# AdvancedPhotonSource/tike

Measured on AMD Instinct MI355X. Metric: diffraction patterns/sec/GPU (256x256, 8-mode probe), higher is better.
Workload: dtype c64; 1 GPU; c3; positions_per_gpu=10000, modes=8, detector=256, eigen_probes=1, solver=lstsq_grad, num_batch=10, chunk_positions=1000, position_correction=False, object_update=after every minibatch (batch_method wobbly_center), route=no_farplane

## Files before the change

include/tike_amd.h:

```cpp
#ifndef TIKE_AMD_H
#define TIKE_AMD_H

#ifdef __cplusplus
extern "C" {
#endif

#define TIKE_ERR_ARG 1000001
#define TIKE_ERR_UNSUPPORTED 1000002
#define TIKE_ERR_COMM 2000000
#define TIKE_COMM_ID_BYTES 128

#define TIKE_ABI_VERSION 25

const char* tike_build_id(void);

int tike_abi_version(void);

int tike_set_deterministic(int on, void* scratch, long bytes);

int tike_init(void);

int tike_patch_fwd(const void* images, void* patches, const float* positions, int nimage, int H,
                   int W, int nscan, int nrepeat, int patch_width, int padded_width,
                   void* stream);
// ... 219 lines not shown

int tike_gen_inv_rows_gradients(const void* hand2, const void* patches, const void* probe,
                                int probe_per_scan, const void* unique, const void* eigen_probe,
                                const float* eigen_weights, int num_eigen, int eigen_modes,
                                void* objproj, void* chi0, void* m_probe_update,
                                float probe_update_scale, int nscan, int S, int pw, int det,
                                float inv_scale, void* stream);

int tike_pfa_supported(int S, int pw, int det);

int tike_pfa_fwd_gather(const void* psi, const float* scan, const void* probe,
                        int probe_per_scan, const void* unique, const void* eigen_probe,
                        const float* eigen_weights, int num_eigen, int eigen_modes,
                        void* subtiles, void* patches, int nscan, int S, int pw, int det, int H,
                        int W, void* stream);

int tike_pfa_fft2(const void* in, void* out, long ntile, int det, int inverse, void* stream);

int tike_pfa_fwd_subtiles_supported(int S, int pw, int det);
int tike_pfa_fwd_subtiles(const void* psi, const float* scan, const void* probe,
                          const void* eigen_probe, const float* eigen_weights, int num_eigen,
                          int eigen_modes, void* probe_scratch, void* subtiles, void* patches,
                          int nscan, int S, int pw, int det, int H, int W, void* stream);

int tike_pfa_combine_gradient(void* subtiles, const float* data, const unsigned char* measured,
                              float* costs, int nscan, int S, int det, float fwd_scale, int model,
                              float unmeasured_scaling, long num_measured, int apply_gradient,
                              void* stream);

int tike_pfa_inv_products(const void* subtiles, const void* patches, const void* probe,
                          int probe_per_scan, const void* unique, const void* eigen_probe,
                          const float* eigen_weights, int num_eigen, int eigen_modes,
                          void* objproj, void* chi0, void* m_probe_update,
                          float probe_update_scale, int nscan, int S, int pw, int det,
                          float inv_scale, void* stream);


int tike_fft2_pass1(const void* in, void* out, long ntile, int det, int inverse, void* stream);

int tike_fft2_pass2_inplace(void* tiles, long ntile, int det, int inverse, float scale,
                            void* stream);

int tike_slice_step(void* wave, const void* psi, const float* scan, void* farplane1, int nscan,
                    int S, int det, int H, int W, float scale, void* stream);

int tike_slice_step_back(const void* work, const void* psi, const float* scan, const void* beam,
                         void* objproj, void* farplane1, int nscan, int S, int det, int H, int W,
                         float inv_scale, void* stream);

int tike_fft2_pass2_intensity(void* tiles, float* amplitude, long nscan, int S, int det,
                              int inverse, float scale, int keep, void* stream);

int tike_fresnel_colpass(const void* colin, const void* propagator, int adjoint, void* work,
                         long ntile, int det, float scale, void* stream);

int tike_ifft2_pass2_products(void* work, const void* psi, const float* scan, const void* probe,
                              int probe_per_scan, void* objproj, void* probe_numerator,
                              float numerator_scale, void* chi0, int keep_chi, int nscan, int S,
                              int det, int H, int W, float inv_scale, void* stream);

int tike_fresnel_spect_prop(const void* in, void* out, const void* propagator, long ntile, int n,
                            int adjoint, float fwd_scale, float inv_scale, void* stream);


int tike_object_update_precond(const float* acc, const void* precond, const float* pmax,
                               float alpha, void* upd_sum, void* upd_precond, float* combined,
                               long npix, void* stream);

int tike_lstsq_step_sums(const float* stats, const float* costs, int B, float eps, float* sums,
                         void* stream);
int tike_lstsq_step_solve(const float* stats, int B, float eps, const float* sums, double count,
                          int recover_psi, int recover_probe, float* out, void* stream);

int tike_probe_update(void* probe, void* combined, const void* mpu, const float* beta,
                      float inv_num_batch, long n, void* stream);

int tike_eigen_weights0(float* weights, const float* stats, int B, int C, int S, int m,
                        float* norms, void* stream);
int tike_eigen_proj_mean(const float* first, int first_stride, const float* weights_c,
                         long weights_row, const float* norm, long P, int B, float* pm,
                         void* stream);
int tike_eigen_normalise(void* eigen, const void* update, double count, float beta, int npix,
                         float* esum, float* work, void* stream);
int tike_eigen_dsum(const float* sums, int B, long P, float* dsum, void* stream);
int tike_eigen_weights(const float* sums, int B, long P, const float* dsum, double count,
                       float* weights_c, long weights_row, void* coefs_c, int coef_stride,
                       const float* esum, void* stream);

int tike_cgrad_direction(const float* update_planar, const void* update_complex, void* gradient,
                         void* direction, long n, int first, const float* costs, int ncost,
                         double count, double* state, double* sums, void* stream);

int tike_cgrad_line_search(int variable, const void* x, const void* d, void* xs,
                           const void* other, const float* scan, const void* data,
                           int data_u16, void* scratch, float* costs, int nscan, int chunk,
                           int S, int det, int H, int W, float fwd_scale, double count,
                           double* state, int* skip, int nslots, void* stream);

int tike_cgrad_line_search_masked(int variable, const void* x, const void* d, void* xs,
                                  const void* other, const float* scan, const void* data,
                                  int data_u16, void* scratch, float* costs, int nscan, int chunk,
                                  int S, int det, int H, int W, float fwd_scale, double count,
                                  double* state, int* skip, int nslots,
                                  const unsigned char* measured, int model, long num_measured,
                                  void* stream);

int tike_cgrad_line_search_linear(int variable, const void* x, const void* d, void* xs,
                                  const void* other, const float* scan, const void* data,
                                  int data_u16, void* far_a, int a_valid, void* far_b,
                                  float* costs_k, int nscan, int chunk, int S, int det, int H,
                                  int W, float fwd_scale, double count, double* state,
                                  int stage, double* sums, void* stream);

int tike_cgrad_line_search_linear_masked(int variable, const void* x, const void* d, void* xs,
                                         const void* other, const float* scan, const void* data,
                                         int data_u16, void* far_a, int a_valid, void* far_b,
                                         float* costs_k, int nscan, int chunk, int S, int det,
                                         int H, int W, float fwd_scale, double count,
                                         double* state, int stage, double* sums,
                                         const unsigned char* measured, int model,
                                         long num_measured, void* stream);

int tike_eigen_pixel_update1(const void* patches, const void* chi0, const void* mpu0,
                             const void* eigen0, const float* eigen_proj,
                             const float* weights_c, long weights_row, const float* norm,
                             void* update, int nscan, int pw, int chi_modes, const float* stats,
                             const float* costs, float eps, float* sums3, const void* psi,
                             const float* scan, int H, int W, void* stream);
int tike_lstsq_tail_mid(void* eigen0, const void* update, int npix, float* nacc,
                        float beta_eigen, const float* stats, int B, float eps,
                        const float* sums3, double count, int recover_psi, int recover_probe,
                        float* tail3, void* stream);
int tike_eigen_position_sums1(const void* patches, const void* chi0, const void* mpu0,
                              const void* eigen0, float* sums5, float* dsum, int nscan, int pw,
                              int chi_modes, const void* psi, const float* scan, int H, int W,
                              void* stream);
int tike_lstsq_tail_finish(const float* tail3, const float* sums3, double count, float* steps,
                           void* probe, void* combined, const void* mpu, float inv_num_batch,
                           long nprobe, float* weights, long weights_row, int S, int m,
                           const float* stats, const float* sums5, int B, int npix,
                           void* stream);

int tike_ifft2_pass2_gradients_eproj(const void* work, const void* patches, const void* probe,
                                     const void* eigen_probe, const float* eigen_weights,
                                     int num_eigen, int eigen_modes, void* objproj, void* chi0,
                                     void* m_probe_update, float mpu_scale, int nscan, int S,
                                     int det, float inv_scale, float* qtab, float* q,
                                     void* stream);
int tike_eigen_pixel_update1q(const void* patches, const void* chi0, const void* mpu0,
                              const void* eigen0, const float* q, const float* weights_c,
                              long weights_row, const float* norm, void* update, int nscan,
                              int pw, int chi_modes, const void* psi, const float* scan, int H,
                              int W, float* c0part, float* eproj_out, void* stream);
int tike_lstsq_step_stats_eigen1(const void* chi, const float* scan,
                                 const void* object_update_precond, const void* probe,
                                 const void* eigen_probe, const float* eigen_weights,
                                 int eigen_modes, const void* m_probe_update, const void* patches,
                                 const void* update, float* nacc, double count, float beta_eigen,
                                 float* stats, float* sums5, int nscan, int S, int chi_modes,
                                 int pw, int H, int W, void* stream);
int tike_lstsq_tail_solve1(void* eigen0, const void* update, int npix, const float* nacc,
                           float beta_eigen, const float* stats, const float* costs,
                           const float* sums5, int B, float eps, double count, int recover_psi,
                           int recover_probe, float* sums3, float* tail3, void* stream);

int tike_lstsq_chunk_gradients(const void* psi, const float* scan, const void* probe,
                               const void* eigen_probe, const float* eigen_weights,
                               int num_eigen, int eigen_modes, const void* data, int data_u16,
                               const unsigned char* measured, int model,
                               float unmeasured_scaling, long num_measured, void* scratch,
                               void* work, float* gscale, void* patches, float* costs,
                               void* objproj, void* chi0, void* m_probe_update,
                               float mpu_scale, float* object_acc, int nscan, int S, int det,
                               int H, int W, float fwd_scale, float inv_scale, void* stream);

int tike_lstsq_chunk_gradients_positions(
    const void* psi, const float* scan, const void* probe, const void* eigen_probe,
    const float* eigen_weights, int num_eigen, int eigen_modes, const void* data, int data_u16,
    const unsigned char* measured, int model, float unmeasured_scaling, long num_measured,
    void* scratch, void* work, float* gscale, void* patches, float* costs, void* objproj,
    void* chi0, void* m_probe_update, float mpu_scale, float* object_acc, int nscan, int S,
    int det, int H, int W, float fwd_scale, float inv_scale, const float* taps, int taps_radius,
    float* intensity_work, float* numerator, float* denominator, void* stream);

int tike_position_pd_sums(const void* far0, const void* far_dx, const void* far_dy,
                          const void* data, int data_u16, float inv_dx, float* sums,
                          float* costs, long nscan, int S, long npix, void* stream);

int tike_fly_farplane_gradient(void* farplane, const void* data, int data_u16,
                               const unsigned char* measured, float* intensity, float* costs,
                               int nframe, int fly, int S, int det, int model,
                               int apply_gradient, float unmeasured_scaling, long num_measured,
                               void* stream);

int tike_farplane_scale(void* farplane, const float* table, long nframe, int P, long npix,
                        float scale, void* stream);

int tike_scan_gradient(const void* objproj, const float* scan, const void* psi, float* grad,
                       long nscan, int pw, int H, int W, void* stream);

int tike_scan_gradient_slices(const void* objproj, long slice_stride, const float* scan,
                              const void* psi, float* grad, long nscan, int D, int pw, int H,
                              int W, void* stream);

int tike_eigen_probe_gradients(const void* chi, const float* scan, const void* psi,
                               const void* probe, const void* eigen_probe,
                               const float* eigen_weights, int num_eigen, int eigen_modes,
                               void* probe_grad, void* eigen_grad, float* weights_grad,
                               void* objproj, void* work, long nscan, int S, int pw, int H,
                               int W, void* stream);

int tike_conv_fwd_tangent(const void* psi, const void* dpsi, const float* scan,
                          const float* dscan, const void* probe, const void* dprobe,
                          void* nearplane, long nscan, int S, int pw, int det, int H, int W,
                          void* stream);

int tike_slice_wave_tangent(const void* psi, const void* dpsi, const float* scan,
                            const float* dscan, const void* beam, int beam_per_scan,
                            const void* dbeam, int dbeam_per_scan, void* dwave, long nscan,
                            int S, int pw, int H, int W, void* stream);

int tike_eigen_wave_tangent(const void* psi, const void* dpsi, const float* scan,
                            const float* dscan, const void* probe, const void* dprobe,
                            const void* eigen_probe, const void* deigen_probe,
                            const float* eigen_weights, const float* deigen_weights,
                            int num_eigen, int eigen_modes, void* nearplane, long nscan, int S,
                            int pw, int det, int H, int W, void* stream);

int tike_intensity_tangent(const void* farplane, const void* dfarplane, float* intensity,
                           float* dintensity, long nframe, int P, long npix, void* stream);

int tike_cost_factor(const void* farplane, const void* data, int data_u16,
                     const unsigned char* measured, const float* upstream, float* costs,
                     float* table, long nframe, int P, long npix, int model,
                     long num_measured, void* stream);

int tike_cost_curvature(const void* farplane, const void* dfarplane, const void* data,
                        int data_u16, const unsigned char* measured, const float* upstream,
                        float* costs, float* dcosts, float* table, long nframe, int P,
                        long npix, int model, float floor, long num_measured, void* stream);


int tike_dm_reflect(const void* psi, const float* scan, const void* probe, const void* waves,
                    void* nearplane, float relaxation, long nscan, int S, int pw, int det, int H,
                    int W, void* stream);

int tike_dm_update(void* waves, const void* chi, const void* psi, const float* scan,
                   const void* probe, float relaxation, double* change, long nscan, int S,
                   int pw, int det, int H, int W, void* stream);

int tike_comm_unique_id(void* id);
int tike_comm_create(const void* id, int nranks, int rank, void** comm);
int tike_comm_destroy(void* comm);
int tike_comm_allreduce_sum(void* comm, void* buf, long count, int f64, void* stream);
int tike_comm_broadcast(void* comm, void* buf, long nbytes, int root, void* stream);

int tike_cluster_farthest_fill(const float* points, long n, long* owner, int num_cluster,
                               long turns);
int tike_cluster_swap_sweep(const double* dist, long n, int k, long* label, const long* best,
                            const long* order, double* regret, int* moved);

#ifdef __cplusplus
}
#endif
#endif
```

tike_amd/_lib.py:

```python
import ctypes
import os
import re

import torch

_HERE = os.path.dirname(os.path.abspath(__file__))
LIB_PATH = os.environ.get("TIKE_AMD_LIB") or os.path.join(
    _HERE, "csrc", "libtike_amd.so")
HEADER_PATH = os.path.join(os.path.dirname(_HERE), "include", "tike_amd.h")

ABI_VERSION = 25
ERR_ARG = 1000001
ERR_UNSUPPORTED = 1000002
ERR_COMM = 2000000
COMM_ID_BYTES = 128

if not os.path.isfile(LIB_PATH):
    raise ImportError(
        f"{LIB_PATH} not found: build the HIP library first "
        "(`make -C tike_amd/csrc` or `python -c 'import __graft_entry__ as g; "
        "g.build()'`). tike_amd has no CPU fallback.")

lib = ctypes.CDLL(LIB_PATH)

_p = ctypes.c_void_p
_i = ctypes.c_int
_l = ctypes.c_long
_f = ctypes.c_float
_d = ctypes.c_double

_PROTOTYPES = {
    "tike_abi_version": [],
    "tike_max_grid_dim_y": [],
    "tike_init": [],
    "tike_set_deterministic": [_i, _p, _l],
    "tike_patch_fwd": [_p, _p, _p, _i, _i, _i, _i, _i, _i, _i, _p],
    "tike_patch_adj": [_p, _p, _p, _i, _i, _i, _i, _i, _i, _i, _i, _p],
    "tike_conv_fwd": [_p, _p, _p, _i, _p, _i, _i, _i, _i, _i, _i, _p],
    "tike_conv_adj": [_p, _p, _p, _i, _p, _i, _i, _i, _i, _i, _i, _p],
    "tike_conv_adj_probe": [_p, _p, _p, _p, _i, _i, _i, _i, _i, _i, _p],
    "tike_fft2": [_p, _p, _l, _i, _i, _f, _p],
    "tike_fft2_supported": [_i],
    "tike_fft2_general": [_p, _p, _l, _i, _i, _f, _i, _i, _p],
    "tike_pfa_supported": [_i, _i, _i],
    "tike_pfa_fwd_gather": [_p, _p, _p, _i, _p, _p, _p, _i, _i, _p, _p, _i, _i, _i,
                            _i, _i, _i, _p],
    "tike_pfa_fwd_subtiles_supported": [_i, _i, _i],
    "tike_pfa_fwd_subtiles": [_p, _p, _p, _p, _p, _i, _i, _p, _p, _p, _i, _i,
                              _i, _i, _i, _i, _p],
    "tike_pfa_fft2": [_p, _p, _l, _i, _i, _p],
    "tike_pfa_combine_gradient": [_p, _p, _p, _p, _i, _i, _i, _f, _i, _f, _l, _i,
                                  _p],
    "tike_pfa_inv_products": [_p, _p, _p, _i, _p, _p, _p, _i, _i, _p, _p, _p, _f,
                              _i, _i, _i, _i, _f, _p],
    "tike_gen_supported": [_i, _i, _i],
    "tike_gen_fwd_rows": [_p, _p, _p, _i, _p, _p, _p, _i, _i, _p, _p, _i, _i, _i,
                          _i, _i, _i, _p],
    "tike_gen_cols_gradient": [_p, _p, _p, _p, _p, _i, _i, _i, _i, _f, _i, _f,
                               _l, _p],
    "tike_gen_inv_rows_gradients": [_p, _p, _p, _i, _p, _p, _p, _i, _i, _p, _p,
                                    _p, _f, _i, _i, _i, _i, _f, _p],
    "tike_fresnel_spect_prop": [_p, _p, _p, _l, _i, _i, _f, _f, _p],
    "tike_fft2_pass1": [_p, _p, _l, _i, _i, _p],
    "tike_fft2_pass2_inplace": [_p, _l, _i, _i, _f, _p],
    "tike_slice_step": [_p, _p, _p, _p, _i, _i, _i, _i, _i, _f, _p],
    "tike_slice_step_back": [_p, _p, _p, _p, _p, _p, _i, _i, _i, _i, _i, _f,
                             _p],
    "tike_fft2_pass2_intensity": [_p, _p, _l, _i, _i, _i, _f, _i, _p],
    "tike_fresnel_colpass": [_p, _p, _i, _p, _l, _i, _f, _p],
    "tike_ifft2_pass2_products": [_p, _p, _p, _p, _i, _p, _p, _f, _p, _i, _i, _i,
                                  _i, _i, _i, _f, _p],
    "tike_ptycho_fwd": [_p, _p, _p, _i, _p, _p, _i, _i, _p, _i, _i, _i, _i,
                        _i, _i, _f, _i, _p],
    "tike_ptycho_adj": [_p, _p, _i, _p, _p, _p, _p, _p, _p, _i, _i, _i, _i, _i,
                        _i, _f, _i, _p],
    "tike_ifft2_crop": [_p, _p, _p, _l, _i, _i, _f, _p],
    "tike_ptycho_fwd_intensity": [_p, _p, _p, _i, _p, _p, _i, _i, _p, _p, _p,
                                  _i, _i, _i, _i, _i, _i, _f, _p],
    "tike_gradient_scale": [_p, _p, _p, _p, _p, _i, _i, _i, _f, _l, _p],
    "tike_ifft2_crop_scaled": [_p, _p, _i, _p, _p, _l, _i, _i, _f, _p],
    "tike_ifft2_crop_scaled_modes": [_p, _p, _p, _p, _i, _p, _p, _l, _i, _i, _f,
                                     _p],
    "tike_poisson_steps": [_p, _p, _p, _p, _p, _i, _i, _i, _f, _f, _i, _p],
    "tike_poisson_steps_handoff": [_p, _p, _i, _p, _p, _p, _p, _p, _i, _i, _i, _f,
                                   _f, _l, _f, _f, _p],
    "tike_scale_modes": [_p, _p, _p, _l, _i, _p],
    "tike_ptycho_fwd_intensity_only": [_p, _p, _p, _i, _p, _p, _i, _i, _p, _p,
                                       _i, _i, _i, _i, _i, _i, _f, _p],
    "tike_ptycho_fwd_gradient_scale": [_p, _p, _p, _i, _p, _p, _i, _i, _p, _p,
                                       _p, _p, _p, _p, _p, _i, _i, _i, _i, _i,
                                       _i, _f, _i, _f, _l, _p],
    "tike_fwd_pass1": [_p, _p, _p, _i, _p, _p, _p, _i, _i, _p, _p, _i, _i, _i,
                       _i, _i, _i, _p],
    "tike_fwd_gradient_scale": [_p, _p, _i, _p, _p, _p, _p, _p, _i, _i, _i, _f,
                                _i, _f, _l, _p],
    "tike_grad_ifft2_pass1": [_p, _p, _p, _p, _i, _p, _l, _i, _f, _p],
    "tike_fwd_grad_ifft2_pass1": [_p, _p, _i, _p, _p, _p, _i, _i, _i, _f, _i, _f,
                                  _l, _p],
    "tike_fwd_grad_ifft2_pass1_slices": [_p, _p, _i, _p, _p, _p, _i, _i, _i, _f, _i, _f,
                                  _l, _p, _i, _p],
    "tike_ifft2_pass1_scaled": [_p, _p, _p, _p, _i, _p, _l, _i, _p],
    "tike_ifft2_pass2_gradients": [_p, _p, _p, _p, _p, _i, _i, _p, _p, _p, _f,
                                   _i, _i, _i, _f, _p],
    "tike_ifft2_pass2_gradients_scaled": [_p, _p, _p, _p, _p, _i, _i, _p, _p,
                                          _p, _f, _i, _i, _i, _f, _p, _p],
    "tike_ifft2_pass2_eigen_fits": [_i, _i, _i],
    "tike_ifft2_pass2_gradients_modes": [_p, _p, _p, _p, _p, _i, _i, _p, _p,
                                         _p, _f, _i, _i, _i, _f, _i, _i, _i, _p],
    "tike_poisson_steps_grad_ifft2_pass1": [_p, _p, _i, _p, _p, _p, _p, _p, _i,
                                            _i, _i, _f, _f, _l, _f, _f, _p],
    "tike_object_update_precond": [_p, _p, _p, _f, _p, _p, _p, _l, _p],
    "tike_lstsq_step_sums": [_p, _p, _i, _f, _p, _p],
    "tike_lstsq_step_solve": [_p, _i, _f, _p, _d, _i, _i, _p, _p],
    "tike_probe_update": [_p, _p, _p, _p, _f, _l, _p],
    "tike_eigen_weights0": [_p, _p, _i, _i, _i, _i, _p, _p],
    "tike_eigen_proj_mean": [_p, _i, _p, _l, _p, _l, _i, _p, _p],
    "tike_eigen_normalise": [_p, _p, _d, _f, _i, _p, _p, _p],
    "tike_eigen_dsum": [_p, _i, _l, _p, _p],
    "tike_eigen_weights": [_p, _i, _l, _p, _d, _p, _l, _p, _i, _p, _p],
    "tike_grad_ifft2_crop": [_p, _p, _p, _p, _i, _p, _p, _l, _i, _i, _f, _f,
                             _p],
    "tike_position_sums": [_p, _p, _i, _p, _p, _p, _i, _i, _p, _i, _p, _p, _i,
                           _i, _i, _p],
    "tike_rpie_position_sums": [_p, _p, _p, _p, _i, _p, _p, _i, _i, _p, _i, _p,
                                _p, _p, _i, _i, _i, _i, _i, _p],
    "tike_farplane_gradient": [_p, _p, _p, _p, _p, _i, _i, _i, _i, _i, _f, _l,
                               _p],
    "tike_intensity": [_p, _p, _l, _i, _l, _p],
    "tike_cost_each_pattern": [_p, _p, _p, _l, _l, _i, _p],
    "tike_objective_grad": [_p, _p, _p, _p, _l, _i, _l, _i, _p],
    "tike_lstsq_gradients": [_p, _p, _p, _p, _p, _p, _i, _i, _p, _p, _p, _p, _i,
                             _i, _i, _i, _i, _p],
    "tike_varying_probe": [_p, _p, _p, _i, _i, _p, _i, _i, _i, _p],
    "tike_scatter_patches": [_p, _p, _p, _i, _i, _i, _i, _p],
    "tike_eigen_position_sums": [_p, _p, _p, _p, _p, _i, _i, _i, _p, _i, _i,
                                 _i, _p],
    "tike_eigen_pixel_update": [_p, _p, _p, _p, _p, _i, _i, _i, _p, _p, _i, _i,
                                _i, _p],
    "tike_probe_grad": [_p, _p, _p, _p, _p, _i, _i, _i, _i, _i, _p],
    "tike_probe_preconditioner": [_p, _p, _p, _i, _i, _i, _i, _p],
    "tike_psi_preconditioner": [_p, _p, _p, _i, _i, _i, _i, _p],
    "tike_scatter_amplitudes": [_p, _p, _p, _i, _i, _i, _i, _p],
    "tike_lstsq_step_stats": [_p, _p, _p, _p, _p, _p, _p, _i, _i, _p, _p, _p,
                              _p, _i, _i, _i, _i, _i, _i, _p, _p, _p],
    "tike_eigen_pixel_update1": [_p, _p, _p, _p, _p, _p, _l, _p, _p, _i, _i, _i,
                                 _p, _p, _f, _p, _p, _p, _i, _i, _p],
    "tike_lstsq_tail_mid": [_p, _p, _i, _p, _f, _p, _i, _f, _p, _d, _i, _i, _p,
                            _p],
    "tike_eigen_position_sums1": [_p, _p, _p, _p, _p, _p, _i, _i, _i, _p, _p,
                                  _i, _i, _p],
    "tike_lstsq_tail_finish": [_p, _p, _d, _p, _p, _p, _p, _f, _l, _p, _l, _i,
                               _i, _p, _p, _i, _i, _p],
    "tike_ifft2_pass2_gradients_eproj": [_p, _p, _p, _p, _p, _i, _i, _p, _p,
                                         _p, _f, _i, _i, _i, _f, _p, _p, _p],
    "tike_eigen_pixel_update1q": [_p, _p, _p, _p, _p, _p, _l, _p, _p, _i, _i,
                                  _i, _p, _p, _i, _i, _p, _p, _p],
    "tike_lstsq_step_stats_eigen1": [_p, _p, _p, _p, _p, _p, _i, _p, _p, _p,
                                     _p, _d, _f, _p, _p, _i, _i, _i, _i, _i,
                                     _i, _p],
    "tike_lstsq_tail_solve1": [_p, _p, _i, _p, _f, _p, _p, _p, _i, _f, _d, _i,
                               _i, _p, _p, _p],
    "tike_lstsq_chunk_gradients": [_p, _p, _p, _p, _p, _i, _i, _p, _i, _p, _i,
                                   _f, _l, _p, _p, _p, _p, _p, _p, _p, _p, _f,
                                   _p, _i, _i, _i, _i, _i, _f, _f, _p],
    "tike_lstsq_chunk_gradients_positions": [
        _p, _p, _p, _p, _p, _i, _i, _p, _i, _p, _i, _f, _l, _p, _p, _p, _p, _p,
        _p, _p, _p, _f, _p, _i, _i, _i, _i, _i, _f, _f, _p, _i, _p, _p, _p, _p],
    "tike_cgrad_direction": [_p, _p, _p, _p, _l, _i, _p, _i, _d, _p, _p, _p],
    "tike_cgrad_line_search": [_i, _p, _p, _p, _p, _p, _p, _i, _p, _p, _i, _i,
                               _i, _i, _i, _i, _f, _d, _p, _p, _i, _p],
    "tike_cgrad_line_search_linear": [_i, _p, _p, _p, _p, _p, _p, _i, _p, _i, _p,
                                      _p, _i, _i, _i, _i, _i, _i, _f, _d, _p, _i,
                                      _p, _p],
    "tike_cgrad_line_search_masked": [_i, _p, _p, _p, _p, _p, _p, _i, _p, _p,
                                      _i, _i, _i, _i, _i, _i, _f, _d, _p, _p,
                                      _i, _p, _i, _l, _p],
    "tike_cgrad_line_search_linear_masked": [_i, _p, _p, _p, _p, _p, _p, _i, _p,
                                             _i, _p, _p, _i, _i, _i, _i, _i, _i,
                                             _f, _d, _p, _i, _p, _p, _i, _l, _p],
    "tike_position_pd_sums": [_p, _p, _p, _p, _i, _f, _p, _p, _l, _i, _l, _p],
    "tike_fly_farplane_gradient": [_p, _p, _i, _p, _p, _p, _i, _i, _i, _i, _i,
                                   _i, _f, _l, _p],
    "tike_farplane_scale": [_p, _p, _l, _i, _l, _f, _p],
    "tike_scan_gradient": [_p, _p, _p, _p, _l, _i, _i, _i, _p],
    "tike_scan_gradient_slices": [_p, _l, _p, _p, _p, _l, _i, _i, _i, _i, _p],
    "tike_eigen_probe_gradients": [_p, _p, _p, _p, _p, _p, _i, _i, _p, _p, _p,
                                   _p, _p, _l, _i, _i, _i, _i, _p],
    "tike_conv_fwd_tangent": [_p, _p, _p, _p, _p, _p, _p, _l, _i, _i, _i, _i,
                              _i, _p],
    "tike_slice_wave_tangent": [_p, _p, _p, _p, _p, _i, _p, _i, _p, _l, _i, _i,
                                _i, _i, _p],
    "tike_intensity_tangent": [_p, _p, _p, _p, _l, _i, _l, _p],
    "tike_eigen_wave_tangent": [_p, _p, _p, _p, _p, _p, _p, _p, _p, _p, _i, _i,
                                _p, _l, _i, _i, _i, _i, _i, _p],
    "tike_cost_factor": [_p, _p, _i, _p, _p, _p, _p, _l, _i, _l, _i, _l, _p],
    "tike_cost_curvature": [_p, _p, _p, _i, _p, _p, _p, _p, _p, _l, _i, _l, _i,
                            _f, _l, _p],
    "tike_dm_reflect": [_p, _p, _p, _p, _p, _f, _l, _i, _i, _i, _i, _i, _p],
    "tike_dm_update": [_p, _p, _p, _p, _p, _f, _p, _l, _i, _i, _i, _i, _i, _p],
    "tike_comm_unique_id": [_p],
    "tike_comm_create": [_p, _i, _i, ctypes.POINTER(_p)],
    "tike_comm_destroy": [_p],
    "tike_comm_allreduce_sum": [_p, _p, _l, _i, _p],
    "tike_comm_broadcast": [_p, _p, _l, _i, _p],
    "tike_cluster_farthest_fill": [_p, _l, _p, _i, _l],
    "tike_cluster_swap_sweep": [_p, _l, _i, _p, _p, _p, _p, _p],
}


def build_id():
    try:
        fn = lib.tike_build_id
    except AttributeError:
        return ""
    fn.restype = ctypes.c_char_p
    fn.argtypes = []
    return fn().decode()


def declared_symbols():
    with open(HEADER_PATH) as f:
        text = f.read()
    return sorted(set(re.findall(r"^int\s+(tike_\w+)\s*\(", text, flags=re.M)))


for _name, _args in _PROTOTYPES.items():
    try:
        _fn = getattr(lib, _name)
    except AttributeError as e:
        raise ImportError(
            f"{LIB_PATH} does not export {_name}: it was built from another "
            "include/tike_amd.h; rebuild it (`make -C tike_amd/csrc`).") from e
    _fn.argtypes = _args
    _fn.restype = ctypes.c_int


def _check_abi_version():
    got = lib.tike_abi_version()
    m = re.search(r"^#define\s+TIKE_ABI_VERSION\s+(\d+)", open(HEADER_PATH).read(),
                  flags=re.M) if os.path.isfile(HEADER_PATH) else None
    if got != ABI_VERSION or (m and int(m.group(1)) != ABI_VERSION):
        raise ImportError(
            f"{LIB_PATH} reports ABI version {got}, include/tike_amd.h "
            f"{m.group(1) if m else '?'}, this binding expects {ABI_VERSION}: "
            "rebuild the library (`make -C tike_amd/csrc`).")


_check_abi_version()


def check(rc, what=""):
    if rc == 0:
        return
    if rc == ERR_ARG:
        raise ValueError(f"{what}: incompatible shapes / arguments")
    if rc == ERR_UNSUPPORTED:
        raise ValueError(f"{what}: unsupported size for the HIP path")
    if rc >= ERR_COMM:
        raise RuntimeError(f"{what}: RCCL error {rc - ERR_COMM}")
    raise RuntimeError(f"{what}: HIP error {rc}")


DETERMINISTIC = os.environ.get("TIKE_DETERMINISTIC", "0") == "1"
DETERMINISTIC_SCRATCH_MIB = int(os.environ.get("TIKE_DETERMINISTIC_MIB", "256"))
_det_scratch = None


def ensure_deterministic():
    global _det_scratch
    if not DETERMINISTIC:
        return
    current = torch.cuda.current_device()
    if _det_scratch is not None and _det_scratch.device.index == current:
        return
    if _det_scratch is not None:
        torch.cuda.synchronize(_det_scratch.device)
    _det_scratch = torch.empty(DETERMINISTIC_SCRATCH_MIB << 20,
                               dtype=torch.uint8,
                               device=torch.device("cuda", current))
    check(lib.tike_set_deterministic(1, _det_scratch.data_ptr(),
                                     _det_scratch.numel()),
          "tike_set_deterministic")
```

tike_amd/csrc/lstsq.hip:

```cpp
#include <type_traits>

#include "internal.h"
#include "tike_amd.h"

template <bool HAVE_PATCHES, bool HAVE_GOBJ>
__device__ __forceinline__ void step_stats_item(
    const cf* __restrict__ chi, const float* __restrict__ scan, const cf* __restrict__ psi,
    const cf* __restrict__ gobj, const TkProbe& probe, const cf* __restrict__ mpu,
    const cf* __restrict__ patches, float* __restrict__ stats, int chi_modes, int pw, int H,
    int W, const cf* __restrict__ eigen0, float* __restrict__ eigen_proj, int nsplit, int n,
    int part, float* red) {
  const long P = (long)pw * pw;
  const long total = (long)H * W;
  const int plen = (int)(P / nsplit);
  {
    const TkCorner c = tk_corner(scan, n);
    const cf* __restrict__ pbase = probe.probe + n * probe.pos_stride;
    float pw0 = 1.0f, pw1 = 0.f;
    int nE = 0;
    const float* __restrict__ wn = nullptr;
    if (probe.weights != nullptr) {
      if (probe.unique != nullptr && 0 < probe.Sm) {
        pbase = probe.unique + (long)n * probe.Sm * P;
      } else {
        wn = probe.weights + n * (long)(probe.C + 1) * probe.S;
        pw0 = wn[0];
        if (probe.eigen != nullptr && 0 < probe.Sm) {
          nE = probe.C;
          pw1 = wn[probe.S];
        }
      }
    }
    float a[8] = {0.f, 0.f, 0.f, 0.f, 0.f, 0.f, 0.f, 0.f};
    float ep = 0.f;
    const int qstep = (int)blockDim.x / pw, rstep = (int)blockDim.x % pw;
    const int pbeg = part * plen + (int)threadIdx.x;
    const int pend = part + 1 == nsplit ? (int)P : (part + 1) * plen;
    int py = pbeg / pw, px = pbeg % pw;
    const bool interior = HAVE_GOBJ && c.sy >= 0 && c.sx >= 0 && c.sy + pw < H && c.sx + pw < W &&
                          total < (1L << 28);
    const bool same_e = eigen_proj != nullptr && nE > 0 && eigen0 == probe.eigen;
    const bool same_p = pbase == probe.probe;
    auto body = [&](auto k_tag) {
      constexpr int K = decltype(k_tag)::value;
      constexpr bool FAST = K >= 1;
      constexpr bool HOT = K >= 2;
#pragma unroll 2
      for (int p = pbeg; p < pend; p += blockDim.x) {
        cf o, g;
        if (FAST) {
          typedef float tk_v4f __attribute__((ext_vector_type(4)));
          const unsigned off =
              (unsigned)((c.sy + py) * W + c.sx + px) * (unsigned)sizeof(cf);
          tk_v4f u, l;
          __builtin_memcpy(&u, reinterpret_cast<const char*>(gobj) + off, sizeof(u));
          __builtin_memcpy(&l, reinterpret_cast<const char*>(gobj) + off + (unsigned)W * 8u,
                           sizeof(l));
          if (HAVE_PATCHES) {
            o = patches[n * P + p];
          } else {
            tk_v4f uo, lo_;
            __builtin_memcpy(&uo, reinterpret_cast<const char*>(psi) + off, sizeof(uo));
            __builtin_memcpy(&lo_, reinterpret_cast<const char*>(psi) + off + (unsigned)W * 8u,
                             sizeof(lo_));
            o = mk(uo.x * c.w00, uo.y * c.w00);
            o.x += uo.z * c.w01;
            o.y += uo.w * c.w01;
            o.x += lo_.x * c.w10;
            o.y += lo_.y * c.w10;
            o.x += lo_.z * c.w11;
            o.y += lo_.w * c.w11;
          }
          g = mk(u.x * c.w00, u.y * c.w00);
          g.x += u.z * c.w01;
          g.y += u.w * c.w01;
          g.x += l.x * c.w10;
          g.y += l.y * c.w10;
          g.x += l.z * c.w11;
          g.y += l.w * c.w11;
        } else {
          const int y = c.sy + py, x = c.sx + px;
          const bool ok = y >= 0 && y < H && x >= 0 && x < W;
          const int yc = y < 0 ? 0 : (y >= H ? H - 1 : y);
          const int xc = x < 0 ? 0 : (x >= W ? W - 1 : x);
          const long ii = (long)yc * W + xc;
          o = HAVE_PATCHES ? patches[n * P + p] : tk_gather(psi, ii, W, total, c);
          g = HAVE_GOBJ ? tk_gather(gobj, ii, W, total, c) : mk(0.f, 0.f);
          if (!ok) {
            if (!HAVE_PATCHES) o = mk(0.f, 0.f);
            g = mk(0.f, 0.f);
          }
        }
        const cf x0 = chi[((long)n * chi_modes) * P + p];
        const cf p0 = probe.probe[p];
        cf pn = (HOT ? p0 : pbase[p]) * pw0;
        cf e1 = mk(0.f, 0.f);
        if (K == 3) {
          e1 = probe.eigen[p];
          pn.x += pw1 * e1.x;
          pn.y += pw1 * e1.y;
        } else if (K < 2 && nE > 0) {
          e1 = probe.eigen[p];
          pn.x += pw1 * e1.x;
          pn.y += pw1 * e1.y;
          for (int e = 1; e < nE; ++e) {
            const cf ee = probe.eigen[(long)e * probe.Sm * P + p];
            const float we = wn[(e + 1) * probe.S];
            pn.x += we * ee.x;
            pn.y += we * ee.y;
          }
        }
        const cf dOP = g * pn;
        const cf m0 = HOT ? mpu[p] : (mpu ? mpu[p] : mk(0.f, 0.f));
        const cf dPO = m0 * o;
        const cf OP = o * p0;
        a[0] += norm2(dOP);
        a[1] += norm2(dPO);
        const cf a2 = dOP * conjf(dPO);
        a[2] += a2.x;
        a[3] += a2.y;
        a[4] += dOP.x * x0.x + dOP.y * x0.y;
        a[5] += dPO.x * x0.x + dPO.y * x0.y;
        a[6] += OP.x * x0.x + OP.y * x0.y;
        a[7] += norm2(OP);
        if (K == 3) {
          const cf r = conjf(o) * x0 - m0;
          ep += r.x * e1.x + r.y * e1.y;
        } else if (K < 2 && eigen_proj) {
          const cf r = conjf(o) * x0 - m0;
          const cf e = same_e ? e1 : eigen0[p];
          ep += r.x * e.x + r.y * e.y;
        }
        py += qstep;
        px += rstep;
        if (px >= pw) {
          px -= pw;
          ++py;
        }
      }
    };
    const bool hot = interior && same_p && mpu != nullptr;
    if (hot && nE == 1 && same_e)
      body(std::integral_constant<int, 3>{});
    else if (hot && nE == 0 && eigen_proj == nullptr)
      body(std::integral_constant<int, 2>{});
    else if (interior)
      body(std::integral_constant<int, 1>{});
    else
      body(std::integral_constant<int, 0>{});
#pragma unroll
    for (int k = 0; k < 8; ++k) {
      const float t = tk_block_sum256(a[k], red);
      if (threadIdx.x == 0) {
        if (nsplit > 1)
          unsafeAtomicAdd(&stats[(long)n * 8 + k], t);
// ... 188 lines not shown
    }
  }
}

extern "C" int tike_lstsq_step_stats(const void* chi, const float* scan, const void* psi,
                                     const void* object_update_precond, const void* probe,
                                     const void* eigen_probe, const float* eigen_weights,
                                     int num_eigen, int eigen_modes, const void* unique_probe,
                                     const void* m_probe_update, const void* patches,
                                     float* stats, int nscan, int S, int chi_modes, int pw, int H,
                                     int W, const void* eigen0, float* eigen_proj, void* stream) {
  TK_ENTER();
  TK_CHECK_ARG(nscan >= 0 && S >= 1 && chi_modes >= 1 && pw >= 1 && H >= 1 && W >= 1);
  if (nscan == 0) return TK_OK;
  TK_CHECK_ARG(chi && scan && psi && probe && stats);
  TK_CHECK_ARG(!eigen_proj || (eigen0 && m_probe_update));
  const TkProbe pr = tk_make_probe(probe, 0, eigen_probe, eigen_weights, num_eigen, eigen_modes,
                                   S, pw, unique_probe);
  const bool no_eigen = (eigen_probe == nullptr || eigen_modes == 0) && eigen_proj == nullptr;
  const bool one_eigen = eigen_probe != nullptr && eigen_weights != nullptr && eigen_modes > 0 &&
                         num_eigen == 1 && eigen_proj != nullptr && eigen0 == eigen_probe;
  const bool pairs = g_stats_pairs && patches && object_update_precond && m_probe_update &&
                     unique_probe == nullptr && (no_eigen || one_eigen) &&
                     (long)H * W < (1L << 28) && nscan > 1;
  const long nitem = pairs ? (nscan + 1) / 2 : nscan;
  int nsplit = 1;
  while (nsplit < 16 && nitem * nsplit * 2 <= 8192 && ((long)pw * pw) % (2048L * nsplit) == 0)
    nsplit *= 2;
  if (tk_deterministic()) nsplit = 1;
  if (nsplit > 1) {
    hipError_t e = hipMemsetAsync(stats, 0, sizeof(float) * 8 * (size_t)nscan, (hipStream_t)stream);
    if (e == hipSuccess && eigen_proj)
      e = hipMemsetAsync(eigen_proj, 0, sizeof(float) * (size_t)nscan, (hipStream_t)stream);
    if (e != hipSuccess) return (int)e;
  }
#define TK_SS(HP, HG)                                                                         \
  hipLaunchKernelGGL((step_stats_kernel<HP, HG>), dim3(tk_grid((long)nscan * nsplit, 16)),    \
                     dim3(256), 0,                                                            \
                     (hipStream_t)stream, (const cf*)chi, scan, (const cf*)psi,               \
                     (const cf*)object_update_precond, pr, (const cf*)m_probe_update,         \
                     (const cf*)patches, stats, nscan, chi_modes, pw, H, W, (const cf*)eigen0, \
                     eigen_proj, nsplit)
#define TK_SP(EIG)                                                                            \
  hipLaunchKernelGGL((step_stats_pair_kernel<EIG>), dim3(tk_grid(nitem * nsplit, 16)),        \
                     dim3(256), 0,                                                            \
                     (hipStream_t)stream, (const cf*)chi, scan, (const cf*)psi,               \
                     (const cf*)object_update_precond, pr, (const cf*)m_probe_update,         \
                     (const cf*)patches, stats, nscan, chi_modes, pw, H, W, (const cf*)eigen0, \
                     eigen_proj, nsplit)
  if (pairs && one_eigen) TK_SP(true);
  else if (pairs) TK_SP(false);
  else if (patches && object_update_precond) TK_SS(true, true);
  else if (patches) TK_SS(true, false);
  else if (object_update_precond) TK_SS(false, true);
  else TK_SS(false, false);
#undef TK_SS
#undef TK_SP
  TK_LAUNCH_CHECK();
  return TK_OK;
}

struct TkResidual {
  const cf* patches;
  const cf* chi0;
  const cf* mpu0;
  const cf* eigen;
  const cf* coefs;
  int C, Sm, c;
  long P;
  long XS;
  template <bool C0>
  __device__ __forceinline__ cf at(long n, long p) const {
    cf r = conjf(patches[n * P + p]) * chi0[n * XS + p] - mpu0[p];
    if (!C0)
      for (int k = 0; k < c; ++k) r = r - coefs[n * C + k] * eigen[((long)k * Sm) * P + p];
    return r;
  }
};

template <bool C0>
__global__ __launch_bounds__(256) void eigen_position_sums_kernel(const TkResidual R,
                                                                  float* __restrict__ sums,
                                                                  int nscan) {
  __shared__ float red[4];
  const cf* __restrict__ E = R.eigen + ((long)R.c * R.Sm) * R.P;
  for (int n = blockIdx.x; n < nscan; n += gridDim.x) {
    float a[5] = {0.f, 0.f, 0.f, 0.f, 0.f};
    for (long p = threadIdx.x; p < R.P; p += blockDim.x) {
      const cf e = E[p];
      const cf r = R.at<C0>(n, p);
      const cf phi = R.patches[n * R.P + p] * e;
      const cf x = R.chi0[n * R.XS + p];
      a[0] += r.x * e.x + r.y * e.y;
      a[1] += x.x * phi.x + x.y * phi.y;
      a[2] += norm2(phi);
      const cf re = r * conjf(e);
      a[3] += re.x;
      a[4] += re.y;
    }
#pragma unroll
    for (int k = 0; k < 5; ++k) {
      const float v = tk_block_sum256(a[k], red);
      if (threadIdx.x == 0) sums[(long)n * 5 + k] = v;
    }
  }
}

template <bool C0>
__global__ __launch_bounds__(256) void eigen_pixel_update_kernel(const TkResidual R,
                                                                 const float* __restrict__ pm,
                                                                 float* __restrict__ update,
                                                                 int nscan, int chunk,
                                                                 float* __restrict__ part) {
  const long p = (long)blockIdx.x * blockDim.x + threadIdx.x;
  if (p >= R.P) return;
  const int b0 = blockIdx.y * chunk;
  const int b1 = min(nscan, b0 + chunk);
  cf acc = mk(0.f, 0.f);
#pragma unroll 4
  for (int n = b0; n < b1; ++n) {
    const cf r = R.at<C0>(n, p);
    const float w = pm[n];
    acc.x += r.x * w;
    acc.y += r.y * w;
  }
  if (part != nullptr) {
    part[2 * ((long)blockIdx.y * R.P + p)] = acc.x;
    part[2 * ((long)blockIdx.y * R.P + p) + 1] = acc.y;
    return;
  }
  unsafeAtomicAdd(&update[2 * p], acc.x);
  unsafeAtomicAdd(&update[2 * p + 1], acc.y);
}

__device__ __forceinline__ cf tk_patch_pixel(const cf* __restrict__ psi, unsigned off,
                                             unsigned row_bytes, const TkCorner& c) {
  typedef float tk_v4f __attribute__((ext_vector_type(4)));
  tk_v4f u, l;
  __builtin_memcpy(&u, reinterpret_cast<const char*>(psi) + off, sizeof(u));
  __builtin_memcpy(&l, reinterpret_cast<const char*>(psi) + off + row_bytes, sizeof(l));
  cf o = mk(u.x * c.w00, u.y * c.w00);
  o.x += u.z * c.w01;
  o.y += u.w * c.w01;
  o.x += l.x * c.w10;
  o.y += l.y * c.w10;
  o.x += l.z * c.w11;
  o.y += l.w * c.w11;
  return o;
}
__device__ __forceinline__ bool tk_interior(const TkCorner& c, int pw, int H, int W) {
  return c.sy >= 0 && c.sx >= 0 && c.sy + pw < H && c.sx + pw < W && (long)H * W < (1L << 28);
}

constexpr int TK_C0_PARTS = 64;
__global__ __launch_bounds__(256) void eigen_proj_offset_kernel(const cf* __restrict__ mpu0,
                                                                const cf* __restrict__ E,
                                                                long P,
                                                                float* __restrict__ part) {
  __shared__ float red[4];
  float a = 0.f;
  for (long p = blockIdx.x * 256L + threadIdx.x; p < P; p += 256L * TK_C0_PARTS) {
    const cf m = mpu0[p], e = E[p];
    a += m.x * e.x + m.y * e.y;
  }
  a = tk_block_sum256(a, red);
  if (threadIdx.x == 0) part[blockIdx.x] = a;
}

__global__ __launch_bounds__(256) void eigen_pixel_update1_kernel(
    const TkResidual R, const float* __restrict__ eproj, const float* __restrict__ weights_c,
    long row, const float* __restrict__ norm, float inv_P, float* __restrict__ update, int nscan,
    int chunk, const float* __restrict__ stats, const float* __restrict__ costs, float eps,
    float* __restrict__ sums3, const cf* __restrict__ psi, const float* __restrict__ scan, int pw,
    int H, int W, float* __restrict__ part, const float* __restrict__ c0part,
    float* __restrict__ eproj_out) {
  float c0 = 0.f;
  if (c0part != nullptr) {
    for (int b = 0; b < TK_C0_PARTS; ++b) c0 += c0part[b];
  }
  if (blockIdx.x + 1 == gridDim.x) {
    if (blockIdx.y != 0) return;
    if (eproj_out != nullptr) {
      for (int n = threadIdx.x; n < nscan; n += 256) eproj_out[n] = eproj[n] - c0;
    }
    if (sums3 == nullptr) return;
    __shared__ float red[4];
    float a1 = 0.f, a4 = 0.f, c = 0.f;
    for (int n = threadIdx.x; n < nscan; n += 256) {
      a1 += stats[8 * n] + eps;
      a4 += stats[8 * n + 1] + eps;
      c += costs[n];
    }
    a1 = tk_block_sum256(a1, red);
    a4 = tk_block_sum256(a4, red);
    c = tk_block_sum256(c, red);
    if (threadIdx.x == 0) {
      sums3[0] = a1;
      sums3[1] = a4;
      sums3[2] = c;
    }
    return;
  }
  const long p = (long)blockIdx.x * blockDim.x + threadIdx.x;
  if (p >= R.P) return;
  const int b0 = blockIdx.y * chunk;
  const int b1 = min(nscan, b0 + chunk);
  const float inv_norm = 1.0f / norm[0];
  cf acc = mk(0.f, 0.f);
  bool gather = psi != nullptr;
  if (gather) {
    for (int n = b0; n < b1; ++n) gather = gather && tk_interior(tk_corner(scan, n), pw, H, W);
  }
  if (gather) {
    const int py = (int)(p / pw), px = (int)(p % pw);
    const unsigned row_bytes = (unsigned)W * (unsigned)sizeof(cf);
    const unsigned lane_off = (unsigned)py * row_bytes + (unsigned)px * (unsigned)sizeof(cf);
    const cf m0 = R.mpu0[p];
#pragma unroll 4
    for (int n = b0; n < b1; ++n) {
      const TkCorner c = tk_corner(scan, n);
      const cf x = R.chi0[n * R.XS + p];
      const cf o = tk_patch_pixel(
          psi, (unsigned)(c.sy * W + c.sx) * (unsigned)sizeof(cf) + lane_off, row_bytes, c);
      const cf r = conjf(o) * x - m0;
      const float w = ((eproj[n] - c0) * inv_P + weights_c[n * row]) * inv_norm;
      acc.x += r.x * w;
      acc.y += r.y * w;
    }
  } else {
#pragma unroll 4
    for (int n = b0; n < b1; ++n) {
      const cf r = R.at<true>(n, p);
      const float w = ((eproj[n] - c0) * inv_P + weights_c[n * row]) * inv_norm;
      acc.x += r.x * w;
      acc.y += r.y * w;
    }
  }
  if (part != nullptr) {
    part[2 * ((long)blockIdx.y * R.P + p)] = acc.x;
    part[2 * ((long)blockIdx.y * R.P + p) + 1] = acc.y;
    return;
  }
  unsafeAtomicAdd(&update[2 * p], acc.x);
  unsafeAtomicAdd(&update[2 * p + 1], acc.y);
}

__global__ __launch_bounds__(256) void column_sum_ordered_kernel(const float* __restrict__ table,
                                                                 int stride, int col, int n,
                                                                 float scale,
                                                                 float* __restrict__ out) {
  __shared__ float red[4];
  float a = 0.f;
  for (int i = threadIdx.x; i < n; i += 256) a += table[(long)i * stride + col] * scale;
  a = tk_block_sum256(a, red);
  if (threadIdx.x == 0) out[0] += a;
}

__global__ __launch_bounds__(256) void eigen_position_sums1_kernel(
    const TkResidual R, float* __restrict__ sums, float* __restrict__ dsum, int nscan,
    const cf* __restrict__ psi, const float* __restrict__ scan, int pw, int H, int W) {
  __shared__ float red[4];
  const cf* __restrict__ E = R.eigen;
  const unsigned row_bytes = (unsigned)W * (unsigned)sizeof(cf);
  const int qstep = (int)blockDim.x / pw, rstep = (int)blockDim.x % pw;
  for (int n = blockIdx.x; n < nscan; n += gridDim.x) {
    float a[5] = {0.f, 0.f, 0.f, 0.f, 0.f};
    TkCorner c = {0, 0, 0.f, 0.f, 0.f, 0.f};
    if (psi != nullptr) c = tk_corner(scan, n);
    const bool gather = psi != nullptr && tk_interior(c, pw, H, W);
    const unsigned off0 = gather ? (unsigned)(c.sy * W + c.sx) * (unsigned)sizeof(cf) : 0u;
    auto body = [&](auto g_tag) {
      constexpr bool G = decltype(g_tag)::value;
      int py = (int)threadIdx.x / pw, px = (int)threadIdx.x % pw;
      for (long p = threadIdx.x; p < R.P; p += blockDim.x) {
        const cf e = E[p];
        const cf x = R.chi0[n * R.XS + p];
        const cf m0 = R.mpu0[p];
        cf o;
        if constexpr (G)
          o = tk_patch_pixel(psi, off0 + (unsigned)py * row_bytes + (unsigned)px * 8u, row_bytes, c);
        else
          o = R.patches[n * R.P + p];
        const cf r = conjf(o) * x - m0;
        const cf phi = o * e;
        py += qstep;
        px += rstep;
        if (px >= pw) {
          px -= pw;
          ++py;
        }
        a[0] += r.x * e.x + r.y * e.y;
        a[1] += x.x * phi.x + x.y * phi.y;
        a[2] += norm2(phi);
        const cf re = r * conjf(e);
        a[3] += re.x;
        a[4] += re.y;
      }
    };
    if (gather)
      body(std::true_type{});
    else
      body(std::false_type{});
#pragma unroll
    for (int k = 0; k < 5; ++k) {
      const float v = tk_block_sum256(a[k], red);
      if (threadIdx.x == 0) {
        sums[(long)n * 5 + k] = v;
        if (k == 2 && dsum != nullptr) unsafeAtomicAdd(dsum, v / (float)R.P);
      }
    }
  }
}

__global__ __launch_bounds__(512) void eigen_position_sums1_pair_kernel(
    const TkResidual R, float* __restrict__ sums, float* __restrict__ dsum, int nscan,
    const cf* __restrict__ psi, const float* __restrict__ scan, int pw, int H, int W) {
  __shared__ float red[8];
  typedef float tk_v4f __attribute__((ext_vector_type(4)));
  const cf* __restrict__ E = R.eigen;
// ... 100 lines not shown
  const float mu = sqrtf(uu * inv_count * inv_count / (float)P);
  const float kk = beta / mu * inv_count;
  const float inv = 1.0f / sqrtf((ee + 2.0f * kk * eu + kk * kk * uu) / (float)P);
  auto enew = [&](const cf e, const long p) { return (e + update[p] * kk) * inv; };
  auto esum = [](float* a, const cf o, const cf x, const cf e, const cf m0) {
    const cf r = conjf(o) * x - m0;
    const cf phi = o * e;
    a[0] += r.x * e.x + r.y * e.y;
    a[1] += x.x * phi.x + x.y * phi.y;
    a[2] += norm2(phi);
    a[3] += r.y * e.x - r.x * e.y;
  };
  auto put = [&](float* dst, const float v) {
    if (nsplit > 1)
      unsafeAtomicAdd(dst, v);
    else
      *dst = v;
  };
  auto finish5 = [&](const float* a, const int n) {
    float t[4];
#pragma unroll
    for (int k = 0; k < 4; ++k) t[k] = tk_block_sum256(a[k], red);
    if (threadIdx.x == 0) {
      float* o = sums5 + (long)n * 5;
      put(o, t[0]);
      put(o + 1, t[1]);
      put(o + 2, t[2]);
      put(o + 3, t[0]);
      put(o + 4, t[3]);
    }
  };
  for (int v = blockIdx.x; v < npair * nsplit; v += gridDim.x) {
    const int n0 = 2 * (v / nsplit), part = v % nsplit;
    const TkCorner c0 = tk_corner(scan, n0);
    const bool two = n0 + 1 < nscan;
    const TkCorner c1 = tk_corner(scan, two ? n0 + 1 : n0);
    const bool in0 = c0.sy >= 0 && c0.sx >= 0 && c0.sy + pw < H && c0.sx + pw < W;
    const bool in1 = c1.sy >= 0 && c1.sx >= 0 && c1.sy + pw < H && c1.sx + pw < W;
    const int pbeg = part * plen + (int)threadIdx.x;
    const int pend = part + 1 == nsplit ? (int)P : (part + 1) * plen;
    if (!(two && in0 && in1)) {
      for (int i = 0; i < (two ? 2 : 1); ++i) {
        const int n = n0 + i;
        step_stats_item<true, true>(chi, scan, nullptr, gobj, probe, mpu, patches, stats,
                                    chi_modes, pw, H, W, nullptr, nullptr, nsplit, n, part, red);
        float a[4] = {0.f, 0.f, 0.f, 0.f};
        for (int p = pbeg; p < pend; p += blockDim.x)
          esum(a, patches[(long)n * P + p], chi[(long)n * chi_modes * P + p],
               enew(probe.eigen[p], p), mpu[p]);
        finish5(a, n);
      }
      continue;
    }
    float s0 = 1.0f, s1 = 1.0f, t0 = 0.f, t1 = 0.f;
    if (probe.weights != nullptr) {
      const float* w = probe.weights + n0 * (long)(probe.C + 1) * probe.S;
      s0 = w[0];
      s1 = w[(long)(probe.C + 1) * probe.S];
      t0 = w[probe.S];
      t1 = w[(long)(probe.C + 1) * probe.S + probe.S];
    }
    float a[8] = {0.f, 0.f, 0.f, 0.f, 0.f, 0.f, 0.f, 0.f};
    float b[8] = {0.f, 0.f, 0.f, 0.f, 0.f, 0.f, 0.f, 0.f};
    float ea[4] = {0.f, 0.f, 0.f, 0.f}, eb[4] = {0.f, 0.f, 0.f, 0.f};
    const unsigned base0 = (unsigned)(c0.sy * W + c0.sx), base1 = (unsigned)(c1.sy * W + c1.sx);
    const cf* __restrict__ chi_a = chi + ((long)n0 * chi_modes) * P;
    const cf* __restrict__ chi_b = chi + ((long)(n0 + 1) * chi_modes) * P;
    const cf* __restrict__ pat_a = patches + (long)n0 * P;
    const cf* __restrict__ pat_b = pat_a + P;
    auto tap = [](const tk_v4f u, const tk_v4f l, const TkCorner& c) {
      cf g = mk(u.x * c.w00, u.y * c.w00);
      g.x += u.z * c.w01;
      g.y += u.w * c.w01;
      g.x += l.x * c.w10;
      g.y += l.y * c.w10;
      g.x += l.z * c.w11;
      g.y += l.w * c.w11;
      return g;
    };
    auto sums = [](float* acc, const cf g, const cf o, const cf x0, const cf p0, const cf pn,
                   const cf m0) {
      const cf dOP = g * pn;
      const cf dPO = m0 * o;
      const cf OP = o * p0;
      acc[0] += norm2(dOP);
      acc[1] += norm2(dPO);
      const cf a2 = dOP * conjf(dPO);
      acc[2] += a2.x;
      acc[3] += a2.y;
      acc[4] += dOP.x * x0.x + dOP.y * x0.y;
      acc[5] += dPO.x * x0.x + dPO.y * x0.y;
      acc[6] += OP.x * x0.x + OP.y * x0.y;
      acc[7] += norm2(OP);
    };
    auto pixel = [&](const int p, const tk_v4f u0, const tk_v4f l0, const tk_v4f u1,
                     const tk_v4f l1) {
      const cf oa = pat_a[p], ob = pat_b[p];
      const cf xa = chi_a[p], xb = chi_b[p];
      const cf p0 = probe.probe[p];
      const cf m0 = mpu[p];
      const cf e1 = probe.eigen[p];
      const cf en = enew(e1, p);
      cf pa = p0 * s0, pb = p0 * s1;
      pa.x += t0 * e1.x;
      pa.y += t0 * e1.y;
      pb.x += t1 * e1.x;
      pb.y += t1 * e1.y;
      sums(a, tap(u0, l0, c0), oa, xa, p0, pa, m0);
      sums(b, tap(u1, l1, c1), ob, xb, p0, pb, m0);
      esum(ea, oa, xa, en, m0);
      esum(eb, ob, xb, en, m0);
    };
    auto taps16 = [&](const unsigned off) {
      tk_v4f t;
      __builtin_memcpy(&t, reinterpret_cast<const char*>(gobj) + off, sizeof(t));
      return t;
    };
    const int cols = pw < 256 ? pw : 256, groups = 256 / cols;
    const int rows = pw / (nsplit * groups);
    const int ybeg = (part * groups + (int)threadIdx.x / cols) * rows;
    for (int x = (int)threadIdx.x % cols; x < pw; x += 256) {
      unsigned rel = (unsigned)(ybeg * W + x);
      tk_v4f u0 = taps16((base0 + rel) * 8u), u1 = taps16((base1 + rel) * 8u);
      int p = ybeg * pw + x;
#pragma unroll 2
      for (int y = 0; y < rows; ++y) {
        rel += (unsigned)W;
        const tk_v4f l0 = taps16((base0 + rel) * 8u), l1 = taps16((base1 + rel) * 8u);
        pixel(p, u0, l0, u1, l1);
        u0 = l0;
        u1 = l1;
        p += pw;
      }
    }
#pragma unroll
    for (int k = 0; k < 8; ++k) {
      const float ta = tk_block_sum256(a[k], red);
      const float tb = tk_block_sum256(b[k], red);
      if (threadIdx.x == 0) {
        put(&stats[(long)n0 * 8 + k], ta);
        put(&stats[(long)n0 * 8 + 8 + k], tb);
      }
    }
    finish5(ea, n0);
    finish5(eb, n0 + 1);
  }
}

__global__ __launch_bounds__(256) void eigen_norm_sums1_kernel(const cf* __restrict__ E,
                                                               const cf* __restrict__ update,
                                                               int npix, float* __restrict__ nacc,
                                                               float* __restrict__ part) {
  __shared__ float red[4];
  float uu = 0.f, ee = 0.f, eu = 0.f;
  for (int i = blockIdx.x * 256 + threadIdx.x; i < npix; i += gridDim.x * 256) {
    const cf e = E[i], u = update[i];
    uu += norm2(u);
    ee += norm2(e);
    eu += e.x * u.x + e.y * u.y;
  }
  uu = tk_block_sum256(uu, red);
  ee = tk_block_sum256(ee, red);
  eu = tk_block_sum256(eu, red);
  if (threadIdx.x == 0) {
    if (part != nullptr) {
      part[3 * blockIdx.x] = uu;
      part[3 * blockIdx.x + 1] = ee;
      part[3 * blockIdx.x + 2] = eu;
    } else {
      unsafeAtomicAdd(&nacc[0], uu);
      unsafeAtomicAdd(&nacc[1], ee);
      unsafeAtomicAdd(&nacc[2], eu);
    }
  }
}

extern "C" int tike_lstsq_step_stats_eigen1(const void* chi, const float* scan,
                                            const void* object_update_precond, const void* probe,
                                            const void* eigen_probe, const float* eigen_weights,
                                            int eigen_modes, const void* m_probe_update,
                                            const void* patches, const void* update, float* nacc,
                                            double count, float beta_eigen, float* stats,
                                            float* sums5, int nscan, int S, int chi_modes,
                                            int pw, int H, int W, void* stream) {
  TK_ENTER();
  TK_CHECK_ARG(nscan >= 0 && S >= 1 && chi_modes >= 1 && pw >= 1 && H >= 1 && W >= 1 &&
               eigen_modes >= 1 && count > 0);
  TK_CHECK_ARG(probe && eigen_probe && eigen_weights && m_probe_update && update && nacc);
  const long P = (long)pw * pw;
  const long nitem = (nscan + 1) / 2;
  int nsplit = 1;
  while (nsplit < 16 && nitem * nsplit * 2 <= 8192 && P % (2048L * nsplit) == 0) nsplit *= 2;
  if (tk_deterministic()) nsplit = 1;
  const int groups = 256 / (pw < 256 ? pw : 256);
  if (!((pw % 256 == 0 || 256 % pw == 0) && pw % (nsplit * groups) == 0 &&
        (long)H * W < (1L << 28)))
    return TK_ERR_UNSUPPORTED;
  int grid = P >= 256 * 64 ? 64 : (int)((P + 255) / 256);
  float* part = nullptr;
  if (tk_deterministic()) {
    part = tk_det_scratch(sizeof(float) * 3 * (size_t)grid);
    if (part == nullptr) grid = 1;
  }
  hipLaunchKernelGGL(eigen_norm_sums1_kernel, dim3(grid), dim3(256), 0, (hipStream_t)stream,
                     (const cf*)eigen_probe, (const cf*)update, (int)P, nacc, part);
  TK_LAUNCH_CHECK();
  if (part != nullptr) {
    int rc = tk_ordered_sum(nacc, part, 3, grid, true, (hipStream_t)stream);
    if (rc) return rc;
  }
  if (nscan == 0) return TK_OK;
  TK_CHECK_ARG(chi && scan && object_update_precond && patches && stats && sums5);
  const TkProbe pr = tk_make_probe(probe, 0, eigen_probe, eigen_weights, 1, eigen_modes, S, pw,
                                   nullptr);
  if (nsplit > 1) {
    hipError_t e = hipMemsetAsync(stats, 0, sizeof(float) * 8 * (size_t)nscan, (hipStream_t)stream);
    if (e == hipSuccess)
      e = hipMemsetAsync(sums5, 0, sizeof(float) * 5 * (size_t)nscan, (hipStream_t)stream);
    if (e != hipSuccess) return (int)e;
  }
  hipLaunchKernelGGL(step_stats_eigen_pair_kernel, dim3(tk_grid(nitem * nsplit, 16)), dim3(256),
                     0, (hipStream_t)stream, (const cf*)chi, scan,
                     (const cf*)object_update_precond, pr, (const cf*)m_probe_update,
                     (const cf*)patches, (const cf*)update, (const float*)nacc,
                     (float)(1.0 / count), beta_eigen, stats, sums5, nscan, chi_modes, pw, H, W,
                     nsplit);
  TK_LAUNCH_CHECK();
  return TK_OK;
}

static TkResidual make_residual(const void* patches, const void* chi0, const void* mpu0,
                                const void* eigen, const void* coefs, int C, int Sm, int c,
                                int pw, int chi_modes) {
  TkResidual R;
  R.patches = (const cf*)patches;
  R.chi0 = (const cf*)chi0;
  R.mpu0 = (const cf*)mpu0;
  R.eigen = (const cf*)eigen;
  R.coefs = (const cf*)coefs;
  R.C = C;
  R.Sm = Sm;
  R.c = c;
  R.P = (long)pw * pw;
  R.XS = R.P * chi_modes;
  return R;
}

extern "C" int tike_eigen_position_sums(const void* patches, const void* chi0, const void* mpu0,
                                        const void* eigen_probe, const void* coefs,
                                        int num_eigen, int eigen_modes, int c, float* sums,
                                        int nscan, int pw, int chi_modes, void* stream) {
  TK_ENTER();
  TK_CHECK_ARG(nscan >= 0 && pw >= 1 && num_eigen >= 1 && c >= 0 && c < num_eigen &&
               chi_modes >= 1);
  if (nscan == 0) return TK_OK;
  TK_CHECK_ARG(patches && chi0 && mpu0 && eigen_probe && sums && (c == 0 || coefs));
  const TkResidual R = make_residual(patches, chi0, mpu0, eigen_probe, coefs, num_eigen,
                                     eigen_modes, c, pw, chi_modes);
  if (c == 0)
    hipLaunchKernelGGL(eigen_position_sums_kernel<true>, dim3(tk_grid(nscan, 16)), dim3(256), 0,
                       (hipStream_t)stream, R, sums, nscan);
  else
    hipLaunchKernelGGL(eigen_position_sums_kernel<false>, dim3(tk_grid(nscan, 16)), dim3(256),
                       0, (hipStream_t)stream, R, sums, nscan);
  TK_LAUNCH_CHECK();
  return TK_OK;
}

extern "C" int tike_eigen_pixel_update(const void* patches, const void* chi0, const void* mpu0,
                                       const void* eigen_probe, const void* coefs,
                                       int num_eigen, int eigen_modes, int c, const float* pm,
                                       void* update, int nscan, int pw, int chi_modes,
                                       void* stream) {
  TK_ENTER();
  TK_CHECK_ARG(nscan >= 0 && pw >= 1 && num_eigen >= 1 && c >= 0 && c < num_eigen &&
               chi_modes >= 1);
  if (nscan == 0) return TK_OK;
  TK_CHECK_ARG(patches && chi0 && mpu0 && eigen_probe && pm && update && (c == 0 || coefs));
  const long P = (long)pw * pw;
  float* part = nullptr;
  const int chunk = probe_chunk(nscan, 2 * P, &part);
  dim3 grid((unsigned)((P + 255) / 256), (unsigned)((nscan + chunk - 1) / chunk));
  const TkResidual R = make_residual(patches, chi0, mpu0, eigen_probe, coefs, num_eigen,
                                     eigen_modes, c, pw, chi_modes);
  if (c == 0)
    hipLaunchKernelGGL(eigen_pixel_update_kernel<true>, grid, dim3(256), 0, (hipStream_t)stream,
                       R, pm, (float*)update, nscan, chunk, part);
  else
    hipLaunchKernelGGL(eigen_pixel_update_kernel<false>, grid, dim3(256), 0,
                       (hipStream_t)stream, R, pm, (float*)update, nscan, chunk, part);
  TK_LAUNCH_CHECK();
  if (part != nullptr)
    return tk_ordered_sum((float*)update, part, 2 * P, (int)grid.y, true, (hipStream_t)stream);
  return TK_OK;
}

extern "C" int tike_eigen_pixel_update1(const void* patches, const void* chi0,
                                        const void* mpu0, const void* eigen0,
                                        const float* eigen_proj, const float* weights_c,
                                        long weights_row, const float* norm, void* update,
                                        int nscan, int pw, int chi_modes, const float* stats,
                                        const float* costs, float eps, float* sums3,
                                        const void* psi, const float* scan, int H, int W,
                                        void* stream) {
  TK_ENTER();
  TK_CHECK_ARG(nscan >= 0 && pw >= 1 && chi_modes >= 1 && weights_row >= 1);
  if (nscan == 0) {
    if (sums3) return (int)hipMemsetAsync(sums3, 0, 3 * sizeof(float), (hipStream_t)stream);
    return TK_OK;
  }
  TK_CHECK_ARG(!sums3 || (stats && costs));
  TK_CHECK_ARG(!psi || (scan && H >= 1 && W >= 1));
  TK_CHECK_ARG(patches && chi0 && mpu0 && eigen0 && eigen_proj && weights_c && norm && update);
  const long P = (long)pw * pw;
  float* part = nullptr;
  const int chunk = probe_chunk(nscan, 2 * P, &part);
  dim3 grid((unsigned)((P + 255) / 256) + 1, (unsigned)((nscan + chunk - 1) / chunk));
  const TkResidual R = make_residual(patches, chi0, mpu0, eigen0, nullptr, 1, 1, 0, pw, chi_modes);
  hipLaunchKernelGGL(eigen_pixel_update1_kernel, grid, dim3(256), 0, (hipStream_t)stream, R,
                     eigen_proj, weights_c, weights_row, norm, 1.0f / (float)P, (float*)update,
                     nscan, chunk, stats, costs, eps, sums3, (const cf*)psi, scan, pw, H, W,
                     part, nullptr, nullptr);
  TK_LAUNCH_CHECK();
  if (part != nullptr)
    return tk_ordered_sum((float*)update, part, 2 * P, (int)grid.y, true, (hipStream_t)stream);
  return TK_OK;
}

extern "C" int tike_eigen_pixel_update1q(const void* patches, const void* chi0,
                                         const void* mpu0, const void* eigen0, const float* q,
                                         const float* weights_c, long weights_row,
                                         const float* norm, void* update, int nscan, int pw,
                                         int chi_modes, const void* psi, const float* scan,
                                         int H, int W, float* c0part, float* eproj_out,
                                         void* stream) {
  TK_ENTER();
  TK_CHECK_ARG(nscan >= 0 && pw >= 1 && chi_modes >= 1 && weights_row >= 1);
  if (nscan == 0) return TK_OK;
  TK_CHECK_ARG(!psi || (scan && H >= 1 && W >= 1));
  TK_CHECK_ARG(patches && chi0 && mpu0 && eigen0 && q && weights_c && norm && update && c0part);
  const long P = (long)pw * pw;
  hipLaunchKernelGGL(eigen_proj_offset_kernel, dim3(TK_C0_PARTS), dim3(256), 0,
                     (hipStream_t)stream, (const cf*)mpu0, (const cf*)eigen0, P, c0part);
  float* part = nullptr;
  const int chunk = probe_chunk(nscan, 2 * P, &part);
  dim3 grid((unsigned)((P + 255) / 256) + 1, (unsigned)((nscan + chunk - 1) / chunk));
  const TkResidual R = make_residual(patches, chi0, mpu0, eigen0, nullptr, 1, 1, 0, pw, chi_modes);
  hipLaunchKernelGGL(eigen_pixel_update1_kernel, grid, dim3(256), 0, (hipStream_t)stream, R, q,
                     weights_c, weights_row, norm, 1.0f / (float)P, (float*)update, nscan, chunk,
                     nullptr, nullptr, 0.f, nullptr, (const cf*)psi, scan, pw, H, W, part,
                     c0part, eproj_out);
  TK_LAUNCH_CHECK();
  if (part != nullptr)
    return tk_ordered_sum((float*)update, part, 2 * P, (int)grid.y, true, (hipStream_t)stream);
  return TK_OK;
}

extern "C" int tike_eigen_position_sums1(const void* patches, const void* chi0,
                                         const void* mpu0, const void* eigen0, float* sums,
                                         float* dsum, int nscan, int pw, int chi_modes,
                                         const void* psi, const float* scan, int H, int W,
                                         void* stream) {
  TK_ENTER();
  TK_CHECK_ARG(nscan >= 0 && pw >= 1 && chi_modes >= 1);
  if (nscan == 0) return TK_OK;
  TK_CHECK_ARG(!psi || (scan && H >= 1 && W >= 1));
  TK_CHECK_ARG(patches && chi0 && mpu0 && eigen0 && sums && dsum);
  const TkResidual R = make_residual(patches, chi0, mpu0, eigen0, nullptr, 1, 1, 0, pw, chi_modes);
  const bool det = tk_deterministic();
  const int cols = pw < 256 ? pw : 256;
  const bool pairs = g_stats_pairs && psi != nullptr && nscan > 1 &&
                     (pw % 256 == 0 || 256 % pw == 0) && pw % (512 / cols) == 0 &&
                     (long)H * W < (1L << 28);
  if (pairs)
    hipLaunchKernelGGL(eigen_position_sums1_pair_kernel, dim3(tk_grid((nscan + 1) / 2, 16)),
                       dim3(512), 0, (hipStream_t)stream, R, sums, det ? nullptr : dsum, nscan,
                       (const cf*)psi, scan, pw, H, W);
  else
    hipLaunchKernelGGL(eigen_position_sums1_kernel, dim3(tk_grid(nscan, 16)), dim3(256), 0,
                       (hipStream_t)stream, R, sums, det ? nullptr : dsum, nscan, (const cf*)psi,
                       scan, pw, H, W);
  if (det)
    hipLaunchKernelGGL(column_sum_ordered_kernel, dim3(1), dim3(256), 0, (hipStream_t)stream, sums,
                       5, 2, nscan, 1.0f / (float)((long)pw * pw), dsum);
  TK_LAUNCH_CHECK();
  return TK_OK;
}

__global__ __launch_bounds__(256) void varying_probe_kernel(const TkProbe probe,
                                                            cf* __restrict__ out, long total,
                                                            long PP) {
  for (long i = blockIdx.x * (long)blockDim.x + threadIdx.x; i < total;
       i += (long)gridDim.x * blockDim.x) {
    const long pix = i % PP;
    const long ns = i / PP;
    out[i] = probe.at(ns / probe.Sm, (int)(ns % probe.Sm), pix);
  }
}

extern "C" int tike_varying_probe(const void* probe, const void* eigen_probe,
                                  const float* eigen_weights, int num_eigen, int eigen_modes,
                                  void* out, int nscan, int S, int pw, void* stream) {
  TK_ENTER();
  TK_CHECK_ARG(nscan >= 0 && S >= 1 && pw >= 1 && eigen_modes >= 1 && eigen_modes <= S);
  if (nscan == 0) return TK_OK;
  TK_CHECK_ARG(probe && eigen_weights && out && (num_eigen == 0 || eigen_probe));
  const long PP = (long)pw * pw;
  const long total = (long)nscan * eigen_modes * PP;
  hipLaunchKernelGGL(varying_probe_kernel, dim3(tk_grid((total + 255) / 256, 16)), dim3(256), 0,
                     (hipStream_t)stream,
                     tk_make_probe(probe, 0, eigen_probe, eigen_weights, num_eigen, eigen_modes,
                                   S, pw),
                     (cf*)out, total, PP);
  TK_LAUNCH_CHECK();
  return TK_OK;
}
```

tike_amd/csrc/lstsq_gradients.hip:

```cpp
#include "fft_engine2.h"
#include <type_traits>

#include "internal.h"
#include "tike_amd.h"

constexpr int TK_MAX_MODES = 16;

template <bool WITH_CHI, int SC>
__global__ __launch_bounds__(256) void probe_grad_kernel(
    const cf* __restrict__ chi, const float* __restrict__ scan, const cf* __restrict__ psi,
    cf* __restrict__ patches, float* __restrict__ out, const TkProbe probe,
    cf* __restrict__ objproj, int nscan, int S_rt, int pw, int H, int W, int chunk,
    float* __restrict__ part) {
  constexpr int SM = SC > 0 ? SC : TK_MAX_MODES;
  const int S = SC > 0 ? SC : S_rt;
  const long P = (long)pw * pw;
  const long total = (long)H * W;
  const long p = (long)blockIdx.x * blockDim.x + threadIdx.x;
  const int b0 = blockIdx.y * chunk;
  const int b1 = min(nscan, b0 + chunk);
  if (p >= P) return;
  const int py = (int)(p / pw), px = (int)(p % pw);
  cf acc[SM];
#pragma unroll
  for (int s = 0; s < SM; ++s) acc[s] = mk(0.f, 0.f);
  const bool hoist = WITH_CHI && objproj != nullptr && probe.pos_stride == 0;
  cf pr[SM];
  if (hoist) {
#pragma unroll
    for (int s = 0; s < SM; ++s)
      if (SC > 0 || s < S) pr[s] = probe.probe[s * P + p];
  }
  for (int b = b0; b < b1; ++b) {
    const TkCorner c = tk_corner(scan, b);
    const int y = c.sy + py, x = c.sx + px;
    const bool ok = y >= 0 && y < H && x >= 0 && x < W;
    const int yc = y < 0 ? 0 : (y >= H ? H - 1 : y);
    const int xc = x < 0 ? 0 : (x >= W ? W - 1 : x);
    cf xs[SM];
    if (WITH_CHI) {
#pragma unroll
      for (int s = 0; s < SM; ++s)
        if (SC > 0 || s < S) xs[s] = tk_ld_stream(chi + ((long)b * S + s) * P + p);
    }
    cf o;
    if (!WITH_CHI && c.sy >= 0 && c.sx >= 0 && c.sy + pw < H && c.sx + pw < W &&
        total < (1L << 28)) {
      typedef float tk_v4f __attribute__((ext_vector_type(4)));
      const unsigned off = (unsigned)(y * W + x) * (unsigned)sizeof(cf);
      tk_v4f u, l;
      __builtin_memcpy(&u, reinterpret_cast<const char*>(psi) + off, sizeof(u));
      __builtin_memcpy(&l, reinterpret_cast<const char*>(psi) + off + (unsigned)W * 8u, sizeof(l));
      o = mk(u.x * c.w00, u.y * c.w00);
      o.x += u.z * c.w01;
      o.y += u.w * c.w01;
      o.x += l.x * c.w10;
      o.y += l.y * c.w10;
      o.x += l.z * c.w11;
      o.y += l.w * c.w11;
    } else {
      o = tk_gather(psi, (long)yc * W + xc, W, total, c);
      if (!ok) o = mk(0.f, 0.f);
    }
    if (patches) patches[b * P + p] = o;
    if (WITH_CHI) {
      const cf oc = conjf(o);
      cf proj = mk(0.f, 0.f);
#pragma unroll
      for (int s = 0; s < SM; ++s)
        if (SC > 0 || s < S) {
          if (out) acc[s] = acc[s] + oc * xs[s];
          if (objproj) {
            cf ps;
            if (hoist && !(probe.weights != nullptr && probe.eigen != nullptr && s < probe.Sm)) {
              const float w0 =
                  probe.weights ? probe.weights[b * (long)(probe.C + 1) * probe.S + s] : 1.0f;
              ps = pr[s] * w0;
            } else {
              ps = probe.at(b, s, p);
            }
            proj = proj + conjf(ps) * xs[s];
          }
        }
      if (objproj) objproj[b * P + p] = proj;
    } else {
      acc[0].x += norm2(o);
    }
  }
  if (WITH_CHI) {
    if (out) {
#pragma unroll
      for (int s = 0; s < SM; ++s)
        if (SC > 0 || s < S) {
          if (part != nullptr) {
            float* o = part + 2 * (((long)blockIdx.y * S + s) * P + p);
            o[0] = acc[s].x;
            o[1] = acc[s].y;
          } else {
            unsafeAtomicAdd(&out[2 * (s * P + p)], acc[s].x);
            unsafeAtomicAdd(&out[2 * (s * P + p) + 1], acc[s].y);
          }
        }
    }
  } else if (part != nullptr) {
    part[(long)blockIdx.y * P + p] = acc[0].x;
  } else {
    unsafeAtomicAdd(&out[2 * p], acc[0].x);
  }
}

template <bool WITH_CHI>
static void launch_probe_grad(dim3 grid, hipStream_t stream, const cf* chi, const float* scan,
                              const cf* psi, cf* patches, float* out, const TkProbe& probe,
                              cf* objproj, int nscan, int S, int pw, int H, int W, int chunk,
                              float* part = nullptr) {
#define TK_PG(SC)                                                                              \
  hipLaunchKernelGGL((probe_grad_kernel<WITH_CHI, SC>), grid, dim3(256), 0, stream, chi, scan, \
                     psi, patches, out, probe, objproj, nscan, S, pw, H, W, chunk, part)
  switch (WITH_CHI ? S : 1) {
    case 1: TK_PG(1); break;
    case 2: TK_PG(2); break;
    case 3: TK_PG(3); break;
    case 4: TK_PG(4); break;
    case 5: TK_PG(5); break;
    case 6: TK_PG(6); break;
    case 8: TK_PG(8); break;
    default: TK_PG(0); break;
  }
#undef TK_PG
}

int probe_chunk(int nscan, long len, float** part) {
  int chunk = (nscan + 31) / 32;
  chunk = chunk < 8 ? 8 : chunk;
  if (!tk_deterministic()) return chunk;
  const int nchunk = (nscan + chunk - 1) / chunk;
  float* p = len > 0 && part ? tk_det_scratch(sizeof(float) * (size_t)len * nchunk) : nullptr;
  if (p != nullptr) {
    *part = p;
    return chunk;
  }
  return nscan > 8 ? nscan : 8;
}

extern "C" int tike_probe_grad(const void* chi, const float* scan, const void* psi,
                               void* patches, void* m_probe_update, int nscan, int S, int pw,
                               int H, int W, void* stream) {
  TK_ENTER();
  TK_CHECK_ARG(nscan >= 0 && S >= 1 && S <= TK_MAX_MODES && pw >= 1 && H >= 1 && W >= 1);
  if (nscan == 0) return TK_OK;
  TK_CHECK_ARG(chi && scan && psi && m_probe_update);
  const long P = (long)pw * pw;
  float* part = nullptr;
  const int chunk = probe_chunk(nscan, 2 * S * P, &part);
  dim3 grid((unsigned)((P + 255) / 256), (unsigned)((nscan + chunk - 1) / chunk));
  launch_probe_grad<true>(grid, (hipStream_t)stream, (const cf*)chi, scan, (const cf*)psi,
// ... 125 lines not shown
#pragma unroll
      for (int yb = 0; yb < RB; ++yb) O[yb] = *tk_at(On + yb * ROW, lo);
    }
    cf* slot = part + ((((n - b0) & (NBUF - 1)) * 4 + w) * RB) * 64 + lane;
    const cf* slots = part + ((((n - b0) & (NBUF - 1)) * 4 + cw * MW) * RB) * 64 + lane;
    const float* __restrict__ wn =
        vary ? probe.weights + n * (long)(probe.C + 1) * probe.S : nullptr;
#pragma unroll
    for (int m = 0; m < MPW; ++m) {
      const int s = mw + MW * m;
      if (s < S) {
        const cf* __restrict__ src = mid + ((long)n * Stot + s) * P + slice0;
        cf u[RB];
#pragma unroll
        for (int k = 0; k < RB; ++k) u[k] = tk_ld_stream(tk_at(src + k * ROW, lo));
        if (HOIST && !O_ONCE) {
#pragma unroll
          for (int yb = 0; yb < RB; ++yb) O[yb] = *tk_at(On + yb * ROW, lo);
        }
        const float w0 = vary ? wn[s] : 1.0f;
        const float sc = mode_scale ? inv_scale * mode_scale[(long)n * Stot + s] : inv_scale;
        Dft<RB, true>::run(u);
        if (HOIST) {
#pragma unroll
          for (int yb = 0; yb < RB; ++yb) {
            u[yb] = u[yb] * sc;
            acc[m][yb] = acc[m][yb] + conjf(O[yb]) * u[yb];
          }
          if (QN && !REDUCE && s == 0) {
            const cf* __restrict__ el = eigl + cw * 64 + lane;
            float q = 0.f;
#pragma unroll
            for (int yb = 0; yb < RB; ++yb) {
              const cf t = conjf(O[yb]) * u[yb];
              const cf e = el[yb * (64 * CW)];
              q += t.x * e.x - t.y * e.y;
            }
            q_store(q, n);
          }
        } else {
#pragma unroll
          for (int g = 0; g < RB; g += 8) {
            cf o[8];
#pragma unroll
            for (int i = 0; i < 8; ++i) o[i] = *tk_at(On + (g + i) * ROW, lo);
#pragma unroll
            for (int i = 0; i < 8; ++i) {
              u[g + i] = u[g + i] * sc;
              acc[m][g + i] = acc[m][g + i] + conjf(o[i]) * u[g + i];
            }
            __builtin_amdgcn_sched_barrier(0);
          }
        }
        if (s == 0 && chi0 != nullptr) {
#pragma unroll
          for (int yb = 0; yb < RB; ++yb)
            tk_st_stream(tk_at(chi0 + (long)n * P + slice0 + yb * ROW, lo), u[yb]);
        }
        if (HAVE_PROJ) {
          const cf* __restrict__ Ps = probe.probe + (long)s * P + slice0;
          const bool eig = EIG && nE > 0 && s < probe.Sm;
#pragma unroll
          for (int g = 0; g < RB; g += 8) {
            cf pc[8];
#pragma unroll
            for (int i = 0; i < 8; ++i)
              pc[i] = HOIST ? Pc[m][g + i] : conjf(*tk_at(Ps + (g + i) * ROW, lo));
#pragma unroll
            for (int i = 0; i < 8; ++i) {
              cf t = (pc[i] * u[g + i]) * w0;
              if (REDUCE) {
                slot[(g + i) * 64] = m == 0 ? t : slot[(g + i) * 64] + t;
              } else {
                if (eig) {
#pragma unroll 1
                  for (int c = 0; c < nE; ++c)
                    t = t + (eigl[((c * probe.Sm + s) * RB + g + i) * (64 * CW) + cw * 64 + lane] *
                             u[g + i]) * wn[(c + 1) * probe.S + s];
                }
                tk_st_stream(tk_at(objproj + (long)n * P + slice0 + (g + i) * ROW, lo), t);
              }
            }
            if (!HOIST) __builtin_amdgcn_sched_barrier(0);
          }
          if (REDUCE && eig) {
#pragma unroll 1
            for (int c = 0; c < nE; ++c) {
              const float wc = wn[(c + 1) * probe.S + s];
              const cf* __restrict__ el =
                  eigl + ((c * probe.Sm + s) * RB) * (64 * CW) + cw * 64 + lane;
              if (QN && c == 0 && s == 0) {
                float q = 0.f;
#pragma unroll
                for (int yb = 0; yb < RB; ++yb) {
                  const cf e = el[yb * (64 * CW)];
                  slot[yb * 64] = slot[yb * 64] + (e * u[yb]) * wc;
                  const cf t = conjf(O[yb]) * u[yb];
                  q += t.x * e.x - t.y * e.y;
                }
                q_store(q, n);
                continue;
              }
#pragma unroll
              for (int yb = 0; yb < RB; ++yb)
                slot[yb * 64] = slot[yb * 64] + (el[yb * (64 * CW)] * u[yb]) * wc;
            }
          }
        }
      } else if (REDUCE && m == 0) {
#pragma unroll
        for (int yb = 0; yb < RB; ++yb) slot[yb * 64] = mk(0.f, 0.f);
      }
    }
    if (REDUCE) {
      __syncthreads();
#pragma unroll
      for (int q = 0; q < RB / MW; ++q) {
        const int yb = mw + MW * q;
        cf sum = slots[yb * 64];
#pragma unroll
        for (int k = 1; k < MW; ++k) sum = sum + slots[(k * RB + yb) * 64];
        if (accumulate) sum = sum + *tk_at(objproj + (long)n * P + slice0 + yb * ROW, lo);
        tk_st_stream(tk_at(objproj + (long)n * P + slice0 + yb * ROW, lo), sum);
      }
      if (NBUF == 1) __syncthreads();
    }
  }
  if (mpu != nullptr) {
#pragma unroll
    for (int m = 0; m < MPW; ++m) {
      const int s = mw + MW * m;
      if (s < S) {
#pragma unroll
        for (int yb = 0; yb < RB; ++yb) {
          if (mpu_part != nullptr) {
            const long ci = (nchunk_ - 1) - b0 / chunk;
            float* o = tk_at(mpu_part + 2 * ((ci * S + s) * P + slice0 + yb * ROW), lb);
            o[0] = acc[m][yb].x * mpu_scale;
            o[1] = acc[m][yb].y * mpu_scale;
          } else {
            float* o = tk_at(mpu + 2 * ((long)s * P + slice0 + yb * ROW), lb);
            unsafeAtomicAdd(o, acc[m][yb].x * mpu_scale);
            unsafeAtomicAdd(o + 1, acc[m][yb].y * mpu_scale);
          }
        }
      }
    }
  }
}

__global__ __launch_bounds__(256) void pass2_q_finish_kernel(const float* __restrict__ qtab,
                                                             int slots, int nscan,
                                                             float* __restrict__ q) {
  const int n = blockIdx.x * 4 + (int)(threadIdx.x >> 6), k = threadIdx.x & 63;
  if (n >= nscan) return;
  float a = k < slots ? qtab[(long)k * nscan + n] : 0.f;
  a = tk_wave_sum(a);
  if (k == 0) q[n] = a;
}

template <int N, int MW_, int MPW_>
static bool launch_pass2_qn(dim3 grid, size_t lds, hipStream_t stream, const cf* work,
                            const cf* patches, const TkProbe& pr, cf* objproj, cf* chi0,
                            float* mpu, float mpu_scale, int nscan, int S, float inv_scale,
                            int chunk, float* mpu_part, const float* mode_scale, float* qtab) {
  if constexpr (N <= 256) {
    hipLaunchKernelGGL((ifft2_pass2_gradients_kernel<N, MW_, MPW_, true, true, false, true>),
                       grid, dim3(256), lds, stream, work, patches, pr, objproj, chi0, mpu,
                       mpu_scale, nscan, S, inv_scale, chunk, mpu_part, mode_scale, 0, 0, qtab);
    return true;
  } else {
    return false;
  }
}

static int launch_pass2_gradients(const void* work, const void* patches, const void* probe,
                                  const void* eigen_probe, const float* eigen_weights,
                                  int num_eigen, int eigen_modes, void* objproj, void* chi0,
                                  void* m_probe_update, float mpu_scale, int nscan, int S,
                                  int det, float inv_scale, const float* mode_scale,
                                  hipStream_t stream, int Stot = 0, int accumulate = 0,
                                  float* qtab = nullptr, float* q = nullptr) {
  TK_CHECK_ARG(nscan >= 0 && S >= 1 && det >= 1);
  if (nscan == 0) return TK_OK;
  TK_CHECK_ARG(work && patches && (probe || !objproj));
  if (S > 8 || (det != 128 && det != 256 && det != 512)) return TK_ERR_UNSUPPORTED;
  const bool qn = q != nullptr;
  TK_CHECK_ARG(!qn || qtab);
  if (qn && (Stot != 0 || det > 256 || !objproj || !eigen_probe || !eigen_weights ||
             num_eigen < 1 || eigen_modes < 1))
    return TK_ERR_UNSUPPORTED;
  const bool grp = Stot != 0;
  if (grp && objproj && S < 2) return TK_ERR_UNSUPPORTED;
  const TkProbe pr = tk_make_probe(probe, 0, eigen_probe, eigen_weights, num_eigen, eigen_modes,
                                   grp ? Stot : S, det);
  int MW = S >= 3 ? 4 : S;
  if (det == 128 && MW == 1) MW = 2;
  auto eig_bytes = [&](int mw) {
    return sizeof(cf) * (size_t)num_eigen * eigen_modes * (det / 16) * 64 * (4 / mw);
  };
  if (objproj && eigen_weights && eigen_probe)
    while (MW < 4 && eig_bytes(MW) > 32 * 1024) MW *= 2;
  const int MPW = S > 4 ? 2 : 1;
  const int nslice = 16 * (det / (64 * (4 / MW)));
  int nchunk = (1024 + nslice - 1) / nslice;
  {
    int unit = 512, a = nslice;
    while (a % 2 == 0 && unit > 1) { a /= 2; unit /= 2; }
    if (nchunk >= unit) nchunk = nchunk / unit * unit;
  }
  int chunk = (nscan + nchunk - 1) / nchunk;
  if (chunk < 8) chunk = 8;
  nchunk = (nscan + chunk - 1) / chunk;
  const dim3 grid((unsigned)(nslice * nchunk)), block(256);
  float* mpu_part = nullptr;
  const long mpu_len = 2L * S * det * det;
  if (m_probe_update && tk_deterministic()) {
    mpu_part = tk_det_scratch(sizeof(float) * (size_t)mpu_len * nchunk);
    if (mpu_part == nullptr) return TK_ERR_ARG;
  }
  size_t eig_lds = 0;
  if (objproj && eigen_weights && eigen_probe) eig_lds = eig_bytes(MW);
  if (eig_lds > 32 * 1024) return TK_ERR_UNSUPPORTED;
#define TK_P2G(N, MW_, MPW_)                                                                 \
  do {                                                                                       \
    if (qn) {                                                                                \
      if (!launch_pass2_qn<N, MW_, MPW_>(grid, eig_lds, stream, (const cf*)work,             \
                                         (const cf*)patches, pr, (cf*)objproj, (cf*)chi0,    \
                                         (float*)m_probe_update, mpu_scale, nscan, S,        \
                                         inv_scale, chunk, mpu_part, mode_scale, qtab))      \
        return TK_ERR_UNSUPPORTED;                                                           \
    } else if (grp && !objproj)                                                              \
      hipLaunchKernelGGL((ifft2_pass2_gradients_kernel<N, MW_, MPW_, false, true, true>),    \
                         grid, block, 0,                                                     \
                         stream, (const cf*)work, (const cf*)patches, pr, (cf*)objproj,      \
                         (cf*)chi0, (float*)m_probe_update, mpu_scale, nscan, S, inv_scale,  \
                         chunk, mpu_part, mode_scale, Stot, accumulate);                     \
    else if (grp && eig_lds > 0)                                                             \
      hipLaunchKernelGGL((ifft2_pass2_gradients_kernel<N, MW_, MPW_, true, true, true>),     \
                         grid, block, eig_lds,                                               \
                         stream, (const cf*)work, (const cf*)patches, pr, (cf*)objproj,      \
                         (cf*)chi0, (float*)m_probe_update, mpu_scale, nscan, S, inv_scale,  \
                         chunk, mpu_part, mode_scale, Stot, accumulate);                     \
    else if (grp)                                                                            \
      hipLaunchKernelGGL((ifft2_pass2_gradients_kernel<N, MW_, MPW_, true, false, true>),    \
                         grid, block, 0,                                                     \
                         stream, (const cf*)work, (const cf*)patches, pr, (cf*)objproj,      \
                         (cf*)chi0, (float*)m_probe_update, mpu_scale, nscan, S, inv_scale,  \
                         chunk, mpu_part, mode_scale, Stot, accumulate);                     \
    else if (objproj && eig_lds > 0)                                                         \
      hipLaunchKernelGGL((ifft2_pass2_gradients_kernel<N, MW_, MPW_, true>), grid, block,    \
                         eig_lds,                                                            \
                         stream, (const cf*)work, (const cf*)patches, pr, (cf*)objproj,      \
                         (cf*)chi0, (float*)m_probe_update, mpu_scale, nscan, S, inv_scale,  \
                         chunk, mpu_part, mode_scale);                                       \
    else if (objproj)                                                                        \
      hipLaunchKernelGGL((ifft2_pass2_gradients_kernel<N, MW_, MPW_, true, false>), grid,    \
                         block, 0,                                                           \
                         stream, (const cf*)work, (const cf*)patches, pr, (cf*)objproj,      \
                         (cf*)chi0, (float*)m_probe_update, mpu_scale, nscan, S, inv_scale,  \
                         chunk, mpu_part, mode_scale);                                       \
    else                                                                                     \
      hipLaunchKernelGGL((ifft2_pass2_gradients_kernel<N, MW_, MPW_, false>), grid, block,   \
                         0, stream, (const cf*)work, (const cf*)patches, pr, (cf*)objproj,   \
                         (cf*)chi0, (float*)m_probe_update, mpu_scale, nscan, S, inv_scale,  \
                         chunk, mpu_part, mode_scale);                                       \
  } while (0)
#define TK_P2G_N(N)                     \
  do {                                  \
    if (MW == 1)                        \
      TK_P2G(N < 256 ? 256 : N, 1, 1);  \
    else if (MW == 2)                   \
      TK_P2G(N, 2, 1);                  \
    else if (MPW == 1)                  \
      TK_P2G(N, 4, 1);                  \
    else                                \
      TK_P2G(N, 4, 2);                  \
  } while (0)
  switch (det) {
    case 128: TK_P2G_N(128); break;
    case 256: TK_P2G_N(256); break;
    default: TK_P2G_N(512); break;
  }
#undef TK_P2G_N
#undef TK_P2G
  TK_LAUNCH_CHECK();
  if (qn) {
    hipLaunchKernelGGL(pass2_q_finish_kernel, dim3((nscan + 3) / 4), dim3(256), 0, stream,
                       qtab, det / 4, nscan, q);
    TK_LAUNCH_CHECK();
  }
  if (mpu_part != nullptr)
    return tk_ordered_sum((float*)m_probe_update, mpu_part, mpu_len, nchunk, true, stream);
  return TK_OK;
}

extern "C" int tike_ifft2_pass2_gradients(const void* work, const void* patches,
                                          const void* probe, const void* eigen_probe,
                                          const float* eigen_weights, int num_eigen,
                                          int eigen_modes, void* objproj, void* chi0,
                                          void* m_probe_update, float mpu_scale, int nscan,
                                          int S, int det, float inv_scale, void* stream) {
  TK_ENTER();
  return launch_pass2_gradients(work, patches, probe, eigen_probe, eigen_weights, num_eigen,
                                eigen_modes, objproj, chi0, m_probe_update, mpu_scale, nscan, S,
                                det, inv_scale, nullptr, (hipStream_t)stream);
}

extern "C" int tike_ifft2_pass2_gradients_scaled(const void* work, const void* patches,
                                                 const void* probe, const void* eigen_probe,
                                                 const float* eigen_weights, int num_eigen,
                                                 int eigen_modes, void* objproj, void* chi0,
                                                 void* m_probe_update, float mpu_scale,
                                                 int nscan, int S, int det, float inv_scale,
                                                 const float* mode_scale, void* stream) {
  TK_ENTER();
  TK_CHECK_ARG(nscan == 0 || mode_scale != nullptr);
  return launch_pass2_gradients(work, patches, probe, eigen_probe, eigen_weights, num_eigen,
                                eigen_modes, objproj, chi0, m_probe_update, mpu_scale, nscan, S,
                                det, inv_scale, mode_scale, (hipStream_t)stream);
}

extern "C" int tike_ifft2_pass2_gradients_eproj(const void* work, const void* patches,
                                                const void* probe, const void* eigen_probe,
                                                const float* eigen_weights, int num_eigen,
                                                int eigen_modes, void* objproj, void* chi0,
                                                void* m_probe_update, float mpu_scale,
                                                int nscan, int S, int det, float inv_scale,
                                                float* qtab, float* q, void* stream) {
  TK_ENTER();
  TK_CHECK_ARG(nscan == 0 || (qtab && q));
  return launch_pass2_gradients(work, patches, probe, eigen_probe, eigen_weights, num_eigen,
                                eigen_modes, objproj, chi0, m_probe_update, mpu_scale, nscan, S,
                                det, inv_scale, nullptr, (hipStream_t)stream, 0, 0, qtab, q);
}

extern "C" int tike_ifft2_pass2_eigen_fits(int det, int num_eigen, int eigen_modes) {
  if (det < 16 || num_eigen < 0 || eigen_modes < 0) return 0;
  return sizeof(cf) * (size_t)num_eigen * eigen_modes * (det / 16) * 64 <= 32 * 1024 ? 1 : 0;
}

extern "C" int tike_ifft2_pass2_gradients_modes(const void* work, const void* patches,
                                                const void* probe, const void* eigen_probe,
                                                const float* eigen_weights, int num_eigen,
                                                int eigen_modes, void* objproj, void* chi0,
                                                void* m_probe_update, float mpu_scale,
                                                int nscan, int S, int det, float inv_scale,
                                                int mode0, int nmodes, int accumulate,
                                                void* stream) {
  TK_ENTER();
  TK_CHECK_ARG(S >= 1 && det >= 1 && mode0 >= 0 && nmodes >= 1 && mode0 + nmodes <= S);
  TK_CHECK_ARG(nscan == 0 || (work && (probe || !objproj)));
  const long P = (long)det * det;
  const bool first = mode0 == 0;
  if (first ? eigen_modes > nmodes : false) return TK_ERR_UNSUPPORTED;
  return launch_pass2_gradients(
      (const cf*)work + mode0 * P, patches, probe ? (const cf*)probe + mode0 * P : nullptr,
      first ? eigen_probe : nullptr, eigen_weights ? eigen_weights + mode0 : nullptr,
      first ? num_eigen : (eigen_weights ? num_eigen : 0), first ? eigen_modes : 0, objproj,
      first ? chi0 : nullptr,
      m_probe_update ? (void*)((float*)m_probe_update + 2 * mode0 * P) : nullptr, mpu_scale,
      nscan, nmodes, det, inv_scale, nullptr, (hipStream_t)stream, S, accumulate);
}

template <int RW>
__global__ __launch_bounds__(256) void probe_precond_rows_kernel(
    const float* __restrict__ scan, const cf* __restrict__ psi, float* __restrict__ out,
    int nscan, int pw, int H, int W, int chunk, float* __restrict__ part) {
  typedef float tk_v4f __attribute__((ext_vector_type(4)));
  const long P = (long)pw * pw;
  const long total = (long)H * W;
  const int cols = pw < 256 ? pw : 256, ncb = pw / cols;
  const int x = ((int)blockIdx.x % ncb) * cols + (int)threadIdx.x % cols;
  const int y0 = (((int)blockIdx.x / ncb) * (256 / cols) + (int)threadIdx.x / cols) * RW;
  const int b0 = blockIdx.y * chunk;
  const int b1 = min(nscan, b0 + chunk);
  float acc[RW];
#pragma unroll
  for (int r = 0; r < RW; ++r) acc[r] = 0.f;
  bool inside = true;
  for (int b = b0; b < b1; ++b) {
    const TkCorner c = tk_corner(scan, b);
    inside = inside && c.sy >= 0 && c.sx >= 0 && c.sy + pw < H && c.sx + pw < W;
  }
  if (inside) {
    const unsigned row_bytes = (unsigned)W * (unsigned)sizeof(cf);
    const unsigned lane_off = (unsigned)y0 * row_bytes + (unsigned)x * (unsigned)sizeof(cf);
#pragma unroll 2
    for (int b = b0; b < b1; ++b) {
      const TkCorner c = tk_corner(scan, b);
      const unsigned off = (unsigned)(c.sy * W + c.sx) * (unsigned)sizeof(cf) + lane_off;
      tk_v4f t[RW + 1];
#pragma unroll
      for (int r = 0; r <= RW; ++r)
        __builtin_memcpy(&t[r], reinterpret_cast<const char*>(psi) + off + (unsigned)r * row_bytes,
                         sizeof(tk_v4f));
#pragma unroll
      for (int r = 0; r < RW; ++r) {
        cf o = mk(t[r].x * c.w00, t[r].y * c.w00);
        o.x += t[r].z * c.w01;
        o.y += t[r].w * c.w01;
        o.x += t[r + 1].x * c.w10;
        o.y += t[r + 1].y * c.w10;
        o.x += t[r + 1].z * c.w11;
        o.y += t[r + 1].w * c.w11;
        acc[r] += norm2(o);
      }
    }
  } else {
    for (int b = b0; b < b1; ++b) {
      const TkCorner c = tk_corner(scan, b);
#pragma unroll
      for (int r = 0; r < RW; ++r) {
        const int y = c.sy + y0 + r, xx = c.sx + x;
        const bool ok = y >= 0 && y < H && xx >= 0 && xx < W;
        const int yc = y < 0 ? 0 : (y >= H ? H - 1 : y);
        const int xc = xx < 0 ? 0 : (xx >= W ? W - 1 : xx);
        const cf o = tk_gather(psi, (long)yc * W + xc, W, total, c);
        acc[r] += ok ? norm2(o) : 0.f;
      }
    }
  }
#pragma unroll
  for (int r = 0; r < RW; ++r) {
    const long p = (long)(y0 + r) * pw + x;
    if (part != nullptr)
      part[(long)blockIdx.y * P + p] = acc[r];
    else
      unsafeAtomicAdd(&out[2 * p], acc[r]);
  }
}

extern "C" int tike_probe_preconditioner(const float* scan, const void* psi, void* out,
                                         int nscan, int pw, int H, int W, void* stream) {
  TK_ENTER();
  TK_CHECK_ARG(nscan >= 0 && pw >= 1 && H >= 1 && W >= 1);
  if (nscan == 0) return TK_OK;
  TK_CHECK_ARG(scan && psi && out);
  const long P = (long)pw * pw;
  float* part = nullptr;
  const int chunk = probe_chunk(nscan, P, &part);
  dim3 grid((unsigned)((P + 255) / 256), (unsigned)((nscan + chunk - 1) / chunk));
  constexpr int RW = 4;
  const int cols = pw < 256 ? pw : 256;
  if (g_stats_pairs && (pw % 256 == 0 || 256 % pw == 0) && pw % ((256 / cols) * RW) == 0 &&
      (long)H * W < (1L << 28)) {
    grid.x = (unsigned)(P / (256 * RW));
    hipLaunchKernelGGL(probe_precond_rows_kernel<RW>, grid, dim3(256), 0, (hipStream_t)stream,
                       scan, (const cf*)psi, (float*)out, nscan, pw, H, W, chunk, part);
  } else {
    launch_probe_grad<false>(grid, (hipStream_t)stream, (const cf*)nullptr, scan,
                             (const cf*)psi, (cf*)nullptr, (float*)out,
                             tk_make_probe(psi, 0, nullptr, nullptr, 0, 0, 1, pw),
                             (cf*)nullptr, nscan, 1, pw, H, W, chunk, part);
  }
  TK_LAUNCH_CHECK();
  if (part != nullptr)
    return tk_ordered_sum((float*)out, part, P, (int)grid.y, true, (hipStream_t)stream, 2);
  return TK_OK;
}
```

tike_amd/csrc/solver.hip:

```cpp
#include "internal.h"
#include "tike_amd.h"

__global__ __launch_bounds__(256) void object_update_precond_kernel(
    const float* __restrict__ acc, const cf* __restrict__ precond,
    const float* __restrict__ pmax, float alpha, cf* __restrict__ upd_sum,
    cf* __restrict__ upd_precond, float* __restrict__ combined, long npix) {
  const float am = alpha * pmax[0];
  for (long i = blockIdx.x * 256L + threadIdx.x; i < npix; i += gridDim.x * 256L) {
    const float re = acc[i], im = acc[npix + i];
    const float p = (1.0f - alpha) * precond[i].x;
    const float inv = 1.0f / sqrtf(p * p + am * am);
    if (upd_sum) upd_sum[i] = mk(re, im);
    if (upd_precond) upd_precond[i] = mk(re * inv, im * inv);
    if (combined) {
      combined[i] += re;
      combined[npix + i] += im;
    }
  }
}

extern "C" int tike_object_update_precond(const float* acc, const void* precond,
                                          const float* pmax, float alpha, void* upd_sum,
                                          void* upd_precond, float* combined, long npix,
                                          void* stream) {
  TK_ENTER();
  TK_CHECK_ARG(npix >= 0);
  if (npix == 0) return TK_OK;
  TK_CHECK_ARG(acc && precond && pmax);
  hipLaunchKernelGGL(object_update_precond_kernel, dim3(tk_grid((npix + 255) / 256, 8)),
                     dim3(256), 0, (hipStream_t)stream, acc, (const cf*)precond, pmax, alpha,
                     (cf*)upd_sum, (cf*)upd_precond, combined, npix);
  TK_LAUNCH_CHECK();
  return TK_OK;
}

__global__ __launch_bounds__(256) void step_sums_kernel(const float* __restrict__ stats,
                                                        const float* __restrict__ costs, int B,
                                                        float eps, float* __restrict__ sums) {
  __shared__ float red[4];
  float a1 = 0.f, a4 = 0.f, c = 0.f;
  for (int n = threadIdx.x; n < B; n += 256) {
    a1 += stats[8 * n] + eps;
    a4 += stats[8 * n + 1] + eps;
    if (costs) c += costs[n];
  }
  a1 = tk_block_sum256(a1, red);
  a4 = tk_block_sum256(a4, red);
  c = tk_block_sum256(c, red);
  if (threadIdx.x == 0) {
    sums[0] = a1;
    sums[1] = a4;
    sums[2] = c;
  }
}

__global__ __launch_bounds__(256) void step_solve_kernel(const float* __restrict__ stats, int B,
                                                         float eps,
                                                         const float* __restrict__ sums,
                                                         float inv_count, int recover_psi,
                                                         int recover_probe,
                                                         float* __restrict__ out) {
  __shared__ float red[4];
  const float r1 = 0.5f * sums[0] * inv_count, r4 = 0.5f * sums[1] * inv_count;
  float so = 0.f, sp = 0.f;
  for (int n = threadIdx.x; n < B; n += 256) {
    const float* s = stats + 8 * n;
    const float A1 = s[0] + eps + r1, A4 = s[1] + eps + r4;
    const float b1 = s[4], b2 = s[5];
    float x1 = 0.f, x2 = 0.f;
    if (recover_psi && recover_probe) {
      const float det = A1 * A4 - (s[2] * s[2] + s[3] * s[3]);
      x1 = -(s[2] * b2 - A4 * b1) / det;
      x2 = (A1 * b2 - s[2] * b1) / det;
    } else if (recover_psi) {
      x1 = b1 / A1;
    } else if (recover_probe) {
      x2 = b2 / A4;
    }
    so += 0.9f * fmaxf(x1, 0.f);
    sp += 0.9f * fmaxf(x2, 0.f);
  }
  so = tk_block_sum256(so, red);
  sp = tk_block_sum256(sp, red);
  if (threadIdx.x == 0) {
    out[0] = so;
    out[1] = sp;
    out[2] = so * inv_count;
    out[3] = sp * inv_count;
    out[4] = sums[2] * inv_count;
  }
}

extern "C" int tike_lstsq_step_sums(const float* stats, const float* costs, int B, float eps,
                                    float* sums, void* stream) {
  TK_ENTER();
  TK_CHECK_ARG(B >= 0 && sums && (B == 0 || stats));
  hipLaunchKernelGGL(step_sums_kernel, dim3(1), dim3(256), 0, (hipStream_t)stream, stats, costs,
                     B, eps, sums);
  TK_LAUNCH_CHECK();
  return TK_OK;
}

extern "C" int tike_lstsq_step_solve(const float* stats, int B, float eps, const float* sums,
                                     double count, int recover_psi, int recover_probe,
                                     float* out, void* stream) {
  TK_ENTER();
  TK_CHECK_ARG(B >= 0 && sums && out && count > 0 && (B == 0 || stats));
  hipLaunchKernelGGL(step_solve_kernel, dim3(1), dim3(256), 0, (hipStream_t)stream, stats, B,
                     eps, sums, (float)(1.0 / count), recover_psi, recover_probe, out);
  TK_LAUNCH_CHECK();
  return TK_OK;
}

__global__ __launch_bounds__(256) void probe_update_kernel(cf* __restrict__ probe,
                                                           cf* __restrict__ combined,
                                                           const cf* __restrict__ mpu,
                                                           const float* __restrict__ beta,
                                                           float inv_num_batch, long n) {
  const float b = beta[0];
  for (long i = blockIdx.x * 256L + threadIdx.x; i < n; i += gridDim.x * 256L) {
    const cf d = mpu[i] * b;
    probe[i] = probe[i] + d;
    if (combined) combined[i] = combined[i] + d * inv_num_batch;
  }
}

extern "C" int tike_probe_update(void* probe, void* combined, const void* mpu,
                                 const float* beta, float inv_num_batch, long n, void* stream) {
  TK_ENTER();
  TK_CHECK_ARG(n >= 0);
  if (n == 0) return TK_OK;
  TK_CHECK_ARG(probe && mpu && beta);
  hipLaunchKernelGGL(probe_update_kernel, dim3(tk_grid((n + 255) / 256, 8)), dim3(256), 0,
                     (hipStream_t)stream, (cf*)probe, (cf*)combined, (const cf*)mpu, beta,
                     inv_num_batch, n);
  TK_LAUNCH_CHECK();
  return TK_OK;
}

__global__ __launch_bounds__(256) void eigen_weights0_kernel(float* __restrict__ weights,
                                                             const float* __restrict__ stats,
                                                             int B, int C, int S, int m,
                                                             float* __restrict__ norms) {
  __shared__ float red[4];
  const long row = (long)(C + 1) * S;
  for (int n = threadIdx.x; n < B; n += 256)
    weights[n * row + m] += 0.1f * stats[8 * n + 6] / stats[8 * n + 7];
  for (int c = 1; c <= C; ++c) {
    float a = 0.f;
    for (int n = threadIdx.x; n < B; n += 256) {
      const float w = weights[n * row + (long)c * S + m];
      a += w * w;
    }
    a = tk_block_sum256(a, red);
    if (threadIdx.x == 0) norms[c - 1] = a;
  }
}

extern "C" int tike_eigen_weights0(float* weights, const float* stats, int B, int C, int S,
                                   int m, float* norms, void* stream) {
  TK_ENTER();
  TK_CHECK_ARG(B >= 0 && C >= 0 && S >= 1 && m >= 0 && m < S);
  if (B == 0) {
    if (C > 0 && norms)
      return (int)hipMemsetAsync(norms, 0, sizeof(float) * (size_t)C, (hipStream_t)stream);
    return TK_OK;
  }
  TK_CHECK_ARG(weights && stats && (C == 0 || norms));
  hipLaunchKernelGGL(eigen_weights0_kernel, dim3(1), dim3(256), 0, (hipStream_t)stream, weights,
                     stats, B, C, S, m, norms);
  TK_LAUNCH_CHECK();
// ... 476 lines not shown
```

tike_amd/ptycho/solvers/_plan.py:

```python
from dataclasses import dataclass
from types import SimpleNamespace

import torch

from ... import _arrays as A
from ..._lib import check, lib

MODELS = {"gaussian": 0, "poisson": 1}


def stored_farplane_gradient(far, data, mask, costs, n, S, det, model,
                             unmeasured, nmeasured, st, rule=None, inten=None,
                             steps=None):
    if rule is not None:
        if inten is None:
            inten = torch.empty((n, det, det), dtype=torch.float32,
                                device=far.device)
        if steps is None:
            steps = torch.empty((n, S), dtype=torch.float32,
                                device=far.device)
        check(lib.tike_intensity(A.ptr(far), A.ptr(inten), n, S, det * det,
                                 st), "intensity")
        check(
            lib.tike_poisson_steps(A.ptr(far), A.ptr(inten), A.ptr(data),
# ... 309 lines not shown
        elif self.one_launch:
            check(
                lib.tike_fwd_grad_ifft2_pass1(
                    A.ptr(b.far), A.ptr(k.data), u16, A.ptr(c.mask_u8),
                    A.ptr(k.costs), A.ptr(b.mid), n, S, det, c.fwd_scale,
                    self.model, c.unmeasured, c.nmeasured, st),
                "column pass + gradient + inverse pass 1")
            return
        else:
            check(
                lib.tike_fwd_gradient_scale(
                    A.ptr(b.far), A.ptr(k.data), u16, A.ptr(c.mask_u8),
                    A.ptr(b.gscale), A.ptr(b.inten) if self.poisson else None,
                    A.ptr(k.costs), None, n, S, det, c.fwd_scale, self.model,
                    c.unmeasured, c.nmeasured, st),
                "forward pass 2 + gradient scale")
        if self.poisson and self.dominant:
            check(
                lib.tike_poisson_steps(
                    None, A.ptr(b.inten), A.ptr(k.data_f32()),
                    A.ptr(c.mask_u8), A.ptr(b.steps), n, S, det, c.step_start,
                    c.step_weight, 1, st), "poisson step lengths")
        steps = A.ptr(b.steps) if self.poisson else None
        smask = A.ptr(c.mask_u8) if self.poisson else None
        if self.fused:
            check(
                lib.tike_grad_ifft2_pass1(A.ptr(b.far), A.ptr(b.gscale), steps,
                                          smask, S, A.ptr(b.mid), n * S, det,
                                          c.fwd_scale, st),
                "gradient + inverse pass 1")
        else:
            check(
                lib.tike_grad_ifft2_crop(A.ptr(b.far), A.ptr(b.gscale), steps,
                                         smask, S, A.ptr(b.mid), A.ptr(b.chi),
                                         n * S, det, pw, c.fwd_scale,
                                         c.inv_scale, st),
                "gradient + ifft2 + crop")

    def _forward_split_kept(self, c, k):
        b, S, det, pw = c.buf, self.S, self.det, self.pw
        n, st, d = k.n, c.st, k.data_f32()
        check(
            lib.tike_fwd_pass1(
                A.ptr(c.psi), A.ptr(k.scan), A.ptr(c.probe), 0, A.ptr(k.uq),
                None, A.ptr(k.w), c.C, c.Sm, A.ptr(b.far), A.ptr(k.patches), n,
                S, pw, det, c.H, c.W, st), "forward pass 1")
        check(
            lib.tike_fwd_gradient_scale(
                A.ptr(b.far), A.ptr(d), 0, A.ptr(c.mask_u8), A.ptr(b.gscale),
                A.ptr(b.inten) if self.poisson else None, A.ptr(k.costs),
                A.ptr(b.mid), n, S, det, c.fwd_scale, self.model, c.unmeasured,
                c.nmeasured, st), "forward pass 2 + gradient scale")
        if self.poisson:
            check(
                lib.tike_poisson_steps(
                    A.ptr(b.mid), A.ptr(b.inten), A.ptr(d), A.ptr(c.mask_u8),
                    A.ptr(b.steps), n, S, det, c.step_start, c.step_weight,
                    self.dominant, st), "poisson step lengths")
        check(
            lib.tike_ifft2_pass1_scaled(
                A.ptr(b.mid), A.ptr(b.gscale),
                A.ptr(b.steps) if self.poisson else None,
                A.ptr(c.mask_u8) if self.poisson else None, S, A.ptr(b.far),
                n * S, det, st), "scaled inverse pass 1")

    def _forward_pos_major(self, c, k):
        b, S, det, pw = c.buf, self.S, self.det, self.pw
        n, st, d = k.n, c.st, k.data_f32()
        check(
            lib.tike_ptycho_fwd_intensity(
                A.ptr(c.psi), A.ptr(k.scan), A.ptr(c.probe), 0, A.ptr(k.uq),
                A.ptr(k.w), c.C, c.Sm, A.ptr(b.far), A.ptr(b.inten),
                A.ptr(k.patches) if self.fused else None, n, S, pw, det, c.H,
                c.W, c.fwd_scale, st), "forward + intensity")
        check(
            lib.tike_gradient_scale(A.ptr(b.inten), A.ptr(d), A.ptr(c.mask_u8),
                                    A.ptr(b.gscale), A.ptr(k.costs), n, det,
                                    self.model, c.unmeasured, c.nmeasured, st),
            "gradient scale")
        if self.poisson:
            check(
                lib.tike_poisson_steps(
                    A.ptr(b.far), A.ptr(b.inten), A.ptr(d), A.ptr(c.mask_u8),
                    A.ptr(b.steps), n, S, det, c.step_start, c.step_weight,
                    self.dominant, st), "poisson step lengths")
        if self.fused:
            check(
                lib.tike_ifft2_pass1_scaled(
                    A.ptr(b.far), A.ptr(b.gscale),
                    A.ptr(b.steps) if self.poisson else None,
                    A.ptr(c.mask_u8) if self.poisson else None, S,
                    A.ptr(b.mid), n * S, det, st), "scaled inverse pass 1")
        elif self.poisson:
            check(
                lib.tike_ifft2_crop_scaled_modes(
                    A.ptr(b.far), A.ptr(b.gscale), A.ptr(b.steps),
                    A.ptr(c.mask_u8), S, A.ptr(b.mid), A.ptr(b.chi), n * S,
                    det, pw, c.inv_scale, st), "scaled ifft2 + crop (poisson)")
        else:
            check(
                lib.tike_ifft2_crop_scaled(A.ptr(b.far), A.ptr(b.gscale), S,
                                           A.ptr(b.mid), A.ptr(b.chi), n * S,
                                           det, pw, c.inv_scale, st),
                "scaled ifft2 + crop")

    def _forward_unfused(self, c, k):
        b, S, det, pw = c.buf, self.S, self.det, self.pw
        n, st, d = k.n, c.st, k.data_f32()
        c.op.fwd_device(c.probe, k.scan, c.psi, c.eigen_probe, k.w,
                        out=b.far[:n])
        stored_farplane_gradient(
            b.far, d, c.mask_u8, k.costs, n, S, det, self.model, c.unmeasured,
            c.nmeasured, st,
            (c.step_start, c.step_weight, self.dominant) if self.poisson
            else None, b.inten, b.steps)
        check(
            lib.tike_ifft2_crop(A.ptr(b.far), A.ptr(b.mid), A.ptr(b.chi), n * S,
                                det, pw, c.inv_scale, st), "ifft2 + crop")

    def gradients(self, c, k):
        b, S, det, pw = c.buf, self.S, self.det, self.pw
        n, st = k.n, c.st
        objproj = (A.ptr(b.objproj) if getattr(c, "want_objproj",
                                               c.recover_psi) else None)
        chi0 = A.ptr(k.chi0) if c.need_chi0 and k.chi0 is not None else None
        if self.pfa:
            check(
                lib.tike_pfa_inv_products(
                    A.ptr(b.far), A.ptr(k.patches), A.ptr(c.probe), 0, None,
                    A.ptr(c.ep), A.ptr(k.w), c.C, c.Sm, objproj, chi0,
                    A.ptr(c.m_probe_update), 1.0 / c.num_batch, n, S, pw, det,
                    c.inv_scale, st), "prime-factor inverse products")
        elif self.general:
            check(
                lib.tike_gen_inv_rows_gradients(
                    A.ptr(b.mid), A.ptr(k.patches), A.ptr(c.probe), 0, None,
                    A.ptr(c.ep), A.ptr(k.w), c.C, c.Sm, objproj, chi0,
                    A.ptr(c.m_probe_update), 1.0 / c.num_batch, n, S, pw, det,
                    c.inv_scale, st), "general inverse rows + gradients")
        elif self.fused:
            p2 = (A.ptr(b.far if self.split_kept else b.mid), A.ptr(k.patches),
                  A.ptr(c.probe), A.ptr(c.ep), A.ptr(k.w), c.C, c.Sm, objproj,
                  chi0, A.ptr(c.m_probe_update), 1.0 / c.num_batch, n, S, det,
                  c.inv_scale)
            if self.groups:
                for first, count in self.groups:
                    check(lib.tike_ifft2_pass2_gradients_modes(
                        *p2, first, count, int(first > 0), st),
                        "inverse pass 2 + gradients (a group of modes)")
            elif self.steps_in_pass2:
                check(lib.tike_ifft2_pass2_gradients_scaled(
                    *p2, A.ptr(b.steps), st),
                    "inverse pass 2 + gradients (x poisson steps)")
            elif k.q is not None:
                check(lib.tike_ifft2_pass2_gradients_eproj(
                    *p2, A.ptr(b.qtab), A.ptr(k.q), st),
                    "inverse pass 2 + gradients + eigen projection")
            else:
                check(lib.tike_ifft2_pass2_gradients(*p2, st),
                      "inverse pass 2 + gradients")
        else:
            check(
                lib.tike_lstsq_gradients(
                    A.ptr(b.chi), A.ptr(k.scan), A.ptr(c.psi), A.ptr(c.probe),
                    A.ptr(c.ep), A.ptr(k.w), c.C, c.Sm,
                    None,
                    A.ptr(k.patches), A.ptr(c.m_probe_update), objproj, n, S,
                    pw, c.H, c.W, st), "probe gradient + object projection")
```

tike_amd/ptycho/solvers/lstsq.py:

```python
import logging
from types import SimpleNamespace

import numpy as np
import torch

from ... import _arrays as A
from ... import _tuning
from ... import linalg
from ... import opt
from ... import random as trandom
from ..._lib import check, lib
from ...operators.propagation import fft_scales
from ..position import gaussian_derivative_taps
from ._plan import MODELS as _MODELS
from ._plan import GradientPlan

logger = logging.getLogger(__name__)


class _Workspace:

    def __init__(self):
        self.buffers = {}

# ... 58 lines not shown
kernels on the mixed-radix transforms or ties with them (300^2 x 1 ... 8 modes
-43 ... -6 %, 400^2 +-0, 500^2 x 4 +7 %, 600^2 x 2 -12 %, 720^2 x 4 -15 %, 1000^2
x 1 ... 4 -3 ... -25 %; with an eigen probe -14 ... +7 %:
profiles/r06_experiments.md section 17).  The launches stay in the tree and
in the tests (`GENERAL_FUSED = "always"`); 256 restores round 6's first rule."""

PFA_ROUTE = True
"""Detector sizes 3 x 2^k, 5 x 2^k and 7 x 2^k (96 ... 3584), and 1024 / 2048, without position-major
kernels take the prime-factor launches of csrc/pfa.hip (tike_pfa_*): the
power-of-two register engine on p x p sub-tiles; tests set this to False to
compare with the LDS line engine of csrc/general.hip."""


MODE_GROUPS = True
"""More modes than one launch of the inverse's second pass holds in registers
(9 ... 32 at 128^2 / 256^2, 5 ... 16 at 512^2; probe window = detector,
gaussian model) run the far-plane-free kernels with that pass in groups of
modes (tike_ifft2_pass2_gradients_modes); False: the position-major kernels
with a stored far plane, as until round 6."""


def mode_groups(S, pw, det, eigen_modes=0):
    cap = 4 if det == 512 else 8
    if not (MODE_GROUPS and pw == det and det in POSITION_MAJOR_SIZES
            and cap < S <= 4 * cap):
        return ()
    k = -(-S // cap)
    base, extra = divmod(S, k)
    sizes = [base + (i < extra) for i in range(k)]
    if min(sizes) < 2 or eigen_modes > sizes[0]:
        return ()
    firsts = [sum(sizes[:i]) for i in range(k)]
    return tuple(zip(firsts, sizes))


PFA_SUBTILES_IN_LDS = True
"""Prime-factor sizes with 128^2 sub-tiles (384, 640, 896): gather and forward
sub-tile transform in one launch, the sub-tile inside LDS
(tike_pfa_fwd_subtiles); False: tike_pfa_fwd_gather + tike_pfa_fft2."""


def pfa_gradients(S, pw, det):
    return bool(PFA_ROUTE and lib.tike_pfa_supported(S, pw, det))


def general_gradients(S, pw, det):
    return bool(GENERAL_FUSED and lib.tike_gen_supported(S, pw, det))


def fused_gradients(S, pw, det):
    return (pw == det and det in POSITION_MAJOR_SIZES
            and S <= (4 if det == 512 else 8))


def chunk_positions(S, det, position_major=False):
    if CHUNK_POSITIONS_OVERRIDE:
        return max(1, int(CHUNK_POSITIONS_OVERRIDE))
    tiles = max(2048, (1 << 33) // (det * det * 8))
    if position_major:
        return max(1024, tiles // max(S, 1))
    return max(64, tiles // max(S, 1))


def global_count(comm, op, lo, hi):
    cache = op.__dict__.setdefault("_tike_amd_counts", {})
    key = minibatch_key(comm, lo, hi)
    if key not in cache:
        cache[key] = comm.Allreduce_count(hi - lo)
    return cache[key]


def minibatch_key(comm, lo, hi):
    return (getattr(comm, "minibatch", None), lo, hi, comm.size)


def mask_info(exitwave_options, det=None):
    mask = exitwave_options.measured_pixels
    if det is not None and tuple(mask.shape) != (det, det):
        raise ValueError(
            f"measured_pixels shape {tuple(mask.shape)} does not match the "
            f"detector ({det}, {det})")
    key = (id(mask), tuple(mask.shape))
    cached = exitwave_options.__dict__.get("_mask_info")
    if cached is None or cached[0] != key:
        m = mask if A.is_device(mask) else A.to_device(
            np.asarray(mask, dtype=bool))
        n = int(m.sum().item())
        info = (n, None if n == m.numel() else m.to(torch.uint8).contiguous())
        cached = (key, info)
        exitwave_options.__dict__["_mask_info"] = cached
    return cached[1]


def lstsq_grad(parameters, data, batches, comm, *, op, epoch):
    scan = parameters.scan
    psi = parameters.psi
    probe = parameters.probe
    algorithm_options = parameters.algorithm_options
    eigen_weights = parameters.eigen_weights
    eigen_probe = parameters.eigen_probe
    exitwave_options = parameters.exitwave_options
    object_options = parameters.object_options
    probe_options = parameters.probe_options
    position_options = parameters.position_options
    if exitwave_options.noise_model not in _MODELS:
        raise ValueError(
            f"unknown noise model {exitwave_options.noise_model!r}")
    recover_probe = (probe_options is not None
                     and epoch >= probe_options.update_start)
    recover_psi = object_options is not None
    num_batch = algorithm_options.num_batch
    compact = algorithm_options.batch_method == "compact"
    order = (range(num_batch) if compact else
             trandom.randomizer_np.permutation(num_batch))
    if hasattr(data, "hint"):
        data.hint([_lo_hi(batches[b]) for b in order])

    dev = psi.device
    H, W = psi.shape[-2:]
    object_combined = (torch.zeros((2, H, W), dtype=torch.float32, device=dev)
                       if recover_psi and compact else None)
    probe_combined_update = torch.zeros_like(probe)
    steps = torch.zeros((num_batch, 5), dtype=torch.float32, device=dev)
    pmax = None
    if recover_psi:
        pmax = torch.amax(object_options.preconditioner.real).reshape(
            1).contiguous()
    beta_object, beta_probe = [], []
    position_terms = None
    if position_options is not None:
        position_terms = (torch.zeros_like(scan), torch.zeros_like(scan))
    packed = PACKED_TAIL and (eigen_probe is None
                              or eigen_probe.shape[-4] == 1)
    eigen_norms = None
    if (packed and recover_probe and eigen_weights is not None
            and eigen_probe is not None):
        eigen_norms = torch.stack([
            torch.square(eigen_weights[_lo_hi(b)[0]:_lo_hi(b)[1], 1, 0]).sum()
            for b in batches
        ]).to(torch.float32).contiguous()
        if comm.collective:
            comm.Allreduce(eigen_norms)

    want_q = bool(FUSED_TAIL and eigen_norms is not None and recover_psi
                  and not comm.collective and not STATS_PATCH_RECOMPUTE)

    for batch_index in order:
        lo, hi = _lo_hi(batches[batch_index])
        comm.minibatch = int(batch_index)
        g = _get_nearplane_gradients(
            data, psi, scan, probe, eigen_probe, eigen_weights, lo, hi, comm,
            num_batch=num_batch, exitwave_options=exitwave_options, op=op,
            recover_psi=recover_psi, recover_probe=recover_probe,
            position_terms=position_terms, want_q=want_q)

        object_update_precond = None
        if recover_psi:
            object_update_precond = _precondition_object_update(
                g["object_acc"], object_options.preconditioner, pmax=pmax,
                combined=object_combined)
        if packed:
            bbeta_object, bbeta_probe = _packed_tail(
                g, psi, scan, probe, eigen_probe, eigen_weights,
                object_update_precond, lo, hi, comm, op=op,
                num_batch=num_batch, recover_psi=recover_psi,
                recover_probe=recover_probe,
                norm=None if eigen_norms is None else
                eigen_norms[batch_index:batch_index + 1],
                steps_row=steps[batch_index],
                probe_combined_update=probe_combined_update)
        else:
            stats = _step_stats(g, psi, scan, probe, eigen_probe,
                                object_update_precond, lo, hi, op=op)

            if recover_probe and eigen_weights is not None:
                eigen_probe, eigen_weights = _update_nearplane(
                    g, stats, probe, eigen_probe, eigen_weights, lo, hi, comm,
                    num_batch=num_batch)

            bbeta_object, bbeta_probe, _ = _solve_steps(
                stats, g["costs"], g["count"], comm, pw=probe.shape[-1],
                recover_psi=recover_psi, recover_probe=recover_probe,
                out=steps[batch_index])

        if recover_psi:
            if not compact:
                dpsi = bbeta_object * object_update_precond
                if object_options.use_adaptive_moment:
                    dpsi, object_options.v, object_options.m = opt.momentum(
                        g=dpsi, v=object_options.v, m=object_options.m,
                        vdecay=object_options.vdecay,
                        mdecay=object_options.mdecay)
                psi = psi + dpsi
            beta_object.append(bbeta_object)

        if recover_probe:
            if not packed:
                check(
                    lib.tike_probe_update(A.ptr(probe),
                                          A.ptr(probe_combined_update),
                                          A.ptr(g["m_probe_update"]),
                                          A.ptr(bbeta_probe), 1.0 / num_batch,
                                          probe.numel(), A.stream_ptr()),
                    "probe update")
            beta_probe.append(bbeta_probe)

    batch_cost = steps[:, 4]
    if position_options is not None:
        scan = _update_position(scan, position_options, *position_terms, comm,
                                epoch=epoch)

    algorithm_options.costs.append([float(batch_cost.mean().item())])
    if (eigen_weights is not None and eigen_weights.shape[1] > 1
            and not np.isfinite(algorithm_options.costs[-1][0])):
        nonzero = torch.stack([
            (eigen_weights[int(idx[0]):int(idx[0]) + len(idx), 1:, 0]
             != 0).sum(dim=0).to(torch.float32) if len(idx) else torch.zeros(
                 eigen_weights.shape[1] - 1, device=psi.device)
            for idx in batches
        ])
        if comm.collective:
            comm.Allreduce(nonzero)
        if bool((nonzero == 0).any().item()):
            raise ValueError("eigen_probe weights cannot all be zero?")

    if recover_psi and compact:
        object_update_precond = _precondition_object_update(
            object_combined, object_options.preconditioner, pmax=pmax)
        bo = torch.mean(torch.stack(beta_object))
        dpsi = bo * object_update_precond
        psi = psi + dpsi
        if object_options.use_adaptive_moment:
            dpsi, object_options.v, object_options.m = _momentum_checked(
                g=dpsi, v=object_options.v, m=object_options.m,
                mdecay=object_options.mdecay,
                errors=[float(x[0]) for x in algorithm_options.costs[-3:]],
                beta=bo, memory_length=3)
            weight = object_options.preconditioner
            weight = weight / (0.1 * weight.real.max() + weight)
            psi = psi + weight * dpsi

    if recover_probe and probe_options.use_adaptive_moment:
        bp = torch.mean(torch.stack(beta_probe))
        dprobe = probe_combined_update
        if probe_options.v is None:
            probe_options.v = torch.zeros((3, *dprobe.shape),
                                          dtype=dprobe.dtype,
                                          device=dprobe.device)
        if probe_options.m is None:
            probe_options.m = torch.zeros_like(dprobe)
        mode = 0
        (d, probe_options.v[..., mode, :, :],
         probe_options.m[..., mode, :, :]) = _momentum_checked(
             g=dprobe[..., mode, :, :], v=probe_options.v[..., mode, :, :],
             m=probe_options.m[..., mode, :, :], mdecay=probe_options.mdecay,
             errors=[float(x[0]) for x in algorithm_options.costs[-3:]],
             beta=bp, memory_length=3)
        probe[..., mode, :, :] = probe[..., mode, :, :] + d

    parameters.scan = scan
    parameters.psi = psi
    parameters.probe = probe
    parameters.eigen_weights = eigen_weights
    parameters.eigen_probe = eigen_probe
    return parameters


EIGEN_PATCH_RECOMPUTE = True
"""The eigen pixel update of the packed tail gathers the object patches from
psi (L2) instead of streaming the stored ones (HBM): 0.186 -> 0.160 ms per 1000
positions at 256^2.  (With two 16-byte tap loads per pixel the position sums
lost by it, 0.215 -> 0.221 ms; see EIGEN_SUMS_RECOMPUTE.)"""

EIGEN_SUMS_RECOMPUTE = _tuning.eigen_sums_gather
"""The position sums gather too, through the two-positions-per-workgroup row
walk of tike_eigen_position_sums1 (one 16-byte tap load per pixel and
position, E_0 and the probe update loaded once per pair): 0.215 -> 0.176 ms
per 1000 positions at 256^2."""

STATS_PATCH_RECOMPUTE = _tuning.stats_gather
"""The step statistics gather O_n from the object with the two 16-byte tap
loads they already issue for the preconditioned update (same offsets)."""

FUSED_TAIL = _tuning.fused_tail
"""One rank, one eigen probe, the fused pass 2 at 128^2 / 256^2: pass 2 leaves
the per-position part of the eigen projection, the eigen update runs before
the step statistics, and the statistics and the eigen position sums are one
pass over chi_n,0 and the patches (tike_lstsq_step_stats_eigen1)."""

PACKED_TAIL = True
"""Tests set this to False to run the staged tail (one entry per step of the
reference's _update_nearplane / _precondition_nearplane_gradients)."""


def _lo_hi(batch):
    lo = int(batch[0]) if len(batch) else 0
    return lo, lo + len(batch)


def _eigen_args(eigen_probe, weights):
    if weights is None:
        return None, None, 0, 0
    C = Sm = 0
    if eigen_probe is not None:
        C, Sm = eigen_probe.shape[-4], eigen_probe.shape[-3]
    assert weights.shape[1] == C + 1, (weights.shape, C)
    return eigen_probe, weights, C, Sm


def _once(make):
    box = []

    def get():
        if not box:
            box.append(make())
        return box[0]

    return get


def _get_nearplane_gradients(data, psi, scan, probe, eigen_probe,
                             eigen_weights, lo, hi, comm, *, num_batch,
                             exitwave_options, op, recover_psi, recover_probe,
                             position_terms=None, need_chi0=True,
                             want_q=False, plain=False,
                             all_mode_position_terms=None):
    dev = psi.device
    B = hi - lo
    S, pw = probe.shape[-3], probe.shape[-1]
    det = op.detector_shape
    H, W = psi.shape[-2:]
    if exitwave_options.noise_model not in _MODELS:
        raise ValueError(
            f"unknown noise model {exitwave_options.noise_model!r}")
    nmeasured, mask_u8 = mask_info(exitwave_options, det)
    fwd_scale, inv_scale = fft_scales(det, op.norm)

    w_old = None if eigen_weights is None else eigen_weights[lo:hi]
    ep, _, C, Sm = _eigen_args(eigen_probe, w_old)
    plan = GradientPlan.for_(op, S, pw, det, exitwave_options, mask_u8,
                             eigen_modes=Sm, num_eigen=C, plain=plain)

    n_obj = 2 * H * W if recover_psi else 0
    n_prb = 2 * probe.numel() if recover_probe else 0
    grads = torch.zeros(n_obj + n_prb, dtype=torch.float32, device=dev)
    obj_acc = grads[:n_obj].view(2, H, W) if recover_psi else None
    m_probe_update = (torch.view_as_complex(
        grads[n_obj:].view(*probe.shape, 2)) if recover_probe else None)
    probe_sum = None
    early = bool(comm.collective and recover_psi and recover_probe)
    buf = plan.buffers(
        _workspace(op), B, dev, varying=Sm if w_old is not None else 0,
        want_patches=bool((recover_probe and eigen_weights is not None)
                          or position_terms))
    if position_terms:
        taps, taps_r = gaussian_derivative_taps(sigma=0.333)
    q = None
    if (want_q and recover_psi and recover_probe and w_old is not None
            and buf.patches is not None and need_chi0
            and plan.eigen_q(C, Sm, H, W)):
        q = _workspace(op).get("eigen_q", (max(B, 1),), torch.float32, dev)
        buf.qtab = _workspace(op).get("eigen_qtab", (min(plan.chunk, max(B, 1)),
                                                     det // 4),
                                      torch.float32, dev)
    c = SimpleNamespace(
        op=op, data=data, psi=psi, probe=probe, ep=ep, eigen_probe=eigen_probe,
        C=C, Sm=Sm, H=H, W=W, st=A.stream_ptr(), fwd_scale=fwd_scale,
        inv_scale=inv_scale, nmeasured=nmeasured, mask_u8=mask_u8,
        unmeasured=(1.0 if plain else
                    float(exitwave_options.unmeasured_pixels_scaling)),
        step_start=float(exitwave_options.step_length_start),
        step_weight=float(exitwave_options.step_length_weight), buf=buf,
        m_probe_update=m_probe_update, num_batch=num_batch,
        recover_psi=recover_psi, need_chi0=need_chi0,
        want_objproj=bool(recover_psi or all_mode_position_terms))
    chunk = plan.chunk
    for clo in range(lo, hi, chunk):
        chi_hi = min(hi, clo + chunk)
        n, blo = chi_hi - clo, clo - lo
        rows = slice(blo, blo + n)
        k = SimpleNamespace(
            n=n, scan=scan[clo:chi_hi], data=data[clo:chi_hi],
            w=None if w_old is None else w_old[rows], uq=None,
            costs=buf.costs[rows],
            patches=None if buf.patches is None else buf.patches[rows],
            chi0=None if buf.chi0 is None else buf.chi0[rows],
            q=None if q is None else q[rows])
        k.data_f32 = _once(lambda a=clo, b=chi_hi: A.data_f32(data, a, b))
        if k.w is not None and Sm > 0 and buf.unique is not None and (
                not plan.no_farplane):
            k.uq = buf.unique[:n]
            check(
                lib.tike_varying_probe(A.ptr(probe), A.ptr(ep), A.ptr(k.w), C,
                                       Sm, A.ptr(k.uq), n, S, pw, c.st),
                "varying probe")
        plan.forward(c, k)
        plan.gradients(c, k)
        stored_chi0 = plan.fused or plan.general
        if position_terms:
            chi_m, chi_modes = ((k.chi0, 1) if stored_chi0 else (buf.chi, S))
            check(
                lib.tike_position_sums(
                    A.ptr(k.patches), A.ptr(chi_m), chi_modes, A.ptr(probe),
                    A.ptr(ep), A.ptr(k.w), C, Sm, taps.ctypes.data, taps_r,
                    A.ptr(position_terms[0][clo:chi_hi]),
                    A.ptr(position_terms[1][clo:chi_hi]), n, S, pw, c.st),
                "position shift sums")
        if all_mode_position_terms:
            all_mode_position_sums(
                op, buf.objproj[:n], psi, k.scan, probe, ep, k.w,
                all_mode_position_terms[0][clo:chi_hi],
                all_mode_position_terms[1][clo:chi_hi])
        if chi_hi == hi and early:
            probe_sum = comm.Allreduce_start(grads[n_obj:])
        if recover_psi:
            check(
                lib.tike_scatter_patches(A.ptr(buf.objproj), A.ptr(k.scan),
                                         A.ptr(obj_acc), n, pw, H, W, c.st),
                "object scatter")
        if not buf.single_chunk and not stored_chi0:
            buf.chi0[rows] = buf.chi[:n, 0, 0]

    if comm.collective and grads.numel():
        if early:
            if probe_sum is None:
                probe_sum = comm.Allreduce_start(grads[n_obj:])
            comm.Allreduce(grads[:n_obj])
            probe_sum.wait()
        else:
            comm.Allreduce(grads)
    count = global_count(comm, op, lo, hi)
    if recover_probe and not (plan.fused or plan.general):
        m_probe_update = m_probe_update / num_batch
    return dict(chi0=buf.chi if buf.single_chunk else buf.chi0[:B],
                chi_modes=S if buf.single_chunk else 1, w_old=w_old,
                patches=None if buf.patches is None else buf.patches[:B],
                object_acc=obj_acc, m_probe_update=m_probe_update,
                costs=buf.costs[:B], count=count, local_count=B,
                q=None if q is None else q[:B])


def all_mode_position_sums(op, objproj, psi, scan, probe, eigen_probe, weights,
                           numerator, denominator, *, per_scan=False):
    n = objproj.shape[0]
    S, pw = probe.shape[-3], probe.shape[-1]
    taps, taps_r = gaussian_derivative_taps(sigma=0.333)
    ep, w, C, Sm = _eigen_args(eigen_probe, weights)
    work = _workspace(op).get("probe_intensity", (pw, pw), torch.float32,
                              psi.device)
    check(
        lib.tike_rpie_position_sums(
            A.ptr(objproj), A.ptr(psi[0]), A.ptr(scan), A.ptr(probe),
            int(per_scan), A.ptr(ep), A.ptr(w), C, Sm, taps.ctypes.data,
            taps_r, A.ptr(work), A.ptr(numerator), A.ptr(denominator), n, S,
            pw, psi.shape[-2], psi.shape[-1], A.stream_ptr()),
        "position shift sums (all modes)")


def positions_allowed_flag(scan, psi_shape, pw):
    corner = torch.floor(scan)
    room = torch.tensor([psi_shape[-2] - pw - 1, psi_shape[-1] - pw - 1],
                        dtype=scan.dtype, device=scan.device)
    ok = ((corner >= 1) & (corner <= room)).all()
    return (~ok).to(torch.float32)


def object_upd_sum(g):
    acc = g["object_acc"]
    return None if acc is None else torch.complex(acc[0], acc[1])[None]


def _precondition_object_update(object_acc, psi_update_denominator,
                                alpha=0.05, *, pmax=None, combined=None):
    H, W = object_acc.shape[-2:]
    if pmax is None:
        pmax = torch.amax(psi_update_denominator.real).reshape(1).contiguous()
    out = torch.empty((1, H, W), dtype=torch.complex64,
                      device=object_acc.device)
    check(
        lib.tike_object_update_precond(A.ptr(object_acc),
                                       A.ptr(psi_update_denominator),
                                       A.ptr(pmax), alpha, None, A.ptr(out),
                                       A.ptr(combined), H * W, A.stream_ptr()),
        "preconditioned object update")
    return out


def _step_stats(g, psi, scan, probe, eigen_probe, object_update_precond, lo,
                hi, *, op):
    B = hi - lo
    dev = psi.device
    S, pw = probe.shape[-3], probe.shape[-1]
    stats = _workspace(op).get("stats", (max(B, 1), 8), torch.float32, dev)
    ep, w_old, C, Sm = _eigen_args(eigen_probe, g["w_old"])
    eigen0 = eproj = None
    if (ep is not None and C >= 1 and Sm >= 1 and g["patches"] is not None
            and g["m_probe_update"] is not None):
        eigen0 = ep[0, 0, 0]
        eproj = _workspace(op).get("eigen_proj", (max(B, 1),), torch.float32,
                                   dev)
    g["eigen_proj"] = None if eproj is None else eproj[:B]
    check(
        lib.tike_lstsq_step_stats(
            A.ptr(g["chi0"]), A.ptr(scan[lo:hi]), A.ptr(psi),
            A.ptr(object_update_precond), A.ptr(probe), A.ptr(ep),
            A.ptr(w_old), C, Sm, None, A.ptr(g["m_probe_update"]),
            None if (STATS_PATCH_RECOMPUTE and psi.shape[0] == 1
                     and object_update_precond is not None) else
            A.ptr(g["patches"]), A.ptr(stats), B,
            S, g["chi_modes"], pw, psi.shape[-2], psi.shape[-1],
            A.ptr(eigen0), A.ptr(eproj), A.stream_ptr()),
        "step-size statistics")
    return stats[:B]


def _packed_tail(g, psi, scan, probe, eigen_probe, eigen_weights,
                 object_update_precond, lo, hi, comm, *, op, num_batch,
                 recover_psi, recover_probe, norm, steps_row,
                 probe_combined_update):
    B = hi - lo
    dev = psi.device
    st = A.stream_ptr()
    S, pw = probe.shape[-3], probe.shape[-1]
    P = pw * pw
    count = float(g["count"])
    ws = _workspace(op)
    eig = recover_probe and eigen_weights is not None
    C = Sm = 0
    if eig and eigen_probe is not None:
        C, Sm = eigen_probe.shape[-4], eigen_probe.shape[-3]
        assert eigen_weights.shape[-2] == C + 1 and C == 1
    mpu = g["m_probe_update"]
    one = (eig and C == 1 and Sm >= 1 and g["patches"] is not None
           and mpu is not None and norm is not None)
    assert one or C == 0, "packed tail: eigen probe without its operands"
    small = ws.get("tail_small", (4 + 2 * P + 8,), torch.float32, dev)
    small.zero_()
    sums3 = small[:3]
    update = small[4:4 + 2 * P]
    nacc = small[4 + 2 * P:4 + 2 * P + 4]
    tail3 = small[4 + 2 * P + 4:4 + 2 * P + 7]
    if (one and g.get("q") is not None and not comm.collective
            and object_update_precond is not None and psi.shape[0] == 1):
        return _fused_tail(g, psi, scan, probe, eigen_probe, eigen_weights,
                           object_update_precond, lo, hi, op=op,
                           num_batch=num_batch, recover_psi=recover_psi,
                           recover_probe=recover_probe, norm=norm,
                           steps_row=steps_row,
                           probe_combined_update=probe_combined_update,
                           sums3=sums3, update=update, nacc=nacc, tail3=tail3)
    stats = _step_stats(g, psi, scan, probe, eigen_probe,
                        object_update_precond, lo, hi, op=op)
    eps_total = float(np.float32(np.float32(1e-9) / P) * P)
    E = w_rows = sums5 = None
    row = 0
    if eig:
        w_rows = eigen_weights[lo:hi]
        row = w_rows.shape[-2] * w_rows.shape[-1]
    gpsi = A.ptr(psi[0]) if EIGEN_PATCH_RECOMPUTE and psi.shape[0] == 1 else None
    if one:
        E = eigen_probe[0, 0, 0]
        check(
            lib.tike_eigen_pixel_update1(
                A.ptr(g["patches"]), A.ptr(g["chi0"]), A.ptr(mpu[0, 0, 0]),
                A.ptr(E), A.ptr(g["eigen_proj"]), w_rows[:, 1, 0].data_ptr(),
                row, A.ptr(norm), A.ptr(update), B, pw, g["chi_modes"],
                A.ptr(stats), A.ptr(g["costs"]), eps_total, A.ptr(sums3),
                gpsi, A.ptr(scan[lo:hi]), psi.shape[-2], psi.shape[-1], st),
            "eigen pixel update")
    else:
        check(
            lib.tike_lstsq_step_sums(A.ptr(stats), A.ptr(g["costs"]), B,
                                     eps_total, A.ptr(sums3), st),
            "step-size sums")
    if comm.collective:
        comm.Allreduce(small[:4 + 2 * P] if one else small[:4])
    beta_eigen = min(0.1, 1.0 / num_batch)
    check(
        lib.tike_lstsq_tail_mid(A.ptr(E), A.ptr(update), P, A.ptr(nacc),
                                beta_eigen, A.ptr(stats), B, eps_total,
                                A.ptr(sums3), count, int(recover_psi),
                                int(recover_probe), A.ptr(tail3), st),
        "step solve")
    if one:
        sums5 = ws.get("eigen_sums5", (max(B, 1), 5), torch.float32, dev)
        check(
            lib.tike_eigen_position_sums1(
                A.ptr(g["patches"]), A.ptr(g["chi0"]), A.ptr(mpu[0, 0, 0]),
                A.ptr(E), A.ptr(sums5), tail3[2:].data_ptr(), B, pw,
                g["chi_modes"], gpsi if EIGEN_SUMS_RECOMPUTE else None,
                A.ptr(scan[lo:hi]), psi.shape[-2], psi.shape[-1], st),
            "eigen position sums")
    if comm.collective:
        comm.Allreduce(tail3)
    check(
        lib.tike_lstsq_tail_finish(
            A.ptr(tail3), A.ptr(sums3), count, A.ptr(steps_row),
            A.ptr(probe) if recover_probe else None,
            A.ptr(probe_combined_update) if recover_probe else None,
            A.ptr(mpu), 1.0 / num_batch, probe.numel(),
            None if w_rows is None else w_rows.data_ptr(), row, S, 0,
            A.ptr(stats), A.ptr(sums5), B, P, st), "minibatch tail")
    return (steps_row[2] if recover_psi else None,
            steps_row[3] if recover_probe else None)


def _fused_tail(g, psi, scan, probe, eigen_probe, eigen_weights,
                object_update_precond, lo, hi, *, op, num_batch, recover_psi,
                recover_probe, norm, steps_row, probe_combined_update, sums3,
                update, nacc, tail3):
    B = hi - lo
    dev = psi.device
    st = A.stream_ptr()
    S, pw = probe.shape[-3], probe.shape[-1]
    P = pw * pw
    H, W = psi.shape[-2:]
    count = float(g["count"])
    ws = _workspace(op)
    mpu = g["m_probe_update"]
    Sm = eigen_probe.shape[-3]
    w_rows = eigen_weights[lo:hi]
    row = w_rows.shape[-2] * w_rows.shape[-1]
    E = eigen_probe[0, 0, 0]
    eps_total = float(np.float32(np.float32(1e-9) / P) * P)
    stats = ws.get("stats", (max(B, 1), 8), torch.float32, dev)
    sums5 = ws.get("eigen_sums5", (max(B, 1), 5), torch.float32, dev)
    eproj = ws.get("eigen_proj", (max(B, 1),), torch.float32, dev)
    c0part = ws.get("eigen_c0part", (64,), torch.float32, dev)
    g["eigen_proj"] = eproj[:B]
    gpsi = A.ptr(psi[0]) if EIGEN_PATCH_RECOMPUTE else None
    scan_b = A.ptr(scan[lo:hi])
    check(
        lib.tike_eigen_pixel_update1q(
            A.ptr(g["patches"]), A.ptr(g["chi0"]), A.ptr(mpu[0, 0, 0]),
            A.ptr(E), A.ptr(g["q"]), w_rows[:, 1, 0].data_ptr(), row,
            A.ptr(norm), A.ptr(update), B, pw, g["chi_modes"], gpsi, scan_b,
            H, W, A.ptr(c0part), A.ptr(eproj), st),
        "eigen pixel update")
    beta_eigen = min(0.1, 1.0 / num_batch)
    check(
        lib.tike_lstsq_step_stats_eigen1(
            A.ptr(g["chi0"]), scan_b, A.ptr(object_update_precond),
            A.ptr(probe), A.ptr(eigen_probe), A.ptr(g["w_old"]), Sm,
            A.ptr(mpu), A.ptr(g["patches"]), A.ptr(update), A.ptr(nacc), count,
            beta_eigen, A.ptr(stats), A.ptr(sums5), B, S, g["chi_modes"], pw,
            H, W, st),
        "step-size statistics + eigen position sums")
    check(
        lib.tike_lstsq_tail_solve1(
            A.ptr(E), A.ptr(update), P, A.ptr(nacc), beta_eigen, A.ptr(stats),
            A.ptr(g["costs"]), A.ptr(sums5), B, eps_total, count,
            int(recover_psi), int(recover_probe), A.ptr(sums3), A.ptr(tail3),
            st), "eigen probe + step solve")
    check(
        lib.tike_lstsq_tail_finish(
            A.ptr(tail3), A.ptr(sums3), count, A.ptr(steps_row),
            A.ptr(probe) if recover_probe else None,
            A.ptr(probe_combined_update) if recover_probe else None,
            A.ptr(mpu), 1.0 / num_batch, probe.numel(), w_rows.data_ptr(), row,
            S, 0, A.ptr(stats), A.ptr(sums5), B, P, st), "minibatch tail")
    g["stats"] = stats[:B]
    g["sums5"] = sums5[:B]
    return (steps_row[2] if recover_psi else None,
            steps_row[3] if recover_probe else None)


def _solve_steps(stats, costs, count, comm, *, pw, recover_psi, recover_probe,
                 out=None):
    dev = stats.device
    B = stats.shape[0]
    st = A.stream_ptr()
    eps_total = float(np.float32(np.float32(1e-9) / (pw * pw)) * (pw * pw))
    if out is None:
        out = torch.zeros(5, dtype=torch.float32, device=dev)
    sums = torch.empty(3, dtype=torch.float32, device=dev)
    check(
        lib.tike_lstsq_step_sums(A.ptr(stats), A.ptr(costs), B, eps_total,
                                 A.ptr(sums), st), "step-size sums")
    if comm.collective:
        comm.Allreduce(sums)
    check(
        lib.tike_lstsq_step_solve(A.ptr(stats), B, eps_total, A.ptr(sums),
                                  float(count), int(recover_psi),
                                  int(recover_probe), A.ptr(out), st),
        "step-size solve")
    if comm.collective:
        comm.Allreduce(out[:2])
        out[2:4] = out[:2] / count
    return (out[2] if recover_psi else None,
            out[3] if recover_probe else None, out[4])


def _update_nearplane(g, stats, probe, eigen_probe, eigen_weights, lo, hi,
                      comm, *, num_batch):
    m = 0
    dev = probe.device
    count = float(g["count"])
    B = hi - lo
    st = A.stream_ptr()
    Cw, S = eigen_weights.shape[-2] - 1, eigen_weights.shape[-1]
    row = (Cw + 1) * S
    w_rows = eigen_weights[lo:hi]
    norms = torch.empty(max(Cw, 1), dtype=torch.float32, device=dev)
    check(
        lib.tike_eigen_weights0(A.ptr(w_rows), A.ptr(stats), B, Cw, S, m,
                                A.ptr(norms), st), "eigen weights (shared)")
    if Cw < 1 or eigen_probe is None:
        return eigen_probe, eigen_weights
    if m >= eigen_probe.shape[-3]:
        return eigen_probe, eigen_weights
    assert eigen_weights.shape[-2] == eigen_probe.shape[-4] + 1
    if comm.collective:
        comm.Allreduce(norms)
    chi0, patches = g["chi0"], g["patches"]
    mpu0 = g["m_probe_update"][0, 0, m]
    C, Sm, pw = eigen_probe.shape[-4], eigen_probe.shape[-3], probe.shape[-1]
    P = pw * pw
    beta = min(0.1, 1.0 / num_batch)
    sums = torch.empty((max(B, 1), 5), dtype=torch.float32, device=dev)
    coefs = torch.zeros((max(B, 1), C), dtype=torch.complex64, device=dev)
    pm = torch.empty(max(B, 1), dtype=torch.float32, device=dev)
    small = torch.empty(2, dtype=torch.float32, device=dev)
    nwork = torch.empty(4, dtype=torch.float32, device=dev)
    ep = eigen_probe

    def position_sums(c):
        check(
            lib.tike_eigen_position_sums(A.ptr(patches), A.ptr(chi0),
                                         A.ptr(mpu0), A.ptr(ep), A.ptr(coefs),
                                         C, Sm, c, A.ptr(sums), B, pw,
                                         g["chi_modes"], st),
            "eigen position sums")

    for c in range(1, C + 1):
        w_c = w_rows[:, c, m]
        if c == 1 and g.get("eigen_proj") is not None:
            first, stride = g["eigen_proj"], 1
        else:
            position_sums(c - 1)
            first, stride = sums, 5
        check(
            lib.tike_eigen_proj_mean(A.ptr(first), stride, w_c.data_ptr(), row,
                                     norms[c - 1:].data_ptr(), P, B,
                                     A.ptr(pm), st), "eigen projection mean")
        update = torch.zeros((pw, pw), dtype=torch.complex64, device=dev)
        check(
            lib.tike_eigen_pixel_update(A.ptr(patches), A.ptr(chi0),
                                        A.ptr(mpu0), A.ptr(ep), A.ptr(coefs),
                                        C, Sm, c - 1, A.ptr(pm),
                                        A.ptr(update), B, pw, g["chi_modes"],
                                        st),
            "eigen pixel update")
        if comm.collective:
            comm.Allreduce(update)
        E = ep[0, c - 1, m]
        check(
            lib.tike_eigen_normalise(A.ptr(E), A.ptr(update), count, beta, P,
                                     small[1:].data_ptr(), A.ptr(nwork), st),
            "eigen probe normalisation")
        position_sums(c - 1)
        check(lib.tike_eigen_dsum(A.ptr(sums), B, P, A.ptr(small), st),
              "eigen weight denominator")
        if comm.collective:
            comm.Allreduce(small[:1])
        more = c + 1 < eigen_weights.shape[-2]
        check(
            lib.tike_eigen_weights(A.ptr(sums), B, P, A.ptr(small), count,
                                   w_c.data_ptr(), row,
                                   coefs[:, c - 1:].data_ptr() if more else
                                   None, C, small[1:].data_ptr(), st),
            "eigen weights")
    return eigen_probe, eigen_weights


def _trimmed_mean(rows, proportion=0.05):
    count = rows.shape[0]
    cut = int(proportion * count)
    return torch.sort(rows, dim=0).values[cut:count - cut].mean(dim=0)


def _update_position(scan, position_options, numerator, denominator, comm,
                     *, alpha=0.05, epoch=0):
    po = position_options
    if epoch < po.update_start:
        return scan
    damping = alpha * torch.clamp(comm.Allreduce_max(denominator.max()),
                                  min=1e-6)
    shift = numerator / ((1 - alpha) * denominator + damping)
    limit = po.update_magnitude_limit
    if limit > 0:
        shift = shift.clamp(-limit, limit)
    shift -= _trimmed_mean(comm.Allgather_rows(shift))
    if po.use_adaptive_moment:
        moments = dict(vdecay=po.vdecay, mdecay=po.mdecay)
# ... 24 lines not shown
```

Measured before the change: 215,400 patterns/s.

## Merge small tail launches into block-range fused kernels around scatter

Defers the object scatter out of the chunked gradient loop when one chunk holds the minibatch. It then merges several small kernels by block ranges: the q finish, the c0 partials and the zeroing go into one prep kernel, and the object preconditioning and eigen norm sums go into one kernel. This cuts the launch count from pass 2 to the end of the tail, which matters because these kernels are small and launch overhead dominates. In exchange it adds new entry points and flags that change the order of state in the tail path, which must stay consistent.

```diff
diff --git a/include/tike_amd.h b/include/tike_amd.h
--- a/include/tike_amd.h
+++ b/include/tike_amd.h
@@ -395,6 +395,31 @@
                               long weights_row, const float* norm, void* update, int nscan,
                               int pw, int chi_modes, const void* psi, const float* scan, int H,
                               int W, float* c0part, float* eproj_out, void* stream);
+int tike_ifft2_pass2_gradients_qtab(const void* work, const void* patches, const void* probe,
+                                    const void* eigen_probe, const float* eigen_weights,
+                                    int num_eigen, int eigen_modes, void* objproj, void* chi0,
+                                    void* m_probe_update, float mpu_scale, int nscan, int S,
+                                    int det, float inv_scale, float* qtab, void* stream);
+int tike_eigen_tail_prep(const float* qtab, int det, int nscan, float* q, const void* mpu0,
+                         const void* eigen0, int pw, float* c0part, float* zero, long nzero,
+                         void* stream);
+int tike_eigen_pixel_update1q_c0(const void* patches, const void* chi0, const void* mpu0,
+                                 const void* eigen0, const float* q, const float* weights_c,
+                                 long weights_row, const float* norm, void* update, int nscan,
+                                 int pw, int chi_modes, const void* psi, const float* scan, int H,
+                                 int W, const float* c0part, float* eproj_out, void* stream);
+int tike_object_precond_norm_sums1(const float* acc, const void* precond, const float* pmax,
+                                   float alpha, void* upd_precond, float* combined, long npix,
+                                   const void* eigen0, const void* update, int pw, float* nacc,
+                                   void* stream);
+int tike_lstsq_step_stats_eigen1_nacc(const void* chi, const float* scan,
+                                      const void* object_update_precond, const void* probe,
+                                      const void* eigen_probe, const float* eigen_weights,
+                                      int eigen_modes, const void* m_probe_update,
+                                      const void* patches, const void* update,
+                                      const float* nacc, double count, float beta_eigen,
+                                      float* stats, float* sums5, int nscan, int S,
+                                      int chi_modes, int pw, int H, int W, void* stream);
 int tike_lstsq_step_stats_eigen1(const void* chi, const float* scan,
                                  const void* object_update_precond, const void* probe,
                                  const void* eigen_probe, const float* eigen_weights,
diff --git a/tike_amd/_lib.py b/tike_amd/_lib.py
--- a/tike_amd/_lib.py
+++ b/tike_amd/_lib.py
@@ -155,6 +155,16 @@
                                          _p, _f, _i, _i, _i, _f, _p, _p, _p],
     "tike_eigen_pixel_update1q": [_p, _p, _p, _p, _p, _p, _l, _p, _p, _i, _i,
                                   _i, _p, _p, _i, _i, _p, _p, _p],
+    "tike_ifft2_pass2_gradients_qtab": [_p, _p, _p, _p, _p, _i, _i, _p, _p, _p,
+                                        _f, _i, _i, _i, _f, _p, _p],
+    "tike_eigen_tail_prep": [_p, _i, _i, _p, _p, _p, _i, _p, _p, _l, _p],
+    "tike_object_precond_norm_sums1": [_p, _p, _p, _f, _p, _p, _l, _p, _p, _i,
+                                       _p, _p],
+    "tike_lstsq_step_stats_eigen1_nacc": [_p, _p, _p, _p, _p, _p, _i, _p, _p,
+                                          _p, _p, _d, _f, _p, _p, _i, _i, _i,
+                                          _i, _i, _i, _p],
+    "tike_eigen_pixel_update1q_c0": [_p, _p, _p, _p, _p, _p, _l, _p, _p, _i,
+                                     _i, _i, _p, _p, _i, _i, _p, _p, _p],
     "tike_lstsq_step_stats_eigen1": [_p, _p, _p, _p, _p, _p, _i, _p, _p, _p,
                                      _p, _d, _f, _p, _p, _i, _i, _i, _i, _i,
                                      _i, _p],
diff --git a/tike_amd/csrc/lstsq.hip b/tike_amd/csrc/lstsq.hip
--- a/tike_amd/csrc/lstsq.hip
+++ b/tike_amd/csrc/lstsq.hip
@@ -1,6 +1,7 @@
 #include <type_traits>
 
 #include "internal.h"
+#include "tail_small.h"
 #include "tike_amd.h"
 
 template <bool HAVE_PATCHES, bool HAVE_GOBJ>
@@ -495,19 +496,12 @@
   return c.sy >= 0 && c.sx >= 0 && c.sy + pw < H && c.sx + pw < W && (long)H * W < (1L << 28);
 }
 
-constexpr int TK_C0_PARTS = 64;
 __global__ __launch_bounds__(256) void eigen_proj_offset_kernel(const cf* __restrict__ mpu0,
                                                                 const cf* __restrict__ E,
                                                                 long P,
                                                                 float* __restrict__ part) {
   __shared__ float red[4];
-  float a = 0.f;
-  for (long p = blockIdx.x * 256L + threadIdx.x; p < P; p += 256L * TK_C0_PARTS) {
-    const cf m = mpu0[p], e = E[p];
-    a += m.x * e.x + m.y * e.y;
-  }
-  a = tk_block_sum256(a, red);
-  if (threadIdx.x == 0) part[blockIdx.x] = a;
+  tk_c0_partial_block(mpu0, E, P, part, blockIdx.x, red);
 }
 
 __global__ __launch_bounds__(256) void eigen_pixel_update1_kernel(
@@ -914,38 +908,16 @@
                                                                int npix, float* __restrict__ nacc,
                                                                float* __restrict__ part) {
   __shared__ float red[4];
-  float uu = 0.f, ee = 0.f, eu = 0.f;
-  for (int i = blockIdx.x * 256 + threadIdx.x; i < npix; i += gridDim.x * 256) {
-    const cf e = E[i], u = update[i];
-    uu += norm2(u);
-    ee += norm2(e);
-    eu += e.x * u.x + e.y * u.y;
-  }
-  uu = tk_block_sum256(uu, red);
-  ee = tk_block_sum256(ee, red);
-  eu = tk_block_sum256(eu, red);
-  if (threadIdx.x == 0) {
-    if (part != nullptr) {
-      part[3 * blockIdx.x] = uu;
-      part[3 * blockIdx.x + 1] = ee;
-      part[3 * blockIdx.x + 2] = eu;
-    } else {
-      unsafeAtomicAdd(&nacc[0], uu);
-      unsafeAtomicAdd(&nacc[1], ee);
-      unsafeAtomicAdd(&nacc[2], eu);
-    }
-  }
-}
-
-extern "C" int tike_lstsq_step_stats_eigen1(const void* chi, const float* scan,
-                                            const void* object_update_precond, const void* probe,
-                                            const void* eigen_probe, const float* eigen_weights,
-                                            int eigen_modes, const void* m_probe_update,
-                                            const void* patches, const void* update, float* nacc,
-                                            double count, float beta_eigen, float* stats,
-                                            float* sums5, int nscan, int S, int chi_modes,
-                                            int pw, int H, int W, void* stream) {
-  TK_ENTER();
+  tk_norm_sums1_block(E, update, npix, nacc, part, blockIdx.x, gridDim.x, red);
+}
+
+static int step_stats_eigen1(const void* chi, const float* scan,
+                             const void* object_update_precond, const void* probe,
+                             const void* eigen_probe, const float* eigen_weights,
+                             int eigen_modes, const void* m_probe_update, const void* patches,
+                             const void* update, float* nacc, double count, float beta_eigen,
+                             float* stats, float* sums5, int nscan, int S, int chi_modes, int pw,
+                             int H, int W, void* stream, bool norm_sums) {
   TK_CHECK_ARG(nscan >= 0 && S >= 1 && chi_modes >= 1 && pw >= 1 && H >= 1 && W >= 1 &&
                eigen_modes >= 1 && count > 0);
   TK_CHECK_ARG(probe && eigen_probe && eigen_weights && m_probe_update && update && nacc);
@@ -958,18 +930,20 @@
   if (!((pw % 256 == 0 || 256 % pw == 0) && pw % (nsplit * groups) == 0 &&
         (long)H * W < (1L << 28)))
     return TK_ERR_UNSUPPORTED;
-  int grid = P >= 256 * 64 ? 64 : (int)((P + 255) / 256);
-  float* part = nullptr;
-  if (tk_deterministic()) {
-    part = tk_det_scratch(sizeof(float) * 3 * (size_t)grid);
-    if (part == nullptr) grid = 1;
-  }
-  hipLaunchKernelGGL(eigen_norm_sums1_kernel, dim3(grid), dim3(256), 0, (hipStream_t)stream,
-                     (const cf*)eigen_probe, (const cf*)update, (int)P, nacc, part);
-  TK_LAUNCH_CHECK();
-  if (part != nullptr) {
-    int rc = tk_ordered_sum(nacc, part, 3, grid, true, (hipStream_t)stream);
-    if (rc) return rc;
+  if (norm_sums) {
+    int grid = P >= 256 * 64 ? 64 : (int)((P + 255) / 256);
+    float* part = nullptr;
+    if (tk_deterministic()) {
+      part = tk_det_scratch(sizeof(float) * 3 * (size_t)grid);
+      if (part == nullptr) grid = 1;
+    }
+    hipLaunchKernelGGL(eigen_norm_sums1_kernel, dim3(grid), dim3(256), 0, (hipStream_t)stream,
+                       (const cf*)eigen_probe, (const cf*)update, (int)P, nacc, part);
+    TK_LAUNCH_CHECK();
+    if (part != nullptr) {
+      int rc = tk_ordered_sum(nacc, part, 3, grid, true, (hipStream_t)stream);
+      if (rc) return rc;
+    }
   }
   if (nscan == 0) return TK_OK;
   TK_CHECK_ARG(chi && scan && object_update_precond && patches && stats && sums5);
@@ -989,6 +963,32 @@
                      nsplit);
   TK_LAUNCH_CHECK();
   return TK_OK;
+}
+
+extern "C" int tike_lstsq_step_stats_eigen1(const void* chi, const float* scan,
+                                            const void* object_update_precond, const void* probe,
+                                            const void* eigen_probe, const float* eigen_weights,
+                                            int eigen_modes, const void* m_probe_update,
+                                            const void* patches, const void* update, float* nacc,
+                                            double count, float beta_eigen, float* stats,
+                                            float* sums5, int nscan, int S, int chi_modes,
+                                            int pw, int H, int W, void* stream) {
+  TK_ENTER();
+  return step_stats_eigen1(chi, scan, object_update_precond, probe, eigen_probe, eigen_weights,
+                           eigen_modes, m_probe_update, patches, update, nacc, count, beta_eigen,
+                           stats, sums5, nscan, S, chi_modes, pw, H, W, stream, true);
+}
+
+extern "C" int tike_lstsq_step_stats_eigen1_nacc(
+    const void* chi, const float* scan, const void* object_update_precond, const void* probe,
+    const void* eigen_probe, const float* eigen_weights, int eigen_modes,
+    const void* m_probe_update, const void* patches, const void* update, const float* nacc,
+    double count, float beta_eigen, float* stats, float* sums5, int nscan, int S, int chi_modes,
+    int pw, int H, int W, void* stream) {
+  TK_ENTER();
+  return step_stats_eigen1(chi, scan, object_update_precond, probe, eigen_probe, eigen_weights,
+                           eigen_modes, m_probe_update, patches, update, (float*)nacc, count,
+                           beta_eigen, stats, sums5, nscan, S, chi_modes, pw, H, W, stream, false);
 }
 
 static TkResidual make_residual(const void* patches, const void* chi0, const void* mpu0,
@@ -1089,21 +1089,20 @@
   return TK_OK;
 }
 
-extern "C" int tike_eigen_pixel_update1q(const void* patches, const void* chi0,
-                                         const void* mpu0, const void* eigen0, const float* q,
-                                         const float* weights_c, long weights_row,
-                                         const float* norm, void* update, int nscan, int pw,
-                                         int chi_modes, const void* psi, const float* scan,
-                                         int H, int W, float* c0part, float* eproj_out,
-                                         void* stream) {
-  TK_ENTER();
+static int eigen_pixel_update1q(const void* patches, const void* chi0, const void* mpu0,
+                                const void* eigen0, const float* q, const float* weights_c,
+                                long weights_row, const float* norm, void* update, int nscan,
+                                int pw, int chi_modes, const void* psi, const float* scan, int H,
+                                int W, float* c0part, float* eproj_out, void* stream,
+                                bool c0_ready) {
   TK_CHECK_ARG(nscan >= 0 && pw >= 1 && chi_modes >= 1 && weights_row >= 1);
   if (nscan == 0) return TK_OK;
   TK_CHECK_ARG(!psi || (scan && H >= 1 && W >= 1));
   TK_CHECK_ARG(patches && chi0 && mpu0 && eigen0 && q && weights_c && norm && update && c0part);
   const long P = (long)pw * pw;
-  hipLaunchKernelGGL(eigen_proj_offset_kernel, dim3(TK_C0_PARTS), dim3(256), 0,
-                     (hipStream_t)stream, (const cf*)mpu0, (const cf*)eigen0, P, c0part);
+  if (!c0_ready)
+    hipLaunchKernelGGL(eigen_proj_offset_kernel, dim3(TK_C0_PARTS), dim3(256), 0,
+                       (hipStream_t)stream, (const cf*)mpu0, (const cf*)eigen0, P, c0part);
   float* part = nullptr;
   const int chunk = probe_chunk(nscan, 2 * P, &part);
   dim3 grid((unsigned)((P + 255) / 256) + 1, (unsigned)((nscan + chunk - 1) / chunk));
@@ -1115,6 +1114,102 @@
   TK_LAUNCH_CHECK();
   if (part != nullptr)
     return tk_ordered_sum((float*)update, part, 2 * P, (int)grid.y, true, (hipStream_t)stream);
+  return TK_OK;
+}
+
+extern "C" int tike_eigen_pixel_update1q(const void* patches, const void* chi0,
+                                         const void* mpu0, const void* eigen0, const float* q,
+                                         const float* weights_c, long weights_row,
+                                         const float* norm, void* update, int nscan, int pw,
+                                         int chi_modes, const void* psi, const float* scan,
+                                         int H, int W, float* c0part, float* eproj_out,
+                                         void* stream) {
+  TK_ENTER();
+  return eigen_pixel_update1q(patches, chi0, mpu0, eigen0, q, weights_c, weights_row, norm, update,
+                              nscan, pw, chi_modes, psi, scan, H, W, c0part, eproj_out, stream,
+                              false);
+}
+
+extern "C" int tike_eigen_pixel_update1q_c0(const void* patches, const void* chi0,
+                                            const void* mpu0, const void* eigen0, const float* q,
+                                            const float* weights_c, long weights_row,
+                                            const float* norm, void* update, int nscan, int pw,
+                                            int chi_modes, const void* psi, const float* scan,
+                                            int H, int W, const float* c0part, float* eproj_out,
+                                            void* stream) {
+  TK_ENTER();
+  return eigen_pixel_update1q(patches, chi0, mpu0, eigen0, q, weights_c, weights_row, norm, update,
+                              nscan, pw, chi_modes, psi, scan, H, W, (float*)c0part, eproj_out,
+                              stream, true);
+}
+
+__global__ __launch_bounds__(256) void eigen_tail_prep_kernel(
+    const float* __restrict__ qtab, int slots, int nscan, float* __restrict__ q, unsigned nq,
+    const cf* __restrict__ mpu0, const cf* __restrict__ E, long P, float* __restrict__ c0part,
+    float* __restrict__ zero, long nzero) {
+  __shared__ float red[4];
+  const unsigned b = blockIdx.x;
+  if (b < nq) {
+    tk_q_finish_block(qtab, slots, nscan, q, b);
+  } else if (b < nq + TK_C0_PARTS) {
+    tk_c0_partial_block(mpu0, E, P, c0part, b - nq, red);
+  } else {
+    const long nb = gridDim.x - nq - TK_C0_PARTS;
+    for (long i = (long)(b - nq - TK_C0_PARTS) * 256 + threadIdx.x; i < nzero; i += nb * 256)
+      zero[i] = 0.f;
+  }
+}
+
+extern "C" int tike_eigen_tail_prep(const float* qtab, int det, int nscan, float* q,
+                                    const void* mpu0, const void* eigen0, int pw, float* c0part,
+                                    float* zero, long nzero, void* stream) {
+  TK_ENTER();
+  TK_CHECK_ARG(nscan >= 0 && det >= 4 && det / 4 <= 64 && pw >= 1 && nzero >= 0);
+  TK_CHECK_ARG(nscan == 0 || (qtab && q));
+  TK_CHECK_ARG(mpu0 && eigen0 && c0part && (nzero == 0 || zero));
+  const unsigned nq = (unsigned)((nscan + 3) / 4);
+  const unsigned nz = (unsigned)tk_grid((nzero + 1023) / 1024, 2);
+  hipLaunchKernelGGL(eigen_tail_prep_kernel, dim3(nq + TK_C0_PARTS + (nzero ? nz : 0)), dim3(256),
+                     0, (hipStream_t)stream, qtab, det / 4, nscan, q, nq, (const cf*)mpu0,
+                     (const cf*)eigen0, (long)pw * pw, c0part, zero, nzero);
+  TK_LAUNCH_CHECK();
+  return TK_OK;
+}
+
+__global__ __launch_bounds__(256) void object_precond_norm_sums1_kernel(
+    const float* __restrict__ acc, const cf* __restrict__ precond,
+    const float* __restrict__ pmax, float alpha, cf* __restrict__ upd_precond,
+    float* __restrict__ combined, long npix, unsigned ng, const cf* __restrict__ E,
+    const cf* __restrict__ update, int P, float* __restrict__ nacc, float* __restrict__ part) {
+  __shared__ float red[4];
+  if (blockIdx.x < ng)
+    tk_object_precond_block(acc, precond, pmax, alpha, nullptr, upd_precond, combined, npix,
+                            blockIdx.x, ng);
+  else
+    tk_norm_sums1_block(E, update, P, nacc, part, blockIdx.x - ng, gridDim.x - ng, red);
+}
+
+extern "C" int tike_object_precond_norm_sums1(const float* acc, const void* precond,
+                                              const float* pmax, float alpha, void* upd_precond,
+                                              float* combined, long npix, const void* eigen0,
+                                              const void* update, int pw, float* nacc,
+                                              void* stream) {
+  TK_ENTER();
+  TK_CHECK_ARG(npix >= 1 && pw >= 1);
+  TK_CHECK_ARG(acc && precond && pmax && upd_precond && eigen0 && update && nacc);
+  const long P = (long)pw * pw;
+  const unsigned ng = (unsigned)tk_grid((npix + 255) / 256, 8);
+  int grid = P >= 256 * 64 ? 64 : (int)((P + 255) / 256);
+  float* part = nullptr;
+  if (tk_deterministic()) {
+    part = tk_det_scratch(sizeof(float) * 3 * (size_t)grid);
+    if (part == nullptr) grid = 1;
+  }
+  hipLaunchKernelGGL(object_precond_norm_sums1_kernel, dim3(ng + (unsigned)grid), dim3(256), 0,
+                     (hipStream_t)stream, acc, (const cf*)precond, pmax, alpha, (cf*)upd_precond,
+                     combined, npix, ng, (const cf*)eigen0, (const cf*)update, (int)P, nacc, part);
+  TK_LAUNCH_CHECK();
+  if (part != nullptr) return tk_ordered_sum(nacc, part, 3, grid, true, (hipStream_t)stream);
   return TK_OK;
 }
 
diff --git a/tike_amd/csrc/lstsq_gradients.hip b/tike_amd/csrc/lstsq_gradients.hip
--- a/tike_amd/csrc/lstsq_gradients.hip
+++ b/tike_amd/csrc/lstsq_gradients.hip
@@ -2,6 +2,7 @@
 #include <type_traits>
 
 #include "internal.h"
+#include "tail_small.h"
 #include "tike_amd.h"
 
 constexpr int TK_MAX_MODES = 16;
@@ -433,11 +434,7 @@
 __global__ __launch_bounds__(256) void pass2_q_finish_kernel(const float* __restrict__ qtab,
                                                              int slots, int nscan,
                                                              float* __restrict__ q) {
-  const int n = blockIdx.x * 4 + (int)(threadIdx.x >> 6), k = threadIdx.x & 63;
-  if (n >= nscan) return;
-  float a = k < slots ? qtab[(long)k * nscan + n] : 0.f;
-  a = tk_wave_sum(a);
-  if (k == 0) q[n] = a;
+  tk_q_finish_block(qtab, slots, nscan, q, blockIdx.x);
 }
 
 template <int N, int MW_, int MPW_>
@@ -461,12 +458,13 @@
                                   void* m_probe_update, float mpu_scale, int nscan, int S,
                                   int det, float inv_scale, const float* mode_scale,
                                   hipStream_t stream, int Stot = 0, int accumulate = 0,
-                                  float* qtab = nullptr, float* q = nullptr) {
+                                  float* qtab = nullptr, float* q = nullptr,
+                                  bool qtab_only = false) {
   TK_CHECK_ARG(nscan >= 0 && S >= 1 && det >= 1);
   if (nscan == 0) return TK_OK;
   TK_CHECK_ARG(work && patches && (probe || !objproj));
   if (S > 8 || (det != 128 && det != 256 && det != 512)) return TK_ERR_UNSUPPORTED;
-  const bool qn = q != nullptr;
+  const bool qn = q != nullptr || qtab_only;
   TK_CHECK_ARG(!qn || qtab);
   if (qn && (Stot != 0 || det > 256 || !objproj || !eigen_probe || !eigen_weights ||
              num_eigen < 1 || eigen_modes < 1))
@@ -566,7 +564,7 @@
 #undef TK_P2G_N
 #undef TK_P2G
   TK_LAUNCH_CHECK();
-  if (qn) {
+  if (q != nullptr) {
     hipLaunchKernelGGL(pass2_q_finish_kernel, dim3((nscan + 3) / 4), dim3(256), 0, stream,
                        qtab, det / 4, nscan, q);
     TK_LAUNCH_CHECK();
@@ -614,6 +612,21 @@
   return launch_pass2_gradients(work, patches, probe, eigen_probe, eigen_weights, num_eigen,
                                 eigen_modes, objproj, chi0, m_probe_update, mpu_scale, nscan, S,
                                 det, inv_scale, nullptr, (hipStream_t)stream, 0, 0, qtab, q);
+}
+
+extern "C" int tike_ifft2_pass2_gradients_qtab(const void* work, const void* patches,
+                                               const void* probe, const void* eigen_probe,
+                                               const float* eigen_weights, int num_eigen,
+                                               int eigen_modes, void* objproj, void* chi0,
+                                               void* m_probe_update, float mpu_scale, int nscan,
+                                               int S, int det, float inv_scale, float* qtab,
+                                               void* stream) {
+  TK_ENTER();
+  TK_CHECK_ARG(nscan == 0 || qtab);
+  return launch_pass2_gradients(work, patches, probe, eigen_probe, eigen_weights, num_eigen,
+                                eigen_modes, objproj, chi0, m_probe_update, mpu_scale, nscan, S,
+                                det, inv_scale, nullptr, (hipStream_t)stream, 0, 0, qtab, nullptr,
+                                true);
 }
 
 extern "C" int tike_ifft2_pass2_eigen_fits(int det, int num_eigen, int eigen_modes) {
diff --git a/tike_amd/csrc/solver.hip b/tike_amd/csrc/solver.hip
--- a/tike_amd/csrc/solver.hip
+++ b/tike_amd/csrc/solver.hip
@@ -1,22 +1,13 @@
 #include "internal.h"
+#include "tail_small.h"
 #include "tike_amd.h"
 
 __global__ __launch_bounds__(256) void object_update_precond_kernel(
     const float* __restrict__ acc, const cf* __restrict__ precond,
     const float* __restrict__ pmax, float alpha, cf* __restrict__ upd_sum,
     cf* __restrict__ upd_precond, float* __restrict__ combined, long npix) {
-  const float am = alpha * pmax[0];
-  for (long i = blockIdx.x * 256L + threadIdx.x; i < npix; i += gridDim.x * 256L) {
-    const float re = acc[i], im = acc[npix + i];
-    const float p = (1.0f - alpha) * precond[i].x;
-    const float inv = 1.0f / sqrtf(p * p + am * am);
-    if (upd_sum) upd_sum[i] = mk(re, im);
-    if (upd_precond) upd_precond[i] = mk(re * inv, im * inv);
-    if (combined) {
-      combined[i] += re;
-      combined[npix + i] += im;
-    }
-  }
+  tk_object_precond_block(acc, precond, pmax, alpha, upd_sum, upd_precond, combined, npix,
+                          blockIdx.x, gridDim.x);
 }
 
 extern "C" int tike_object_update_precond(const float* acc, const void* precond,
diff --git a/tike_amd/csrc/tail_small.h b/tike_amd/csrc/tail_small.h
--- /dev/null
+++ b/tike_amd/csrc/tail_small.h
@@ -0,0 +1,72 @@
+#pragma once
+#include "common.h"
+
+__device__ __forceinline__ void tk_q_finish_block(const float* __restrict__ qtab, int slots,
+                                                  int nscan, float* __restrict__ q, unsigned block) {
+  const int n = block * 4 + (int)(threadIdx.x >> 6), k = threadIdx.x & 63;
+  if (n >= nscan) return;
+  float a = k < slots ? qtab[(long)k * nscan + n] : 0.f;
+  a = tk_wave_sum(a);
+  if (k == 0) q[n] = a;
+}
+
+constexpr int TK_C0_PARTS = 64;
+__device__ __forceinline__ void tk_c0_partial_block(const cf* __restrict__ mpu0,
+                                                    const cf* __restrict__ E, long P,
+                                                    float* __restrict__ part, unsigned block,
+                                                    float* red) {
+  float a = 0.f;
+  for (long p = block * 256L + threadIdx.x; p < P; p += 256L * TK_C0_PARTS) {
+    const cf m = mpu0[p], e = E[p];
+    a += m.x * e.x + m.y * e.y;
+  }
+  a = tk_block_sum256(a, red);
+  if (threadIdx.x == 0) part[block] = a;
+}
+
+__device__ __forceinline__ void tk_object_precond_block(
+    const float* __restrict__ acc, const cf* __restrict__ precond,
+    const float* __restrict__ pmax, float alpha, cf* __restrict__ upd_sum,
+    cf* __restrict__ upd_precond, float* __restrict__ combined, long npix, unsigned block,
+    unsigned nblock) {
+  const float am = alpha * pmax[0];
+  for (long i = block * 256L + threadIdx.x; i < npix; i += nblock * 256L) {
+    const float re = acc[i], im = acc[npix + i];
+    const float p = (1.0f - alpha) * precond[i].x;
+    const float inv = 1.0f / sqrtf(p * p + am * am);
+    if (upd_sum) upd_sum[i] = mk(re, im);
+    if (upd_precond) upd_precond[i] = mk(re * inv, im * inv);
+    if (combined) {
+      combined[i] += re;
+      combined[npix + i] += im;
+    }
+  }
+}
+
+__device__ __forceinline__ void tk_norm_sums1_block(const cf* __restrict__ E,
+                                                    const cf* __restrict__ update, int npix,
+                                                    float* __restrict__ nacc,
+                                                    float* __restrict__ part, unsigned block,
+                                                    unsigned nblock, float* red) {
+  float uu = 0.f, ee = 0.f, eu = 0.f;
+  for (int i = block * 256 + threadIdx.x; i < npix; i += nblock * 256) {
+    const cf e = E[i], u = update[i];
+    uu += norm2(u);
+    ee += norm2(e);
+    eu += e.x * u.x + e.y * u.y;
+  }
+  uu = tk_block_sum256(uu, red);
+  ee = tk_block_sum256(ee, red);
+  eu = tk_block_sum256(eu, red);
+  if (threadIdx.x == 0) {
+    if (part != nullptr) {
+      part[3 * block] = uu;
+      part[3 * block + 1] = ee;
+      part[3 * block + 2] = eu;
+    } else {
+      unsafeAtomicAdd(&nacc[0], uu);
+      unsafeAtomicAdd(&nacc[1], ee);
+      unsafeAtomicAdd(&nacc[2], eu);
+    }
+  }
+}
diff --git a/tike_amd/ptycho/solvers/_plan.py b/tike_amd/ptycho/solvers/_plan.py
--- a/tike_amd/ptycho/solvers/_plan.py
+++ b/tike_amd/ptycho/solvers/_plan.py
@@ -485,6 +485,10 @@
                 check(lib.tike_ifft2_pass2_gradients_scaled(
                     *p2, A.ptr(b.steps), st),
                     "inverse pass 2 + gradients (x poisson steps)")
+            elif k.q is not None and getattr(c, "q_unfinished", False):
+                check(lib.tike_ifft2_pass2_gradients_qtab(
+                    *p2, A.ptr(b.qtab), st),
+                    "inverse pass 2 + gradients + eigen projection partials")
             elif k.q is not None:
                 check(lib.tike_ifft2_pass2_gradients_eproj(
                     *p2, A.ptr(b.qtab), A.ptr(k.q), st),
diff --git a/tike_amd/ptycho/solvers/lstsq.py b/tike_amd/ptycho/solvers/lstsq.py
--- a/tike_amd/ptycho/solvers/lstsq.py
+++ b/tike_amd/ptycho/solvers/lstsq.py
@@ -234,10 +234,19 @@
             data, psi, scan, probe, eigen_probe, eigen_weights, lo, hi, comm,
             num_batch=num_batch, exitwave_options=exitwave_options, op=op,
             recover_psi=recover_psi, recover_probe=recover_probe,
-            position_terms=position_terms, want_q=want_q)
+            position_terms=position_terms, want_q=want_q,
+            defer_scatter=want_q and MERGED_SMALL_LAUNCHES)
 
         object_update_precond = None
-        if recover_psi:
+        if g.get("objproj") is not None:
+            _second_pass(
+                g, psi, scan, eigen_probe, eigen_weights, lo, hi, op=op,
+                norm=eigen_norms[batch_index:batch_index + 1])
+        if g.get("eigen_updated"):
+            object_update_precond = _precondition_object_update(
+                g["object_acc"], object_options.preconditioner, pmax=pmax,
+                combined=object_combined, eigen=(g, eigen_probe, op))
+        elif recover_psi:
             object_update_precond = _precondition_object_update(
                 g["object_acc"], object_options.preconditioner, pmax=pmax,
                 combined=object_combined)
@@ -370,6 +379,13 @@
 the step statistics, and the statistics and the eigen position sums are one
 pass over chi_n,0 and the patches (tike_lstsq_step_stats_eigen1)."""
 
+MERGED_SMALL_LAUNCHES = True
+"""Where the fused tail applies and one chunk holds the minibatch, the small
+launches around its scatter and eigen pixel update are merged by block
+ranges: [q finish | c0 partials | zeroing] in front (tike_eigen_tail_prep),
+[precondition | norm sums] behind (tike_object_precond_norm_sums1): eight
+launches from pass 2 to the end of the tail instead of eleven."""
+
 PACKED_TAIL = True
 """Tests set this to False to run the staged tail (one entry per step of the
 reference's _update_nearplane / _precondition_nearplane_gradients)."""
@@ -406,7 +422,8 @@
                              exitwave_options, op, recover_psi, recover_probe,
                              position_terms=None, need_chi0=True,
                              want_q=False, plain=False,
-                             all_mode_position_terms=None):
+                             all_mode_position_terms=None,
+                             defer_scatter=False):
     dev = psi.device
     B = hi - lo
     S, pw = probe.shape[-3], probe.shape[-1]
@@ -457,6 +474,9 @@
         recover_psi=recover_psi, need_chi0=need_chi0,
         want_objproj=bool(recover_psi or all_mode_position_terms))
     chunk = plan.chunk
+    deferred = bool(defer_scatter and q is not None and psi.shape[0] == 1
+                    and 0 < B <= chunk and not comm.collective)
+    c.q_unfinished = deferred
     for clo in range(lo, hi, chunk):
         chi_hi = min(hi, clo + chunk)
         n, blo = chi_hi - clo, clo - lo
@@ -495,7 +515,7 @@
                 all_mode_position_terms[1][clo:chi_hi])
         if chi_hi == hi and early:
             probe_sum = comm.Allreduce_start(grads[n_obj:])
-        if recover_psi:
+        if recover_psi and not deferred:
             check(
                 lib.tike_scatter_patches(A.ptr(buf.objproj), A.ptr(k.scan),
                                          A.ptr(obj_acc), n, pw, H, W, c.st),
@@ -519,7 +539,9 @@
                 patches=None if buf.patches is None else buf.patches[:B],
                 object_acc=obj_acc, m_probe_update=m_probe_update,
                 costs=buf.costs[:B], count=count, local_count=B,
-                q=None if q is None else q[:B])
+                q=None if q is None else q[:B],
+                objproj=buf.objproj[:B] if deferred else None,
+                qtab=buf.qtab if deferred else None)
 
 
 def all_mode_position_sums(op, objproj, psi, scan, probe, eigen_probe, weights,
@@ -553,12 +575,28 @@
 
 
 def _precondition_object_update(object_acc, psi_update_denominator,
-                                alpha=0.05, *, pmax=None, combined=None):
+                                alpha=0.05, *, pmax=None, combined=None,
+                                eigen=None):
     H, W = object_acc.shape[-2:]
     if pmax is None:
         pmax = torch.amax(psi_update_denominator.real).reshape(1).contiguous()
     out = torch.empty((1, H, W), dtype=torch.complex64,
                       device=object_acc.device)
+    if eigen is not None:
+        g, eigen_probe, op = eigen
+        pw = eigen_probe.shape[-1]
+        P = pw * pw
+        small = _workspace(op).get("tail_small", (4 + 2 * P + 8,),
+                                   torch.float32, object_acc.device)
+        check(
+            lib.tike_object_precond_norm_sums1(
+                A.ptr(object_acc), A.ptr(psi_update_denominator), A.ptr(pmax),
+                alpha, A.ptr(out), A.ptr(combined), H * W,
+                A.ptr(eigen_probe[0, 0, 0]), A.ptr(small[4:4 + 2 * P]), pw,
+                A.ptr(small[4 + 2 * P:4 + 2 * P + 4]), A.stream_ptr()),
+            "preconditioned object update + eigen update norms")
+        g["nacc_ready"] = True
+        return out
     check(
         lib.tike_object_update_precond(A.ptr(object_acc),
                                        A.ptr(psi_update_denominator),
@@ -617,7 +655,8 @@
            and mpu is not None and norm is not None)
     assert one or C == 0, "packed tail: eigen probe without its operands"
     small = ws.get("tail_small", (4 + 2 * P + 8,), torch.float32, dev)
-    small.zero_()
+    if not g.get("eigen_updated"):
+        small.zero_()
     sums3 = small[:3]
     update = small[4:4 + 2 * P]
     nacc = small[4 + 2 * P:4 + 2 * P + 4]
@@ -687,6 +726,40 @@
             steps_row[3] if recover_probe else None)
 
 
+def _second_pass(g, psi, scan, eigen_probe, eigen_weights, lo, hi, *, op, norm):
+    B = hi - lo
+    dev = psi.device
+    pw = g["objproj"].shape[-1]
+    P = pw * pw
+    H, W = psi.shape[-2:]
+    st = A.stream_ptr()
+    ws = _workspace(op)
+    small = ws.get("tail_small", (4 + 2 * P + 8,), torch.float32, dev)
+    eproj = ws.get("eigen_proj", (max(B, 1),), torch.float32, dev)
+    c0part = ws.get("eigen_c0part", (64,), torch.float32, dev)
+    w_rows = eigen_weights[lo:hi]
+    row = w_rows.shape[-2] * w_rows.shape[-1]
+    mpu0, E = g["m_probe_update"][0, 0, 0], eigen_probe[0, 0, 0]
+    scan_b = A.ptr(scan[lo:hi])
+    check(
+        lib.tike_eigen_tail_prep(A.ptr(g["qtab"]), op.detector_shape, B,
+                                 A.ptr(g["q"]), A.ptr(mpu0), A.ptr(E), pw,
+                                 A.ptr(c0part), A.ptr(small), small.numel(),
+                                 st), "eigen tail preparation")
+    check(
+        lib.tike_scatter_patches(A.ptr(g["objproj"]), scan_b,
+                                 A.ptr(g["object_acc"]), B, pw, H, W, st),
+        "object scatter")
+    check(
+        lib.tike_eigen_pixel_update1q_c0(
+            A.ptr(g["patches"]), A.ptr(g["chi0"]), A.ptr(mpu0), A.ptr(E),
+            A.ptr(g["q"]), w_rows[:, 1, 0].data_ptr(), row, A.ptr(norm),
+            A.ptr(small[4:4 + 2 * P]), B, pw, g["chi_modes"],
+            A.ptr(psi[0]) if EIGEN_PATCH_RECOMPUTE else None, scan_b, H, W,
+            A.ptr(c0part), A.ptr(eproj), st), "eigen pixel update")
+    g["eigen_updated"] = True
+
+
 def _fused_tail(g, psi, scan, probe, eigen_probe, eigen_weights,
                 object_update_precond, lo, hi, *, op, num_batch, recover_psi,
                 recover_probe, norm, steps_row, probe_combined_update, sums3,
@@ -712,16 +785,19 @@
     g["eigen_proj"] = eproj[:B]
     gpsi = A.ptr(psi[0]) if EIGEN_PATCH_RECOMPUTE else None
     scan_b = A.ptr(scan[lo:hi])
-    check(
-        lib.tike_eigen_pixel_update1q(
-            A.ptr(g["patches"]), A.ptr(g["chi0"]), A.ptr(mpu[0, 0, 0]),
-            A.ptr(E), A.ptr(g["q"]), w_rows[:, 1, 0].data_ptr(), row,
-            A.ptr(norm), A.ptr(update), B, pw, g["chi_modes"], gpsi, scan_b,
-            H, W, A.ptr(c0part), A.ptr(eproj), st),
-        "eigen pixel update")
+    if not g.get("eigen_updated"):
+        check(
+            lib.tike_eigen_pixel_update1q(
+                A.ptr(g["patches"]), A.ptr(g["chi0"]), A.ptr(mpu[0, 0, 0]),
+                A.ptr(E), A.ptr(g["q"]), w_rows[:, 1, 0].data_ptr(), row,
+                A.ptr(norm), A.ptr(update), B, pw, g["chi_modes"], gpsi,
+                scan_b, H, W, A.ptr(c0part), A.ptr(eproj), st),
+            "eigen pixel update")
     beta_eigen = min(0.1, 1.0 / num_batch)
-    check(
-        lib.tike_lstsq_step_stats_eigen1(
+    stats_entry = (lib.tike_lstsq_step_stats_eigen1_nacc
+                   if g.get("nacc_ready") else lib.tike_lstsq_step_stats_eigen1)
+    check(
+        stats_entry(
             A.ptr(g["chi0"]), scan_b, A.ptr(object_update_precond),
             A.ptr(probe), A.ptr(eigen_probe), A.ptr(g["w_old"]), Sm,
             A.ptr(mpu), A.ptr(g["patches"]), A.ptr(update), A.ptr(nacc), count,
```

Result: no change. 215,200 patterns/s (-0.1%).
